# iosefa/obia

Measured on AMD Instinct MI355X. Metric: Mpixel/s (SLIC+zonal feats) on 16384²×8-band; achieved HBM GB/s fraction, higher is better.
Workload: dtype f32

## Files before the change

include/obia_testing.h:

```cpp
#ifndef OBIA_TESTING_H
#define OBIA_TESTING_H

#include "obia_hip.h"

#ifdef __cplusplus
extern "C" {
#endif

int obia_test_clear_ranges_dev(obia_ctx *ctx, void *const *dev_ptrs, const int64_t *bytes, const int32_t *values, int n);

int obia_test_sweep_plan(const int64_t *problems, int n_problems, const int32_t *settings, int repeat, const int32_t *switches,
                         const int64_t *residencies, char *text, int64_t text_bytes);

int obia_test_launch_grid(const char *name, const int64_t *sizes, int n_sizes, int64_t *out4);

int obia_test_launch_grid_names(char *text, int64_t text_bytes);

int obia_test_seam_sort_limit(void);

#ifdef __cplusplus
}
#endif
#endif
```

obia_amd/_lib.py:

```python
import ctypes
import os
import subprocess

import numpy as np

_CSRC = os.path.join(os.path.dirname(os.path.abspath(__file__)), "csrc")
LIB_PATH = os.environ.get("OBIA_HIP_LIB") or os.path.join(_CSRC, "libobia_hip.so")

OBIA_OK = 0
MASK_SEEDS_CHUNK = 1024
E_INVALID, E_HIP, E_NOMEM, E_UNSUPPORTED, E_EMPTY, E_NONFINITE = -1, -2, -3, -4, -5, -6
E_INTERNAL = -7


class SlicParams(ctypes.Structure):
    _fields_ = [("compactness", ctypes.c_double), ("min_size_factor", ctypes.c_double),
                ("max_size_factor", ctypes.c_double), ("n_segments", ctypes.c_int32),
                ("max_num_iter", ctypes.c_int32), ("convert2lab", ctypes.c_int32),
                ("enforce_connectivity", ctypes.c_int32), ("slic_zero", ctypes.c_int32),
                ("start_label", ctypes.c_int32), ("normalize_bands", ctypes.c_int32),
                ("exit_on_fixed_point", ctypes.c_int32), ("reserved", ctypes.c_int32),
                ("sigma_zyx", ctypes.c_double * 3), ("spacing_zyx", ctypes.c_double * 3)]


class SlicSeeds(ctypes.Structure):
    _fields_ = [("yx", ctypes.c_void_p), ("steps_zyx", ctypes.c_double * 3), ("n", ctypes.c_int32),
                ("reserved", ctypes.c_int32)]


class SlicStages(ctypes.Structure):
    _fields_ = [("features", ctypes.c_void_p), ("seeds_yx", ctypes.c_void_p), ("centroids", ctypes.c_void_p),
                ("labels_pre", ctypes.c_void_p), ("centroid_capacity", ctypes.c_int32), ("prepass_only", ctypes.c_int32),
                ("prepass_iters", ctypes.c_int32), ("K", ctypes.c_int32), ("step", ctypes.c_double), ("prescale", ctypes.c_double),
                ("fscale", ctypes.c_double)]


class TilingParams(ctypes.Structure):
    _fields_ = [("crown_radius", ctypes.c_double), ("pixel_width", ctypes.c_double),
                ("pixel_height", ctypes.c_double), ("tile_size", ctypes.c_int32), ("buffer", ctypes.c_int32),
                ("white_order", ctypes.c_int32), ("reserved", ctypes.c_int32)]


class Forest(ctypes.Structure):
    _fields_ = [("threshold", ctypes.c_void_p), ("feature", ctypes.c_void_p), ("left", ctypes.c_void_p), ("right", ctypes.c_void_p),
                ("missing_go_to_left", ctypes.c_void_p), ("tree_offset", ctypes.c_void_p), ("tree_offset_host", ctypes.c_void_p),
                ("value", ctypes.c_void_p), ("n_nodes", ctypes.c_int64), ("n_trees", ctypes.c_int32), ("n_classes", ctypes.c_int32)]


class Mlp(ctypes.Structure):
    _fields_ = [("weights", ctypes.c_void_p), ("biases", ctypes.c_void_p), ("layer_sizes", ctypes.c_void_p), ("n_layers", ctypes.c_int32),
                ("hidden_activation", ctypes.c_int32), ("out_activation", ctypes.c_int32), ("n_classes", ctypes.c_int32)]


_P = ctypes.c_void_p
_I = ctypes.c_int
SEEDING_GRID, SEEDING_SKIMAGE = 0, 1
PickFn = ctypes.CFUNCTYPE(ctypes.c_int, ctypes.c_void_p, ctypes.c_int64, ctypes.c_int32, ctypes.POINTER(ctypes.c_void_p),
                          ctypes.POINTER(ctypes.c_int32), ctypes.POINTER(ctypes.c_void_p), ctypes.POINTER(ctypes.c_int64))
_SIGNATURES = {
    "obia_abi_version": (ctypes.c_int, []),
    "obia_last_error": (ctypes.c_char_p, []),
    "obia_create": (_P, [_I]),
    "obia_create_on_stream": (_P, [_I, _P]),
    "obia_destroy": (None, [_P]),
    "obia_synchronize": (_I, [_P]),
    "obia_workspace_bytes": (ctypes.c_int64, [_P]),
    "obia_slic_default_params": (None, [ctypes.POINTER(SlicParams)]),
    "obia_slic_f32": (_I, [_P, _P, _I, _I, _I, _P, ctypes.POINTER(SlicParams), _P, ctypes.POINTER(_I)]),
    "obia_slic_f32_dev": (_I, [_P, _P, _I, _I, _I, _P, ctypes.POINTER(SlicParams), _P, ctypes.POINTER(_I)]),
    "obia_slic_assign_only_f32_dev": (_I, [_P, _P, _I, _I, _I, _P, ctypes.POINTER(SlicParams), _P, ctypes.POINTER(_I)]),
    "obia_slic_seeded_f32_dev": (_I, [_P, _P, _I, _I, _I, _P, ctypes.POINTER(SlicParams), ctypes.POINTER(SlicSeeds), _I, _P,
                                      ctypes.POINTER(_I)]),
    "obia_mask_centroids_dev": (_I, [_P, _P, _I, _I, _P, ctypes.c_int32, _P, ctypes.c_int64, _I, _P, _P]),
    "obia_slic_stages_f32_dev": (_I, [_P, _P, _I, _I, _I, _P, ctypes.POINTER(SlicParams), ctypes.POINTER(SlicSeeds),
                                      ctypes.POINTER(SlicStages)]),
    "obia_enforce_connectivity_i32_dev": (_I, [_P, _P, _I, _I, _I, _I, _I, _P, ctypes.POINTER(_I)]),
    "obia_zonal_stats_f32": (_I, [_P, _P, _P, _I, _I, _I, _P, _I, _I, _I, _P, _P, _P, _P, _P]),
    "obia_zonal_stats_f32_dev": (_I, [_P, _P, _P, _I, _I, _I, _P, _I, _I, _I, _P, _P, _P, _P, _P]),
    "obia_zonal_moments_f32_dev": (_I, [_P, _P, _P, _I, _I, _I, _P, _I, _I, _I, _P, _P, _P, _P]),
    "obia_zonal_moments_f32": (_I, [_P, _P, _P, _I, _I, _I, _P, _I, _I, _I, _P, _P, _P]),
    "obia_texture_stats_f32_dev": (_I, [_P, _P, _P, _I, _I, _I, _P, _I, _I, _I, _P]),
    "obia_label_edges_u8_dev": (_I, [_P, _P, _I, _I, _P, _P]),
    "obia_sample_labels_i32_dev": (_I, [_P, _P, _I, _I, _P, _P, ctypes.c_int64, _I, _P]),
    "obia_cost_bands_f32_dev": (_I, [_P, _P, ctypes.c_int64, _P, _P]),
    "obia_cost_ndvi_f32_dev": (_I, [_P, _P, _P, ctypes.c_int64, _P]),
    "obia_cost_sobel_f32_dev": (_I, [_P, _P, _I, _I, _P]),
    "obia_cost_select_dev": (_I, [_P, _P, _I, ctypes.c_int64, ctypes.c_double, ctypes.c_double, _P, _P]),
    "obia_cost_entropy_f32_dev": (_I, [_P, _P, _I, _I, ctypes.c_double, ctypes.c_double, _P, _P]),
    "obia_cost_normalise_dev": (_I, [_P, _P, _I, ctypes.c_int64, ctypes.c_double, ctypes.c_double, _P]),
    "obia_cost_edge_count_dev": (_I, [_P, _P, _I, _I, _P]),
    "obia_cost_combine_dev": (_I, [_P, _P, _P, _P, _P, _I, _I, _P, _P, _P, _P]),
    "obia_seeds_peaks_dev": (_I, [_P, _P, _I, _I, ctypes.c_double, _I, ctypes.c_float, _P, _P, _P, _P]),
    "obia_seeds_peaks_gather_dev": (_I, [_P, _P, _P, _P, _P, _I, _I, ctypes.c_int64, _P, _P, _P, _P]),
    "obia_seeds_pair_link_dev": (_I, [_P, _P, _P, _I, _P, _I, _I, _P, ctypes.c_double, ctypes.c_double, _I, _P, ctypes.c_double, _I, _P,
                                      ctypes.POINTER(_I)]),
    "obia_seeds_pair_stats_dev": (_I, [_P, _P, _P, _I, _P, _I, _I, _P, ctypes.c_double, ctypes.c_double, _I, _P, _P, _P]),
    "obia_seeds_pair_matrix_dev": (_I, [_P, _P, _P, _I, _P, _I, _I, _P, ctypes.c_double, ctypes.c_double, _I, _P, _P]),
    "obia_polygon_count_i32_dev": (_I, [_P, _P, _I, _I, _I, _P, _P]),
    "obia_polygon_rings_i32_dev": (_I, [_P, _P, _I, _I, _I, ctypes.c_int64, ctypes.c_int64, _P, _P, _P, _P, _P, _P]),
    "obia_rasterize_polygons_dev": (_I, [_P, _P, _P, ctypes.c_int64, _P, _P, ctypes.c_int64, _I, _I, ctypes.c_int32, _P]),
    "obia_rasterize_info": (_I, [ctypes.POINTER(ctypes.c_int64)]),
    "obia_quickshift_f32": (_I, [_P, _P, _I, _I, _I, ctypes.c_double, ctypes.c_double, ctypes.c_double, ctypes.c_double, _I, _P, _I, _P, ctypes.POINTER(_I)]),
    "obia_quickshift_f32_dev": (_I, [_P, _P, _I, _I, _I, ctypes.c_double, ctypes.c_double, ctypes.c_double, ctypes.c_double, _I, _P, _I, _P, ctypes.POINTER(_I)]),
    "obia_quickshift_stages_f32_dev": (_I, [_P, _P, _I, _I, _I, ctypes.c_double, ctypes.c_double, ctypes.c_double, ctypes.c_double, _I, _P, _I, _P,
                                            ctypes.POINTER(_I), _P, _P, _P, _P, _P, _P]),
    "obia_tiled_slic_f32_dev": (_I, [_P, _P, _P, _I, _I, _I, ctypes.POINTER(TilingParams), ctypes.POINTER(SlicParams), _P,
                                     ctypes.POINTER(ctypes.c_int64)]),
    "obia_tiled_slic_f32": (_I, [_P, _P, _P, _I, _I, _I, ctypes.POINTER(TilingParams), ctypes.POINTER(SlicParams), _P,
                                 ctypes.POINTER(ctypes.c_int64)]),
    "obia_tiled_slic_seeded_f32_dev": (_I, [_P, _P, _P, _I, _I, _I, ctypes.POINTER(TilingParams), ctypes.POINTER(SlicParams), _I, PickFn, _P,
                                            _P, ctypes.POINTER(ctypes.c_int64)]),
    "obia_tiled_slic_seeded_f32": (_I, [_P, _P, _P, _I, _I, _I, ctypes.POINTER(TilingParams), ctypes.POINTER(SlicParams), _I, PickFn, _P,
                                        _P, ctypes.POINTER(ctypes.c_int64)]),
    "obia_tiler_set_seeding": (_I, [_P, _I, PickFn, _P]),
    "obia_tiler_create": (_P, [_P, _P, _P, _I, _I, _I, _I, _I, ctypes.POINTER(TilingParams), ctypes.POINTER(SlicParams), _P, _I]),
    "obia_tiler_destroy": (None, [_P]),
    "obia_tiler_run": (_I, [_P, _I, _I, _I, _I]),
    "obia_tiler_next_id": (_I, [_P]),
    "obia_tiler_set_segments": (_I, [_P, _I, _I, _P]),
    "obia_tiler_get_alive": (_I, [_P, _P, _I]),
    "obia_tiler_set_alive": (_I, [_P, _P, _I]),
    "obia_tiler_finalize": (_I, [_P, ctypes.POINTER(ctypes.c_int64)]),
    "obia_tiler_import_seam": (_I, [_P, _P, _I, _I, _I, _P, _I, _P, _P, ctypes.POINTER(ctypes.c_int), ctypes.POINTER(ctypes.c_int),
                                    ctypes.POINTER(ctypes.c_int)]),
    "obia_table_scale_dev": (_I, [_P, _P, ctypes.c_int64, _I, _P, _P, _P]),
    "obia_forest_predict_dev": (_I, [_P, _P, ctypes.c_int64, _I, ctypes.POINTER(Forest), _P, _P, _P, _P]),
    "obia_mlp_predict_dev": (_I, [_P, _P, ctypes.c_int64, _I, ctypes.POINTER(Mlp), _P, _P, _P, _P, _P]),
    "obia_table_scale_f64_dev": (_I, [_P, _P, ctypes.c_int64, _I, _P, _P, _P]),
    "obia_forest_shap_dev": (_I, [_P, _P, ctypes.c_int64, _I, ctypes.POINTER(Forest), _P, _P, _P]),
    "obia_mlp_coalition_dev": (_I, [_P, _P, ctypes.c_int64, _I, ctypes.POINTER(Mlp), _P, ctypes.c_int64, _P, ctypes.c_int64, _P]),
    "obia_shapley_combine_dev": (_I, [_P, _P, ctypes.c_int64, _I, _I, _P, _P]),
    "obia_set_profiling": (_I, [_P, _I]),
    "obia_last_timing": (ctypes.c_double, [_P, _I]),
}
EXPORTED_SYMBOLS = tuple(_SIGNATURES)
_IMAGE_SIGNATURES = {
    "obia_image_stretch_u8_dev": (_I, [_P, _P, _I, ctypes.c_int64, ctypes.c_double, ctypes.c_double, _P]),
    "obia_image_gray_hist_dev": (_I, [_P, _P, _I, ctypes.c_int64, _P, _P]),
    "obia_image_lut_u8_dev": (_I, [_P, _P, ctypes.c_int64, _P, _I, _P]),
    "obia_image_clahe_u8_dev": (_I, [_P, _P, _I, _I, _I, _I, _P]),
    "obia_image_boundaries_dev": (_I, [_P, _P, _I, _I, _P]),
    "obia_image_mark_u8_dev": (_I, [_P, _P, _I, _P, _I, _I, _P, _P, _P]),
}
SHARP_MAX_WIN = 65536
_SHARPNESS_SIGNATURES = {
    "obia_sharp_gray_lap_dev": (_I, [_P, _P, _I, _I, _I, ctypes.POINTER(ctypes.c_int32), _P, _P]),
    "obia_sharp_laplacian_dev": (_I, [_P, _P, _I, _I, _P, _P]),
    "obia_sharp_box_dev": (_I, [_P, _P, _I, _I, _I, _P, _P, _P]),
    "obia_sharp_variance_dev": (_I, [_P, _P, _I, _I, _I, _P, _P]),
    "obia_sharp_stretch_f32_dev": (_I, [_P, _P, ctypes.c_int64, ctypes.c_double, ctypes.c_double, _P]),
}
TRAIN_MAX_KSIZE = 31
TRAIN_MAX_SIDE = 4096
TRAIN_MINMAX_WORK = 512
_TRAINING_SIGNATURES = {
    "obia_train_blur_u8_dev": (_I, [_P, _P, _I, _I, _I, _I, _I, _P, _P, _P]),
    "obia_train_distance_dev": (_I, [_P, _P, _I, _I, _I, _P, _P]),
    "obia_train_compose_u8_dev": (_I, [_P, _P, _P, _P, _P, _I, _I, _P, ctypes.c_double, _P, _P]),
    "obia_train_minmax_u8_dev": (_I, [_P, _P, ctypes.c_int64, _P, _P, _P]),
}
CROWNS_TILE = 32
_D = ctypes.c_double
_CROWNS_SIGNATURES = {
    "obia_crowns_allocate_dev": (_I, [_P, _P, _P, _I, _I, _P, _P, _I, _D, _D, _D, _D, _I, _D, _P, _P, _P]),
    "obia_crowns_last_work": (_I, [_P, _P]),
}
_L = ctypes.c_int64
_F = ctypes.c_float
_SEED_TABLE_SIGNATURES = {
    "obia_seedtab_cells_dev": (_I, [_P, _P, _P, _L, _D, _P, _P]),
    "obia_seedtab_sample_dev": (_I, [_P, _P, _P, _L, _P, _I, _I, _P, _P, _P]),
    "obia_seedtab_stage1_dev": (_I, [_P, _P, _P, _P, _P, _P, _L, _L, _F, _F, _F, _F, _I, _P, _P, _P]),
    "obia_seedtab_last_work": (_I, [_P, _P]),
    "obia_seedtab_segments_dev": (_I, [_P, _P, _P, _L, _F, _P, _P, _P]),
    "obia_seedtab_nms_dev": (_I, [_P, _P, _P, _P, _P, _P, _P, _L, _L, _D, _D, _P]),
}
BOXES_TABLE = 256
_I32 = ctypes.c_int32
_BOXES_SIGNATURES = {
    "obia_boxes_assign_dev": (_I, [_P, _P, _I, _I, _P, _L, _I32, _P, _P]),
    "obia_boxes_pair_count_dev": (_I, [_P, _P, _I, _I, _P, _L, _I32, _P, _P]),
    "obia_boxes_pair_write_dev": (_I, [_P, _P, _I, _I, _P, _L, _I32, _P, _P, _L, _P, _P, _P, _P]),
    "obia_boxes_dissolve_dev": (_I, [_P, _P, _L, _P, _I32, _P]),
    "obia_boxes_iou_dev": (_I, [_P, _P, _L, _P, _L, _P]),
    "obia_boxes_nms_dev": (_I, [_P, _P, _P, _P, _P, _L, _L, _D, _P, ctypes.POINTER(_I32)]),
}
POINTS_MAX_NZ = 4096
POINTS_CHUNK = 2048
_POINTS_SIGNATURES = {
    "obia_points_rasters_dev": (_I, [_P, _P, _P, _P, _L, ctypes.POINTER(_D), _I, _I, _P, _P]),
    "obia_points_rasters_finish_dev": (_I, [_P, _P, _P, _I, _I, _D, _P, _P]),
    "obia_points_segments_dev": (_I, [_P, _P, _P, _P, _P, _L, ctypes.POINTER(_D), _P, _I, _I, _I32, _I32, _I32, _D, _P, _P, _P, _P, _P, _P]),
    "obia_points_segment_columns_dev": (_I, [_P, _P, _P, _P, _P, _P, _I32, _I32, _D, _D, _D, _P, _P, _P, _P, _P, _P, _P]),
}
_TEST_SIGNATURES = {
    "obia_test_clear_ranges_dev": (_I, [_P, _P, _P, _P, _I]),
    "obia_test_sweep_plan": (_I, [_P, _I, _P, _I, _P, _P, _P, ctypes.c_int64]),
    "obia_test_launch_grid": (_I, [ctypes.c_char_p, _P, _I, _P]),
    "obia_test_launch_grid_names": (_I, [_P, ctypes.c_int64]),
    "obia_test_seam_sort_limit": (_I, []),
}

_lib = None


def build(force=False):
    args = ["make", "-C", _CSRC, "-j8"]
    if force:
        args.append("-B")
    subprocess.check_call(args, stdout=subprocess.DEVNULL)
    return LIB_PATH


def load():
    global _lib
    if _lib is None:
        if not os.path.exists(LIB_PATH):
            raise ImportError(f"{LIB_PATH} not found: build it with `python -c 'import __graft_entry__ as g; g.build()'` "
                              "(hipcc, gfx950). obia_amd has no CPU fallback.")
        lib = ctypes.CDLL(LIB_PATH)
        for name, (res, args) in (list(_SIGNATURES.items()) + list(_IMAGE_SIGNATURES.items()) + list(_SHARPNESS_SIGNATURES.items())
                                   + list(_TRAINING_SIGNATURES.items()) + list(_CROWNS_SIGNATURES.items()) + list(_SEED_TABLE_SIGNATURES.items())
                                   + list(_BOXES_SIGNATURES.items()) + list(_POINTS_SIGNATURES.items()) + list(_TEST_SIGNATURES.items())):
            try:
                fn = getattr(lib, name)
            except AttributeError:
                if os.environ.get("OBIA_HIP_LIB"):
                    continue
                raise
            fn.restype = res
            fn.argtypes = args
        _lib = lib
    return _lib


def last_error():
    return load().obia_last_error().decode("utf-8", "replace")


def check(rc):
    if rc == OBIA_OK:
        return
    msg = last_error()
    if rc in (E_INVALID, E_EMPTY, E_NONFINITE):
        raise ValueError(msg)
    if rc == E_UNSUPPORTED:
        raise NotImplementedError(msg)
    if rc == E_NOMEM:
        raise MemoryError(msg)
    raise RuntimeError(f"obia_hip error {rc}: {msg}")


class Context:

    def __init__(self, device=0, stream=None):
        lib = load()
        if stream is None:
            self._h = lib.obia_create(int(device))
        else:
            self._h = lib.obia_create_on_stream(int(device), ctypes.c_void_p(int(stream)))
        if not self._h:
            raise RuntimeError(f"obia_create failed: {last_error()} (obia_amd needs an AMD GPU; there is no CPU path)")
        self.device = int(device)

    @property
    def handle(self):
        return self._h

    def close(self):
        if getattr(self, "_h", None):
            load().obia_destroy(self._h)
            self._h = None

    def __del__(self):
        try:
            self.close()
        except Exception:
            pass

    def set_profiling(self, on):
        check(load().obia_set_profiling(self._h, int(on)))

    def timing(self):
        lib = load()
        names = ["assign_ms", "sweeps", "features_ms", "connectivity_ms", "zonal_ms", "total_ms", "prepass_ms", "assign_px",
                 "prepass_px", "assign_store_px", "assign_busy_ms", "prepass_busy_ms", "batch_repeats",
                 "prepass_shared_px", "feature_fused_px", "prepass_group_launches", "fills", "uploads", "readbacks",
                 "assign_group_launches", "assign_launch_sum_ms"]
        return {n: lib.obia_last_timing(self._h, i) for i, n in enumerate(names)}

    def workspace_bytes(self):
        return int(load().obia_workspace_bytes(self._h))


_default_ctx = {}


def default_context(device=0):
    ctx = _default_ctx.get(device)
    if ctx is None:
        ctx = _default_ctx[device] = Context(device)
    return ctx


def np_ptr(a):
    return None if a is None else ctypes.c_void_p(a.ctypes.data)


def mask_bytes(mask, device=None):
    import torch
    m = torch.as_tensor(mask, device=device)
    if m.dtype == torch.bool:
        m = m.contiguous().view(torch.uint8)
    elif m.dtype != torch.uint8:
        m = (m != 0).view(torch.uint8)
    return m.contiguous()
```

obia_amd/csrc/common.hpp:

```cpp
#pragma once
#include <hip/hip_runtime.h>
#include <algorithm>
#include <cstdint>
#include <cstdio>
#include <cstring>
#include <string>
#include <vector>

#include "../../include/obia_hip.h"
#include "launch_grids.hpp"

struct obia_ctx;

namespace obia {

void set_error(const char *fmt, ...);

#define OBIA_HIP_TRY(expr)                                                                       \
    do {                                                                                         \
        hipError_t e__ = (expr);                                                                 \
        if (e__ != hipSuccess) {                                                                 \
            obia::set_error("%s:%d: %s -> %s", __FILE__, __LINE__, #expr, hipGetErrorString(e__)); \
            return OBIA_E_HIP;                                                                   \
        }                                                                                        \
    } while (0)

#define OBIA_TRY(expr)            \
    do {                          \
        int rc__ = (expr);        \
        if (rc__ != OBIA_OK) return rc__; \
    } while (0)

class Arena {
  public:
    ~Arena() { release(); }
    void *alloc(size_t bytes);
    template <typename T> T *get(size_t n) { return static_cast<T *>(alloc(n * sizeof(T))); }
    void reset();
    void release();
    struct Mark { size_t block, used, total; };
    Mark mark() const;
    void rewind(const Mark &m);
    size_t capacity() const;
    bool failed() const { return failed_; }

  private:
    struct Block { char *p; size_t size; size_t used; };
    std::vector<Block> blocks_;
    size_t high_water_ = 0, cur_total_ = 0, cur_ = 0;
    bool failed_ = false;
};

class PlanBlob {
  public:
    template <typename T> T *add(obia_ctx *ctx, const T *host, size_t n) { return static_cast<T *>(add_bytes(ctx, host, n * sizeof(T))); }
    int flush(obia_ctx *ctx);
    void drop() { dev_ = host_ = nullptr; cap_ = used_ = 0; }
  private:
    void *add_bytes(obia_ctx *ctx, const void *host, size_t bytes);
    char *dev_ = nullptr, *host_ = nullptr;
    size_t cap_ = 0, used_ = 0;
};

struct Timing {
    double assign_ms = 0, prepass_ms = 0, feat_ms = 0, cc_ms = 0, zonal_ms = 0, total_ms = 0;
    double assign_px = 0, prepass_px = 0;
    double prepass_shared_px = 0;
    double assign_store_px = 0;
    double feat_fused_px = 0;
    int sweeps = 0;
    int prepass_group_launches = 0;
    int assign_group_launches = 0;
    int assign_group_batches = 0;
    double assign_launch_sum_ms = 0;
    int batch_repeats = 0;
    double assign_busy_ms = 0, prepass_busy_ms = 0;
    int fills = 0, uploads = 0, readbacks = 0;
};

}

struct obia_ctx {
    int device = 0;
    hipStream_t stream = nullptr;
    bool own_stream = false;
    obia::Arena arena;
    void *pinned = nullptr;
    size_t pinned_bytes = 0;
    unsigned long long *defer_buf = nullptr;
    bool defer_pending = false;
    double defer_shared_px = 0;
    int32_t *cc_visited = nullptr;
    size_t cc_visited_px = 0;
    bool cc_visited_dirty = false;
    char *up_buf = nullptr;
    size_t up_bytes = 0, up_used = 0;
    obia::PlanBlob plan;
    int profiling = 0;
    obia::Timing timing;
    struct Span { int kind; hipEvent_t a, b; int tag = 0; };
    std::vector<Span> spans;
    std::vector<hipEvent_t> event_pool;
    size_t events_used = 0;
    hipStream_t side = nullptr;
    hipEvent_t aux_fork = nullptr, aux_join = nullptr;
    hipEvent_t grp_fork = nullptr, grp_join = nullptr;
    int spatial_residency[4] = {0, 0, 0, 0};
    int sweep_residency[64] = {};
};

namespace obia {

enum TimeKind { T_ASSIGN = 0, T_FEAT = 2, T_CC = 3, T_ZONAL = 4, T_TOTAL = 5, T_PREPASS = 6, T_ASSIGN_GRP = 7 };

struct ScopedSpan {
    obia_ctx *ctx; bool on; size_t idx;
    ScopedSpan(obia_ctx *c, int kind);
    ~ScopedSpan();
};
struct KernelSpan {
    hipEvent_t a = nullptr, b = nullptr;
    KernelSpan() = default;
    KernelSpan(obia_ctx *c, int kind, int tag = 0);
};
void begin_timing(obia_ctx *ctx);
void resolve_timing(obia_ctx *ctx);

int read_back(obia_ctx *ctx, void *host_dst, const void *dev_src, size_t bytes);
int upload_async(obia_ctx *ctx, void *dev_dst, const void *host_src, size_t bytes);
int fill_async(obia_ctx *ctx, void *dev_dst, int byte, size_t bytes);

struct ClearRange { void *p; unsigned long long bytes; unsigned value, pad; };
struct ClearTable { ClearRange r[16]; int n; };
class ClearSet {
  public:
    explicit ClearSet(obia_ctx *ctx) : ctx_(ctx) { t_.n = 0; }
    int add(void *dev, int byte, size_t bytes);
    int flush();
  private:
    obia_ctx *ctx_;
    ClearTable t_;
};

int side_stream(obia_ctx *ctx);
void debug_sync(obia_ctx *ctx, const char *stage);

static inline int cdiv(long long a, long long b) { return (int)((a + b - 1) / b); }
static inline dim3 to_dim3(const grids::Grid &g) { return dim3((unsigned)g.x.n, (unsigned)g.y.n); }
static inline unsigned flat_grid(long long n) { return (unsigned)grids::flat(n).x.n; }

inline bool misaligned(const void *p, uintptr_t a) { return ((uintptr_t)p & (a - 1)) != 0; }
template <typename... P> bool shared_start(int n_out, P... ps) {
    const void *v[] = {static_cast<const void *>(ps)...};
    const int m = (int)sizeof...(ps);
    for (int i = 0; i < n_out; ++i)
        for (int j = i + 1; j < m; ++j)
            if (v[i] && v[i] == v[j]) return true;
    return false;
}


int enter(obia_ctx *ctx);

int quiesce(obia_ctx *ctx, int rc);

enum FrameOpts : unsigned { FRAME_PLAIN = 0, FRAME_TIMING = 1, FRAME_TOTAL = 2 | FRAME_TIMING };
void frame_begin(obia_ctx *ctx, unsigned opts);
int frame_end(obia_ctx *ctx, unsigned opts, int rc);
template <typename Body> int call_frame(obia_ctx *ctx, unsigned opts, Body &&body) {
    frame_begin(ctx, opts);
    int rc;
    if ((opts & FRAME_TOTAL) == FRAME_TOTAL) {
        ScopedSpan total(ctx, T_TOTAL);
        rc = body();
    } else {
        rc = body();
    }
    return frame_end(ctx, opts, rc);
}

class Staging {
  public:
    explicit Staging(obia_ctx *ctx) : ctx_(ctx) {}
    ~Staging() { (void)finish(); }
    Staging(const Staging &) = delete;
    Staging &operator=(const Staging &) = delete;
    template <typename T> T *in(const T *host, size_t n) { return static_cast<T *>(upload(host, n * sizeof(T))); }
    template <typename T> T *out(size_t n) { return static_cast<T *>(alloc(n * sizeof(T))); }
    template <typename T> void fetch(T *host, const T *dev, size_t n) { download(host, dev, n * sizeof(T)); }
    bool ok() const { return rc_ == OBIA_OK; }
    template <typename Call> void run(Call &&call) { if (ok()) rc_ = call(); }
    int finish();
  private:
    void *alloc(size_t bytes);
    void *upload(const void *host, size_t bytes);
    void download(void *host, const void *dev, size_t bytes);
    obia_ctx *ctx_;
    int rc_ = OBIA_OK;
    bool open_ = true;
    std::vector<void *> bufs_;
};

#if defined(__HIPCC__)
typedef float obia_v4f __attribute__((ext_vector_type(4)));
__device__ __forceinline__ float4 ld_stream_f4(const void *p) {
    const obia_v4f t = __builtin_nontemporal_load(reinterpret_cast<const obia_v4f *>(p));
    return make_float4(t.x, t.y, t.z, t.w);
}
__device__ __forceinline__ unsigned zkey(float f) {
    unsigned b = __float_as_uint(f);
    return (b & 0x80000000u) ? ~b : (b | 0x80000000u);
}
__device__ __forceinline__ float zunkey(unsigned k) {
    unsigned b = (k & 0x80000000u) ? (k & 0x7fffffffu) : ~k;
    return __uint_as_float(b);
}
#endif

}
```

obia_amd/csrc/context.cpp:

```cpp
#include "common.hpp"
#include "../../include/obia_testing.h"

#include <algorithm>
#include <cstdlib>
#include <utility>

#include <cstdarg>

namespace obia {

static thread_local std::string g_last_error;

void set_error(const char *fmt, ...) {
    char buf[1024];
    va_list ap;
    va_start(ap, fmt);
    vsnprintf(buf, sizeof(buf), fmt, ap);
    va_end(ap);
    g_last_error = buf;
}

void *Arena::alloc(size_t bytes) {
    bytes = (bytes + 255) & ~size_t(255);
    if (bytes == 0) bytes = 256;
    for (; cur_ < blocks_.size(); ++cur_) {
        Block &b = blocks_[cur_];
        if (b.size - b.used >= bytes) {
            void *p = b.p + b.used;
            b.used += bytes;
            cur_total_ += bytes;
            if (cur_total_ > high_water_) high_water_ = cur_total_;
            return p;
        }
    }
    size_t want = bytes;
    size_t grow = blocks_.empty() ? (size_t(64) << 20) : 2 * blocks_.back().size;
    if (grow > (size_t(4) << 30)) grow = size_t(4) << 30;
    if (want < grow) want = grow;
    void *p = nullptr;
    if (hipMalloc(&p, want) != hipSuccess) {
        if (want == bytes || hipMalloc(&p, bytes) != hipSuccess) {
            failed_ = true;
            set_error("workspace hipMalloc of %zu bytes failed", bytes);
            return nullptr;
        }
        want = bytes;
    }
    blocks_.push_back(Block{static_cast<char *>(p), want, bytes});
    cur_ = blocks_.size() - 1;
    cur_total_ += bytes;
    if (cur_total_ > high_water_) high_water_ = cur_total_;
    return p;
}

Arena::Mark Arena::mark() const {
    Mark m;
    m.block = cur_ < blocks_.size() ? cur_ : blocks_.size();
    m.used = m.block < blocks_.size() ? blocks_[m.block].used : 0;
    m.total = cur_total_;
    return m;
}

void Arena::rewind(const Mark &m) {
    for (size_t i = m.block + 1; i < blocks_.size(); ++i) blocks_[i].used = 0;
    if (m.block < blocks_.size()) blocks_[m.block].used = m.used;
    cur_ = m.block;
    cur_total_ = m.total;
}

void Arena::reset() {
    failed_ = false;
    cur_total_ = 0;
    cur_ = 0;
    if (blocks_.size() > 1) {
        size_t total = 0;
        for (auto &b : blocks_) total += b.size;
        for (auto &b : blocks_) (void)hipFree(b.p);
        blocks_.clear();
        void *p = nullptr;
        if (hipMalloc(&p, high_water_ + (high_water_ >> 3)) == hipSuccess) blocks_.push_back(Block{static_cast<char *>(p), high_water_ + (high_water_ >> 3), 0});
        (void)total;
    } else if (!blocks_.empty()) {
        blocks_[0].used = 0;
    }
}

void Arena::release() {
    for (auto &b : blocks_) (void)hipFree(b.p);
    blocks_.clear();
}

size_t Arena::capacity() const {
    size_t t = 0;
    for (auto &b : blocks_) t += b.size;
    return t;
}

static hipEvent_t get_event(obia_ctx *ctx) {
    if (ctx->events_used == ctx->event_pool.size()) {
        hipEvent_t e = nullptr;
        (void)hipEventCreate(&e);
        ctx->event_pool.push_back(e);
    }
    return ctx->event_pool[ctx->events_used++];
}

ScopedSpan::ScopedSpan(obia_ctx *c, int kind) : ctx(c), on(c->profiling == 1 || (c->profiling == 2 && kind == T_ASSIGN)), idx(0) {
    if (!on) return;
    obia_ctx::Span s{kind, get_event(ctx), get_event(ctx)};
    (void)hipEventRecord(s.a, ctx->stream);
    idx = ctx->spans.size();
    ctx->spans.push_back(s);
}
ScopedSpan::~ScopedSpan() {
    if (on) (void)hipEventRecord(ctx->spans[idx].b, ctx->stream);
}

int side_stream(obia_ctx *ctx) {
    if (!ctx->aux_fork) OBIA_HIP_TRY(hipEventCreateWithFlags(&ctx->aux_fork, hipEventDisableTiming));
    if (!ctx->aux_join) OBIA_HIP_TRY(hipEventCreateWithFlags(&ctx->aux_join, hipEventDisableTiming));
    if (!ctx->grp_fork) OBIA_HIP_TRY(hipEventCreateWithFlags(&ctx->grp_fork, hipEventDisableTiming));
    if (!ctx->grp_join) OBIA_HIP_TRY(hipEventCreateWithFlags(&ctx->grp_join, hipEventDisableTiming));
    if (!ctx->side) OBIA_HIP_TRY(hipStreamCreateWithFlags(&ctx->side, hipStreamNonBlocking));
    return OBIA_OK;
}

KernelSpan::KernelSpan(obia_ctx *c, int kind, int tag) {
    if (!(c->profiling == 1 || (c->profiling == 2 && (kind == T_ASSIGN || kind == T_ASSIGN_GRP)))) return;
    a = get_event(c);
    b = get_event(c);
    c->spans.push_back(obia_ctx::Span{kind, a, b, tag});
}

void begin_timing(obia_ctx *ctx) {
    ctx->spans.clear();
    ctx->events_used = 0;
    ctx->timing = Timing();
}

void resolve_timing(obia_ctx *ctx) {
    if (!ctx->profiling) return;
    (void)hipStreamSynchronize(ctx->stream);
    typedef std::vector<std::pair<double, double>> Intervals;
    auto union_ms = [](Intervals &v) {
        std::sort(v.begin(), v.end());
        double busy = 0, lo = 0, hi = -1;
        for (auto &x : v) {
            if (hi < lo || x.first > hi) { if (hi > lo) busy += hi - lo; lo = x.first; hi = x.second; }
            else if (x.second > hi) hi = x.second;
        }
        if (hi > lo) busy += hi - lo;
        return busy;
    };
    Intervals iv[2];
    std::vector<Intervals> grouped;
    hipEvent_t ref = nullptr;
    for (auto &s : ctx->spans) {
        float ms = 0;
        if (hipEventElapsedTime(&ms, s.a, s.b) != hipSuccess) { (void)hipGetLastError(); continue; }
        if (s.kind == T_ASSIGN || s.kind == T_ASSIGN_GRP || s.kind == T_PREPASS) {
            if (!ref) ref = s.a;
            float end = 0;
            if (hipEventElapsedTime(&end, ref, s.b) == hipSuccess) {
                const std::pair<double, double> x((double)end - ms, (double)end);
                iv[s.kind == T_PREPASS ? 1 : 0].push_back(x);
                if (s.kind == T_ASSIGN_GRP) {
                    const size_t batch = (size_t)(s.tag >> 1);
                    if (grouped.size() <= batch) grouped.resize(batch + 1);
                    grouped[batch].push_back(x);
                }
            }
            else (void)hipGetLastError();
        }
        switch (s.kind) {
            case T_ASSIGN: ctx->timing.assign_ms += ms; ctx->timing.assign_launch_sum_ms += ms; ctx->timing.sweeps += 1; break;
            case T_ASSIGN_GRP: ctx->timing.assign_launch_sum_ms += ms; if (!(s.tag & 1)) ctx->timing.sweeps += 1; break;
            case T_FEAT: ctx->timing.feat_ms += ms; break;
            case T_CC: ctx->timing.cc_ms += ms; break;
            case T_ZONAL: ctx->timing.zonal_ms += ms; break;
            case T_TOTAL: ctx->timing.total_ms += ms; break;
            case T_PREPASS: ctx->timing.prepass_ms += ms; break;
            default: break;
        }
    }
    for (auto &g : grouped) ctx->timing.assign_ms += union_ms(g);
    ctx->timing.assign_busy_ms += union_ms(iv[0]);
    ctx->timing.prepass_busy_ms += union_ms(iv[1]);
    ctx->spans.clear();
}

int read_back(obia_ctx *ctx, void *host_dst, const void *dev_src, size_t bytes) {
    if (bytes > ctx->pinned_bytes) {
        if (ctx->pinned) (void)hipHostFree(ctx->pinned);
        ctx->pinned = nullptr;
        size_t want = bytes < 4096 ? 4096 : bytes;
        OBIA_HIP_TRY(hipHostMalloc(&ctx->pinned, want, hipHostMallocDefault));
        ctx->pinned_bytes = want;
    }
    OBIA_TRY(ctx->plan.flush(ctx));
    OBIA_HIP_TRY(hipMemcpyAsync(ctx->pinned, dev_src, bytes, hipMemcpyDeviceToHost, ctx->stream));
    ctx->timing.readbacks += 1;
    OBIA_HIP_TRY(hipStreamSynchronize(ctx->stream));
    ctx->up_used = 0;
    memcpy(host_dst, ctx->pinned, bytes);
    return OBIA_OK;
}

void debug_sync(obia_ctx *ctx, const char *stage) {
    static const bool on = std::getenv("OBIA_DEBUG_SYNC") != nullptr;
    if (!on) return;
    const hipError_t e = hipStreamSynchronize(ctx->stream);
    fprintf(stderr, "[obia debug] %s: %s\n", stage, e == hipSuccess ? "ok" : hipGetErrorString(e));
    fflush(stderr);
}

int fill_async(obia_ctx *ctx, void *dev_dst, int byte, size_t bytes) {
    if (bytes == 0) return OBIA_OK;
    OBIA_HIP_TRY(hipMemsetAsync(dev_dst, byte, bytes, ctx->stream));
    ctx->timing.fills += 1;
    return OBIA_OK;
}

template <bool RAGGED> __global__ __launch_bounds__(256) void clear_ranges_kernel(const ClearTable T) {
    const size_t tid = (size_t)blockIdx.x * blockDim.x + threadIdx.x, stride = (size_t)gridDim.x * blockDim.x;
    for (int k = 0; k < T.n; ++k) {
        unsigned char *p = static_cast<unsigned char *>(T.r[k].p);
        const size_t n = T.r[k].bytes;
        const unsigned v = (T.r[k].value & 0xffu) * 0x01010101u;
        size_t head = RAGGED ? (16 - (reinterpret_cast<uintptr_t>(p) & 15)) & 15 : 0;
        if (head > n) head = n;
        const size_t nvec = (n - head) / 16, tail0 = head + nvec * 16;
        uint4 *pv = reinterpret_cast<uint4 *>(p + head);
        for (size_t i = tid; i < nvec; i += stride) pv[i] = make_uint4(v, v, v, v);
        if (RAGGED) {
            if (tid < head) p[tid] = (unsigned char)v;
            if (tid < n - tail0) p[tail0 + tid] = (unsigned char)v;
        }
    }
}

int ClearSet::add(void *dev, int byte, size_t bytes) {
    if (bytes == 0) return OBIA_OK;
    if (t_.n == 16) OBIA_TRY(flush());
    t_.r[t_.n++] = ClearRange{dev, (unsigned long long)bytes, (unsigned)byte & 0xffu, 0u};
    return OBIA_OK;
}

int ClearSet::flush() {
    const int n = t_.n;
    t_.n = 0;
    if (n == 0) return OBIA_OK;
    if (n == 1) return fill_async(ctx_, t_.r[0].p, (int)t_.r[0].value, (size_t)t_.r[0].bytes);
    unsigned long long longest = 0;
    bool ragged = false;
    for (int k = 0; k < n; ++k) {
        longest = std::max(longest, t_.r[k].bytes);
        ragged = ragged || ((reinterpret_cast<uintptr_t>(t_.r[k].p) | (uintptr_t)t_.r[k].bytes) & 15) != 0;
    }
    ClearTable t = t_;
    t.n = n;
    const dim3 grid(flat_grid((long long)((longest + 15) / 16)));
    if (ragged) hipLaunchKernelGGL(HIP_KERNEL_NAME(clear_ranges_kernel<true>), grid, dim3(256), 0, ctx_->stream, t);
    else hipLaunchKernelGGL(HIP_KERNEL_NAME(clear_ranges_kernel<false>), grid, dim3(256), 0, ctx_->stream, t);
    OBIA_HIP_TRY(hipGetLastError());
    ctx_->timing.fills += 1;
    return OBIA_OK;
}

constexpr size_t RING = 8u << 20;

static int ring_ready(obia_ctx *ctx) {
    if (ctx->up_buf) return OBIA_OK;
    void *p = nullptr;
    OBIA_HIP_TRY(hipHostMalloc(&p, RING, hipHostMallocDefault));
    ctx->up_buf = static_cast<char *>(p);
    ctx->up_bytes = RING;
    ctx->up_used = 0;
    return OBIA_OK;
}

void *PlanBlob::add_bytes(obia_ctx *ctx, const void *host, size_t bytes) {
    constexpr size_t BLOCK = 64u << 10;
    const size_t need = (bytes + 15) & ~size_t(15);
    if (dev_ && used_ + need > cap_ && flush(ctx) != OBIA_OK) return nullptr;
    if (ring_ready(ctx) != OBIA_OK) return nullptr;
    if (need > ctx->up_bytes / 2) {
        if (flush(ctx) != OBIA_OK) return nullptr;
        void *d = ctx->arena.alloc(need);
        return d && upload_async(ctx, d, host, bytes) == OBIA_OK ? d : nullptr;
    }
    if (!dev_) {
        const size_t cap = (std::max(need, BLOCK) + 63) & ~size_t(63);
        if (ctx->up_used + cap > ctx->up_bytes) {
            if (hipStreamSynchronize(ctx->stream) != hipSuccess) { set_error("stream synchronisation failed (plan upload)"); return nullptr; }
            ctx->up_used = 0;
        }
        char *d = static_cast<char *>(ctx->arena.alloc(cap));
        if (!d) return nullptr;
        dev_ = d;
        host_ = ctx->up_buf + ctx->up_used;
        ctx->up_used += cap;
        cap_ = cap;
        used_ = 0;
    }
    void *d = dev_ + used_;
    if (bytes) memcpy(host_ + used_, host, bytes);
    used_ += need;
    return d;
}

int PlanBlob::flush(obia_ctx *ctx) {
    if (!dev_) return OBIA_OK;
    char *const dev = dev_, *const host = host_;
    const size_t used = used_, cap = cap_;
    dev_ = host_ = nullptr;
    cap_ = used_ = 0;
    if (ctx->up_buf && host + cap == ctx->up_buf + ctx->up_used) ctx->up_used -= cap - ((used + 63) & ~size_t(63));
    if (used == 0) return OBIA_OK;
    OBIA_HIP_TRY(hipMemcpyAsync(dev, host, used, hipMemcpyHostToDevice, ctx->stream));
    ctx->timing.uploads += 1;
    return OBIA_OK;
}

int upload_async(obia_ctx *ctx, void *dev_dst, const void *host_src, size_t bytes) {
    if (bytes == 0) return OBIA_OK;
    ctx->timing.uploads += 1;
    OBIA_TRY(ring_ready(ctx));
    if (bytes > ctx->up_bytes) {
        OBIA_TRY(ctx->plan.flush(ctx));
        OBIA_HIP_TRY(hipMemcpyAsync(dev_dst, host_src, bytes, hipMemcpyHostToDevice, ctx->stream));
        OBIA_HIP_TRY(hipStreamSynchronize(ctx->stream));
        ctx->up_used = 0;
        return OBIA_OK;
    }
    if (ctx->up_used + bytes > ctx->up_bytes) {
        OBIA_TRY(ctx->plan.flush(ctx));
        OBIA_HIP_TRY(hipStreamSynchronize(ctx->stream));
        ctx->up_used = 0;
    }
    char *slot = ctx->up_buf + ctx->up_used;
    memcpy(slot, host_src, bytes);
    OBIA_HIP_TRY(hipMemcpyAsync(dev_dst, slot, bytes, hipMemcpyHostToDevice, ctx->stream));
    ctx->up_used += (bytes + 63) & ~(size_t)63;
    return OBIA_OK;
}

int enter(obia_ctx *ctx) {
    if (!ctx) { set_error("null context"); return OBIA_E_INVALID; }
    if (hipSetDevice(ctx->device) != hipSuccess) { set_error("hipSetDevice(%d) failed", ctx->device); return OBIA_E_HIP; }
    return OBIA_OK;
}

int quiesce(obia_ctx *ctx, int rc) {
    (void)hipStreamSynchronize(ctx->stream);
    if (ctx->side) (void)hipStreamSynchronize(ctx->side);
    return rc;
}

void frame_begin(obia_ctx *ctx, unsigned opts) {
    ctx->plan.drop();
    ctx->arena.reset();
    if (opts & FRAME_TIMING) begin_timing(ctx);
}

int frame_end(obia_ctx *ctx, unsigned opts, int rc) {
    if (rc != OBIA_OK) return quiesce(ctx, rc);
    OBIA_TRY(ctx->plan.flush(ctx));
    OBIA_HIP_TRY(hipStreamSynchronize(ctx->stream));
    if (opts & FRAME_TIMING) resolve_timing(ctx);
    return OBIA_OK;
}

void *Staging::alloc(size_t bytes) {
    if (!ok()) return nullptr;
    void *p = nullptr;
    if (hipMalloc(&p, bytes) != hipSuccess) {
        set_error("device allocation for host-pointer call failed");
        rc_ = OBIA_E_NOMEM;
        return nullptr;
    }
    bufs_.push_back(p);
    return p;
}

void *Staging::upload(const void *host, size_t bytes) {
    if (!host) return nullptr;
    void *p = alloc(bytes);
    if (p && hipMemcpyAsync(p, host, bytes, hipMemcpyHostToDevice, ctx_->stream) != hipSuccess) {
        set_error("host->device copy failed in a host-pointer call");
        rc_ = OBIA_E_HIP;
    }
    return p;
}

void Staging::download(void *host, const void *dev, size_t bytes) {
    if (ok() && hipMemcpyAsync(host, dev, bytes, hipMemcpyDeviceToHost, ctx_->stream) != hipSuccess) {
        set_error("device->host copy failed in a host-pointer call");
        rc_ = OBIA_E_HIP;
    }
}

int Staging::finish() {
    if (open_) {
        open_ = false;
        (void)hipStreamSynchronize(ctx_->stream);
        for (void *p : bufs_) (void)hipFree(p);
        bufs_.clear();
    }
    return rc_;
}

}

using namespace obia;

extern "C" {

int obia_abi_version(void) { return OBIA_ABI_VERSION; }

const char *obia_last_error(void) { return g_last_error.c_str(); }

static obia_ctx *create_impl(int device_id, void *stream, bool own) {
    int n = 0;
    if (hipGetDeviceCount(&n) != hipSuccess || n <= 0) {
        set_error("no HIP device available");
        return nullptr;
    }
    if (device_id < 0 || device_id >= n) {
        set_error("device_id %d out of range (%d devices)", device_id, n);
        return nullptr;
    }
    if (hipSetDevice(device_id) != hipSuccess) {
        set_error("hipSetDevice(%d) failed", device_id);
        return nullptr;
    }
    obia_ctx *ctx = new obia_ctx();
    ctx->device = device_id;
    if (own) {
        if (hipStreamCreateWithFlags(&ctx->stream, hipStreamNonBlocking) != hipSuccess) {
            set_error("hipStreamCreate failed");
            delete ctx;
            return nullptr;
        }
        ctx->own_stream = true;
    } else {
        ctx->stream = static_cast<hipStream_t>(stream);
    }
    return ctx;
}

obia_ctx *obia_create(int device_id) { return create_impl(device_id, nullptr, true); }
obia_ctx *obia_create_on_stream(int device_id, void *hip_stream) { return create_impl(device_id, hip_stream, false); }

void obia_destroy(obia_ctx *ctx) {
    if (!ctx) return;
    (void)hipSetDevice(ctx->device);
    (void)hipStreamSynchronize(ctx->stream);
    ctx->arena.release();
    if (ctx->up_buf) (void)hipHostFree(ctx->up_buf);
    if (ctx->pinned) (void)hipHostFree(ctx->pinned);
    if (ctx->defer_buf) (void)hipHostFree(ctx->defer_buf);
    if (ctx->cc_visited) (void)hipFree(ctx->cc_visited);
    for (auto e : ctx->event_pool) (void)hipEventDestroy(e);
    if (ctx->side) (void)hipStreamDestroy(ctx->side);
    if (ctx->aux_fork) (void)hipEventDestroy(ctx->aux_fork);
    if (ctx->aux_join) (void)hipEventDestroy(ctx->aux_join);
    if (ctx->grp_fork) (void)hipEventDestroy(ctx->grp_fork);
    if (ctx->grp_join) (void)hipEventDestroy(ctx->grp_join);
    if (ctx->own_stream) (void)hipStreamDestroy(ctx->stream);
    delete ctx;
}

int obia_synchronize(obia_ctx *ctx) {
    if (!ctx) { set_error("null context"); return OBIA_E_INVALID; }
    OBIA_HIP_TRY(hipStreamSynchronize(ctx->stream));
    return OBIA_OK;
}

int obia_test_clear_ranges_dev(obia_ctx *ctx, void *const *dev_ptrs, const int64_t *bytes, const int32_t *values, int n) {
    OBIA_TRY(enter(ctx));
    if (!dev_ptrs || !bytes || !values || n < 0) { set_error("clear ranges: null array or negative count"); return OBIA_E_INVALID; }
    for (int i = 0; i < n; ++i)
        if (bytes[i] < 0 || (bytes[i] > 0 && !dev_ptrs[i])) { set_error("clear ranges: range %d is not a range", i); return OBIA_E_INVALID; }
    return call_frame(ctx, FRAME_TIMING, [&] {
        ClearSet clr(ctx);
        for (int i = 0; i < n; ++i) OBIA_TRY(clr.add(dev_ptrs[i], values[i], (size_t)bytes[i]));
        return clr.flush();
    });
}

int64_t obia_workspace_bytes(obia_ctx *ctx) { return ctx ? (int64_t)ctx->arena.capacity() : 0; }

void obia_slic_default_params(obia_slic_params *p) {
    if (!p) return;
    p->n_segments = 100;
    p->compactness = 10.0;
    p->max_num_iter = 10;
    p->convert2lab = -1;
    p->enforce_connectivity = 1;
    p->min_size_factor = 0.5;
    p->max_size_factor = 3.0;
    p->slic_zero = 0;
    p->start_label = 1;
    p->normalize_bands = 0;
    p->exit_on_fixed_point = 0;
    p->reserved = 0;
    p->sigma_zyx[0] = p->sigma_zyx[1] = p->sigma_zyx[2] = 0.0;
    p->spacing_zyx[0] = p->spacing_zyx[1] = p->spacing_zyx[2] = 1.0;
}

int obia_set_profiling(obia_ctx *ctx, int enabled) {
    if (!ctx) { set_error("null context"); return OBIA_E_INVALID; }
    ctx->profiling = enabled < 0 ? 0 : (enabled > 2 ? 1 : enabled);
    return OBIA_OK;
}

double obia_last_timing(obia_ctx *ctx, int what) {
    if (!ctx) return -1.0;
    switch (what) {
        case 0: return ctx->timing.assign_ms;
        case 1: return (double)ctx->timing.sweeps;
        case 2: return ctx->timing.feat_ms;
        case 3: return ctx->timing.cc_ms;
        case 4: return ctx->timing.zonal_ms;
        case 5: return ctx->timing.total_ms;
        case 6: return ctx->timing.prepass_ms;
        case 7: return ctx->timing.assign_px;
        case 8: return ctx->timing.prepass_px;
        case 9: return ctx->timing.assign_store_px;
        case 10: return ctx->timing.assign_busy_ms;
        case 11: return ctx->timing.prepass_busy_ms;
        case 12: return (double)ctx->timing.batch_repeats;
        case 13: return ctx->timing.prepass_shared_px;
        case 14: return ctx->timing.feat_fused_px;
        case 15: return (double)ctx->timing.prepass_group_launches;
        case 16: return (double)ctx->timing.fills;
        case 17: return (double)ctx->timing.uploads;
        case 18: return (double)ctx->timing.readbacks;
        case 19: return (double)ctx->timing.assign_group_launches;
        case 20: return ctx->timing.assign_launch_sum_ms;
        default: return -1.0;
    }
}

}
```

obia_amd/csrc/launch_grids.hpp:

```cpp
#pragma once
#include <algorithm>
#include <cstdint>

#include "../../include/obia_points.h"
#include "../../include/obia_training.h"

namespace obia {
namespace grids {

constexpr long long GRID_X_MAX = 0x7fffffffLL, GRID_Y_MAX = 65535;

constexpr int COST_SOBEL_TW = 64, COST_SOBEL_TH = 16;
constexpr int COST_ENTROPY_TW = 64, COST_ENTROPY_TH = 16;
constexpr int COST_SELECT_THREADS = 1024;
constexpr int SEEDS_FLAG_TW = 64, SEEDS_FLAG_TH = 16;
constexpr int SEEDS_PAIR_TILE = 64;
constexpr int CLAHE_ROWS = 32;
constexpr int QS_TILE = 16;
constexpr int RAST_LARGE_TILE_W = 2048;
constexpr int SHARPNESS_MINMAX_PARTS = 2048;
constexpr int TILER_IDS_PER_WG = 256 * 16;

inline long long cdivl(long long a, long long b) { return (a + b - 1) / b; }

struct Axis { long long n, trips; };
struct Grid { Axis x, y; };

inline Axis strided(long long units, long long cap) {
    const long long g = std::max(1LL, std::min(units, std::max(1LL, cap)));
    return Axis{g, std::max(1LL, cdivl(units, g))};
}
inline Axis whole(long long units) { return Axis{std::max(1LL, units), 1}; }
inline Grid one_axis(Axis x) { return Grid{x, Axis{1, 1}}; }

inline Grid flat(long long n) { return one_axis(strided(cdivl(n, 256), 8192)); }
inline Grid image_stretch(long long n) { return flat(n / 4 + 2); }
inline Grid image_lut(long long n, long long rep) { return flat(n * rep / 4 + 2); }
inline Grid image_gray_hist(long long n) { return one_axis(strided(cdivl(n / 4 + 2, 256), 2048)); }
inline Grid training_compose(long long npx) { return flat((3 * npx + 6) / 4); }
inline Grid training_minmax_scale(long long n) { return flat((n + 6) / 4); }
inline Grid training_minmax_reduce(long long n) { return one_axis(strided(cdivl(n, 256), OBIA_TRAIN_MINMAX_WORK / 2)); }
inline Grid sharpness_minmax(long long npx) { return one_axis(strided(cdivl(npx, 256), SHARPNESS_MINMAX_PARTS)); }
inline Grid scale_transform(long long n_rows, long long F) { return one_axis(strided(cdivl(n_rows * F, 256), 2048)); }
inline Grid cost_select(long long nv) { return one_axis(strided(cdivl(nv, COST_SELECT_THREADS), 512)); }
inline Grid seeds_gauss(long long npx) { return one_axis(strided(cdivl(npx, 256), 16384)); }
inline Grid seeds_pairs(long long n) {
    const long long nt = cdivl(n, SEEDS_PAIR_TILE);
    return one_axis(strided(nt * (nt + 1) / 2, 256 * 16));
}
inline Grid points_segments(long long n) { return one_axis(strided(cdivl(n, OBIA_POINTS_CHUNK), 1280)); }
inline Grid boxes_walk(long long n) { return one_axis(strided(n, 4096)); }
inline Grid quickshift_flat(long long npx) { return one_axis(strided(cdivl(npx, 256 * 4), 65535)); }
inline Grid quickshift_gauss(long long n) { return one_axis(strided(cdivl(n, 256), 65535)); }
inline Grid polygons_candidates(long long npx) { return one_axis(strided(cdivl(npx, 256 * 4), 262144)); }
inline Grid rast_value(long long npx) { return one_axis(strided(cdivl(npx, 256 * 4), 16384)); }
inline Grid zonal_labels(long long nlb) { return one_axis(strided(cdivl(nlb, 256), 4096)); }
inline Grid texture_segments(long long n_labels) { return one_axis(strided(n_labels, 65536)); }
inline Grid texture_big_segments(long long n_big) { return one_axis(strided(n_big, 256)); }
inline Grid label_edges(long long H) { return one_axis(strided(H, 8192)); }

inline Grid image_rows(long long H, long long W) { return Grid{strided(cdivl(W / 4 + 2, 256), 64), strided(H, GRID_Y_MAX)}; }
inline Grid image_clahe_interp(long long H, long long W) { return Grid{whole(cdivl(W, 256)), strided(cdivl(H, CLAHE_ROWS), GRID_Y_MAX)}; }
inline long long image_clahe_hist_rows(long long th, long long tw) {
    return std::max(std::max(1LL, 16384 / std::max(1LL, tw)), cdivl(th, GRID_Y_MAX));
}
inline Grid image_clahe_hist(long long th, long long tw) { return Grid{whole(64), whole(cdivl(th, image_clahe_hist_rows(th, tw)))}; }
inline Grid cost_rows(long long H, long long W) { return Grid{whole(cdivl(W, 256)), strided(H, GRID_Y_MAX)}; }
inline Grid tiles(long long H, long long W, long long tw, long long th) { return Grid{whole(cdivl(W, tw)), strided(cdivl(H, th), GRID_Y_MAX)}; }
inline Grid cost_sobel(long long H, long long W) { return tiles(H, W, COST_SOBEL_TW, COST_SOBEL_TH); }
inline Grid cost_entropy(long long H, long long W) { return tiles(H, W, COST_ENTROPY_TW, COST_ENTROPY_TH); }
inline Grid seeds_flag(long long H, long long W) { return tiles(H, W, SEEDS_FLAG_TW, SEEDS_FLAG_TH); }
inline Grid quickshift_density(long long H, long long W) { return tiles(H, W, QS_TILE, QS_TILE); }
inline Grid cost_edge_count(long long H, long long W) {
    const Axis x = strided(cdivl(W, 256), 16);
    return Grid{x, strided(H, std::max(1LL, 4096 / x.n))};
}
inline Grid boxes_iou(long long na, long long nb) { return Grid{strided(cdivl(nb, 256), 4096), strided(na, 4096)}; }
inline Grid rast_band_bin(long long n_large, long long max_nv) { return Grid{whole(n_large), strided(cdivl(max_nv, 256), 64)}; }
inline Grid rast_large(long long n_bands, long long max_w) { return Grid{whole(n_bands), strided(cdivl(max_w, RAST_LARGE_TILE_W), 1024)}; }

inline Grid slic_band_minmax(long long maxh, long long np) { return Grid{strided(maxh, 2048), whole(np)}; }
inline Grid slic_feature_rows(long long rows, long long np) { return Grid{strided(rows, 4096), whole(np)}; }
inline Grid slic_gauss(long long n, long long np) { return Grid{strided(cdivl(n, 256), 65535), whole(np)}; }
inline Grid slic_stage_features(long long n) { return one_axis(strided(cdivl(n, 256), 65535)); }
inline Grid slic_fill_labels(long long npx) { return one_axis(strided(cdivl(npx, 256 * 8), 65535)); }
inline Grid slic_mask_pack(long long maxh, long long np) { return Grid{strided((maxh + 3) / 4, 16384), whole(np)}; }
inline Grid slic_maxdist(long long maxh, long long np) { return Grid{strided(maxh, 4096), whole(np)}; }
inline Grid cc_flat(long long npx) { return one_axis(strided(cdivl(npx, 256 * 4), 65535 * 4)); }
inline Grid cc_seam(long long max_seam, long long np) { return Grid{strided(cdivl(max_seam, 256), 65535), whole(np)}; }
inline Grid tiler_rows(long long maxh, long long np) { return Grid{strided(maxh, 8192), whole(np)}; }
inline Grid tiler_ids_apply(long long npx) { return one_axis(strided(cdivl(npx, TILER_IDS_PER_WG), 65535)); }
inline Grid tiler_seam(long long n) { return one_axis(strided(cdivl(n, 256), 2048)); }

struct Named {
    const char *name;
    int n_sizes;
    const char *sizes;
    Grid (*fn)(const long long *s);
};

#define OBIA_GRID1(f, doc) {#f, 1, doc, [](const long long *s) { return f(s[0]); }}
#define OBIA_GRID2(f, doc) {#f, 2, doc, [](const long long *s) { return f(s[0], s[1]); }}
#define OBIA_GRID4(f, doc) {#f, 4, doc, [](const long long *s) { return f(s[0], s[1], s[2], s[3]); }}
inline const Named *table(int *count) {
    static const Named TABLE[] = {
    OBIA_GRID1(flat, "n"),
    OBIA_GRID1(image_stretch, "n"),
    OBIA_GRID2(image_lut, "n rep"),
    OBIA_GRID1(image_gray_hist, "n"),
    OBIA_GRID1(training_compose, "npx"),
    OBIA_GRID1(training_minmax_scale, "n"),
    OBIA_GRID1(training_minmax_reduce, "n"),
    OBIA_GRID1(sharpness_minmax, "npx"),
    OBIA_GRID2(scale_transform, "n_rows F"),
    OBIA_GRID1(cost_select, "nv"),
    OBIA_GRID1(seeds_gauss, "npx"),
    OBIA_GRID1(seeds_pairs, "n"),
    OBIA_GRID1(points_segments, "n"),
    OBIA_GRID1(boxes_walk, "n"),
    OBIA_GRID1(quickshift_flat, "npx"),
    OBIA_GRID1(quickshift_gauss, "n"),
    OBIA_GRID1(polygons_candidates, "npx"),
    OBIA_GRID1(rast_value, "npx"),
    OBIA_GRID1(zonal_labels, "nlb"),
    OBIA_GRID1(texture_segments, "n_labels"),
    OBIA_GRID1(texture_big_segments, "n_big"),
    OBIA_GRID1(label_edges, "H"),
    OBIA_GRID2(image_rows, "H W"),
    OBIA_GRID2(image_clahe_interp, "H W"),
    OBIA_GRID2(image_clahe_hist, "th tw"),
    OBIA_GRID2(cost_rows, "H W"),
    OBIA_GRID4(tiles, "H W tw th"),
    OBIA_GRID2(cost_sobel, "H W"),
    OBIA_GRID2(cost_entropy, "H W"),
    OBIA_GRID2(seeds_flag, "H W"),
    OBIA_GRID2(quickshift_density, "H W"),
    OBIA_GRID2(cost_edge_count, "H W"),
    OBIA_GRID2(boxes_iou, "na nb"),
    OBIA_GRID2(rast_band_bin, "n_large max_nv"),
    OBIA_GRID2(rast_large, "n_bands max_w"),
    OBIA_GRID2(slic_band_minmax, "maxh np"),
    OBIA_GRID2(slic_feature_rows, "rows np"),
    OBIA_GRID2(slic_gauss, "n np"),
    OBIA_GRID1(slic_stage_features, "n"),
    OBIA_GRID1(slic_fill_labels, "npx"),
    OBIA_GRID2(slic_mask_pack, "maxh np"),
    OBIA_GRID2(slic_maxdist, "maxh np"),
    OBIA_GRID1(cc_flat, "npx"),
    OBIA_GRID2(cc_seam, "max_seam np"),
    OBIA_GRID2(tiler_rows, "maxh np"),
    OBIA_GRID1(tiler_ids_apply, "npx"),
    OBIA_GRID1(tiler_seam, "n"),
    };
    *count = (int)(sizeof(TABLE) / sizeof(TABLE[0]));
    return TABLE;
}
#undef OBIA_GRID1
#undef OBIA_GRID2
#undef OBIA_GRID4

}
}
```

obia_amd/csrc/slic.hip:

```cpp
#include "slic.hpp"
#include "slic_features.hpp"

#include <cmath>
#include <cstdlib>

namespace obia {

void regular_grid_hw(long long H, long long W, long long n, long long out[4]) {
    long long dims[3] = {1, H, W};
    int order[3] = {0, 1, 2};
    for (int i = 0; i < 3; ++i)
        for (int j = i + 1; j < 3; ++j)
            if (dims[order[j]] < dims[order[i]]) std::swap(order[i], order[j]);
    double sd[3];
    for (int i = 0; i < 3; ++i) sd[i] = (double)dims[order[i]];
    double space = sd[0] * sd[1] * sd[2];
    if (space <= (double)n) { out[0] = out[1] = out[2] = out[3] = 0; return; }
    double st[3];
    for (int i = 0; i < 3; ++i) st[i] = std::pow(space / (double)n, 1.0 / 3.0);
    auto all_ge = [&]() { return sd[0] >= st[0] && sd[1] >= st[1] && sd[2] >= st[2]; };
    if (!all_ge()) {
        for (int d = 0; d < 3; ++d) {
            st[d] = sd[d];
            double sp = 1.0;
            for (int e = d + 1; e < 3; ++e) sp *= sd[e];
            if (d < 2) {
                double v = std::pow(sp / (double)n, 1.0 / (double)(3 - d - 1));
                for (int e = d + 1; e < 3; ++e) st[e] = v;
            }
            if (all_ge()) break;
        }
    }
    long long start[3], step[3], s_of[3], t_of[3];
    for (int i = 0; i < 3; ++i) {
        start[i] = (long long)std::floor(st[i] / 2.0);
        step[i] = (long long)std::nearbyint(st[i]);
    }
    for (int i = 0; i < 3; ++i) { s_of[order[i]] = start[i]; t_of[order[i]] = step[i]; }
    out[0] = s_of[1]; out[1] = t_of[1]; out[2] = s_of[2]; out[3] = t_of[2];
}

static long long slice_len(long long L, long long start, long long step) {
    if (step == 0) return L;
    if (start >= L) return 0;
    return (L - start + step - 1) / step;
}


constexpr int FP_NT = 256;

__device__ __forceinline__ void lazy_atomic_min(unsigned *a, unsigned v) {
    if (v < __hip_atomic_load(a, __ATOMIC_RELAXED, __HIP_MEMORY_SCOPE_AGENT)) atomicMin(a, v);
}
__device__ __forceinline__ void lazy_atomic_max(unsigned *a, unsigned v) {
    if (v > __hip_atomic_load(a, __ATOMIC_RELAXED, __HIP_MEMORY_SCOPE_AGENT)) atomicMax(a, v);
}

template <int VEC>
__global__ __launch_bounds__(FP_NT) void band_minmax_kernel(const float *__restrict__ src, int Ws, int C,
                                                            const SrcWindow *__restrict__ wins,
                                                            unsigned *__restrict__ keys ,
                                                            int *__restrict__ nonfinite) {
    __shared__ unsigned s_mn[32], s_mx[32];
    const int p = blockIdx.y;
    const SrcWindow wdw = wins[p];
    const int period = C / VEC;
    const int active = (FP_NT / period) * period;
    const int tid = threadIdx.x;
    if (tid < 32) { s_mn[tid] = 0xffffffffu; s_mx[tid] = 0u; }
    __syncthreads();
    float lo[VEC], hi[VEC];
#pragma unroll
    for (int v = 0; v < VEC; ++v) { lo[v] = INFINITY; hi[v] = -INFINITY; }
    bool bad = false;
    if (tid < active) {
        const long long row_vecs = (long long)wdw.w * period;
        for (int y = blockIdx.x; y < wdw.h; y += gridDim.x) {
            const float *row = src + ((long long)(wdw.y0 + y) * Ws + wdw.x0) * C;
            constexpr int MU = 4;
            for (long long e0 = tid; e0 < row_vecs; e0 += (long long)MU * active) {
                float v[MU][VEC];
#pragma unroll
                for (int u = 0; u < MU; ++u) {
                    const long long e = e0 + (long long)u * active;
                    if (e < row_vecs) {
                        if (VEC == 4) {
                            const float4 t = *reinterpret_cast<const float4 *>(row + 4 * e);
                            v[u][0] = t.x; v[u][1 % VEC] = t.y; v[u][2 % VEC] = t.z; v[u][3 % VEC] = t.w;
                        } else v[u][0] = row[e];
                    } else {
#pragma unroll
                        for (int q = 0; q < VEC; ++q) v[u][q] = lo[q];
                    }
                }
#pragma unroll
                for (int u = 0; u < MU; ++u) {
                    const bool live = e0 + (long long)u * active < row_vecs;
#pragma unroll
                    for (int q = 0; q < VEC; ++q) {
                        if (live) bad |= !(fabsf(v[u][q]) <= 3.4028234e38f);
                        lo[q] = fminf(lo[q], v[u][q]);
                        if (live) hi[q] = fmaxf(hi[q], v[u][q]);
                    }
                }
            }
        }
        const int band0 = (tid % period) * VEC;
#pragma unroll
        for (int q = 0; q < VEC; ++q)
            if (lo[q] <= hi[q]) {
                atomicMin(&s_mn[band0 + q], f2key(lo[q]));
                atomicMax(&s_mx[band0 + q], f2key(hi[q]));
            }
        if (bad && __hip_atomic_load(&nonfinite[p], __ATOMIC_RELAXED, __HIP_MEMORY_SCOPE_AGENT) == 0) atomicOr(&nonfinite[p], 1);
    }
    __syncthreads();
    if (tid < C) {
        if (s_mn[tid] != 0xffffffffu) atomicMin(&keys[((long long)p * C + tid) * 2 + 0], s_mn[tid]);
        if (s_mx[tid] != 0u) atomicMax(&keys[((long long)p * C + tid) * 2 + 1], s_mx[tid]);
    }
}

__device__ __forceinline__ void rgb2lab_f32(float r, float g, float b, float &L, float &A, float &B) {
    float a[3] = {r, g, b};
#pragma unroll
    for (int c = 0; c < 3; ++c) {
        float v = a[c];
        a[c] = (v > 0.04045f) ? powf((v + 0.055f) / 1.055f, 2.4f) : v / 12.92f;
    }
    const float m[3][3] = {{0.412453f, 0.357580f, 0.180423f},
                           {0.212671f, 0.715160f, 0.072169f},
                           {0.019334f, 0.119193f, 0.950227f}};
    const float wr[3] = {0.95047f, 1.0f, 1.08883f};
    float xyz[3];
#pragma unroll
    for (int i = 0; i < 3; ++i) {
        float s = a[0] * m[i][0];
        s = s + a[1] * m[i][1];
        s = s + a[2] * m[i][2];
        s = s / wr[i];
        xyz[i] = (s > 0.008856f) ? cbrtf(s) : 7.787f * s + 16.0f / 116.0f;
    }
    L = 116.0f * xyz[1] - 16.0f;
    A = 500.0f * (xyz[0] - xyz[1]);
    B = 200.0f * (xyz[1] - xyz[2]);
}

template <int CP>
__device__ __forceinline__ float feature_pixel(const float *__restrict__ px, int C, bool vec, int normalize, int to_lab, float ratio,
                                               const float (&bmn)[CP], const float (&bden)[CP], float (&v)[CP]) {
    if (vec) {
#pragma unroll
        for (int q = 0; q < CP / 4; ++q) {
            const float4 t = reinterpret_cast<const float4 *>(px)[q];
            v[4 * q] = t.x; v[4 * q + 1] = t.y; v[4 * q + 2] = t.z; v[4 * q + 3] = t.w;
        }
    } else {
#pragma unroll
        for (int c = 0; c < CP; ++c) v[c] = (c < C) ? px[c] : 0.0f;
    }
    if (normalize) {
#pragma unroll
        for (int c = 0; c < CP; ++c) v[c] = feature_normalized(v[c], bmn[c], bden[c]);
    } else {
#pragma unroll
        for (int c = 0; c < CP; ++c) if (!(fabsf(v[c]) <= 3.0e38f)) v[c] = 0.0f;
    }
    if (to_lab) {
        float L, A, B;
        rgb2lab_f32(v[0], v[1], v[2], L, A, B);
        v[0] = L; v[1] = A; v[2] = B;
    }
    float m = 0.0f;
#pragma unroll
    for (int c = 0; c < CP; ++c) {
        v[c] = v[c] * ratio;
        m = fmaxf(m, fabsf(v[c]));
    }
    return m;
}

template <int CP>
__device__ __forceinline__ void feature_band_params(const unsigned *__restrict__ keys, int p, int C, int normalize, float (&bmn)[CP],
                                                    float (&bden)[CP]) {
#pragma unroll
    for (int c = 0; c < CP; ++c) {
        bmn[c] = 0.0f; bden[c] = 1.0f;
        if (normalize && c < C) feature_band_param(keys, p, C, c, bmn[c], bden[c]);
    }
}

template <int CP>
__global__ __launch_bounds__(256) void features_kernel(const float *__restrict__ src, int Ws, int C,
                                                       const SrcWindow *__restrict__ wins,
                                                       const unsigned *__restrict__ keys, int normalize,
                                                       int to_lab, float ratio, float *__restrict__ feat,
                                                       unsigned *__restrict__ maxabs_bits) {
    const int p = blockIdx.y;
    const SrcWindow wdw = wins[p];
    float bmn[CP], bden[CP];
    feature_band_params<CP>(keys, p, C, normalize, bmn, bden);
    const bool vec = (C == CP);
    float local_max = 0.0f;
    for (int y = blockIdx.x; y < wdw.h; y += gridDim.x)
    for (int x = threadIdx.x; x < wdw.w; x += blockDim.x) {
        const long long i = (long long)y * wdw.w + x;
        const float *px = src + ((long long)(wdw.y0 + y) * Ws + wdw.x0 + x) * C;
        float v[CP];
        local_max = fmaxf(local_max, feature_pixel<CP>(px, C, vec, normalize, to_lab, ratio, bmn, bden, v));
        float4 *dst = reinterpret_cast<float4 *>(feat + (wdw.pix_off + i) * CP);
#pragma unroll
        for (int q = 0; q < CP / 4; ++q) dst[q] = make_float4(v[4 * q], v[4 * q + 1], v[4 * q + 2], v[4 * q + 3]);
    }
#pragma unroll
    for (int off = 32; off > 0; off >>= 1) local_max = fmaxf(local_max, __shfl_xor(local_max, off));
    if ((threadIdx.x & 63) == 0) lazy_atomic_max(maxabs_bits + p, __float_as_uint(local_max));
}

template <int CP, bool BOX>
__global__ __launch_bounds__(256) void features_planes_kernel(const float *__restrict__ src, int Ws, int C,
                                                              const SrcWindow *__restrict__ wins,
                                                              const unsigned *__restrict__ keys, int normalize,
                                                              int to_lab, float ratio, float *__restrict__ feat,
                                                              unsigned *__restrict__ maxabs_bits, float *__restrict__ fbox, int dense) {
    const int p = blockIdx.y;
    const SrcWindow wdw = wins[p];
    float bmn[CP], bden[CP];
    feature_band_params<CP>(keys, p, C, normalize, bmn, bden);
    const bool vec = (C == CP);
    float local_max = 0.0f;
    const int QH = (wdw.h + 3) >> 2, XB = (wdw.w + 15) >> 4;
    float4 *__restrict__ planes = reinterpret_cast<float4 *>(feat) + wdw.feat_off;
    auto quad = [&](int q, int x, float (&v)[4][CP]) {
#pragma unroll
        for (int i = 0; i < 4; ++i) {
            const int y = 4 * q + i;
            if (y < wdw.h && x < wdw.w) {
                const float *px = dense ? src + (wdw.pix_off + (long long)y * wdw.w + x) * CP
                                        : src + ((long long)(wdw.y0 + y) * Ws + wdw.x0 + x) * C;
                local_max = fmaxf(local_max, feature_pixel<CP>(px, C, vec, normalize, to_lab, ratio, bmn, bden, v[i]));
            } else {
#pragma unroll
                for (int c = 0; c < CP; ++c) v[i][c] = 0.0f;
            }
        }
        float4 *dst = planes + ((long long)q * XB + (x >> 4)) * (CP * 16) + (x & 15);
#pragma unroll
        for (int c = 0; c < CP; ++c)
            if (c < C) dst[c * 16] = make_float4(v[0][c], v[1][c], v[2][c], v[3][c]);
    };
    if (!BOX) {
        for (int q = blockIdx.x; q < QH; q += gridDim.x)
            for (int x = threadIdx.x; x < 16 * XB; x += blockDim.x) {
                float v[4][CP];
                quad(q, x, v);
            }
    } else {
        const int FH = (QH + 3) >> 2;
        for (int fy = blockIdx.x; fy < FH; fy += gridDim.x)
            for (int x = threadIdx.x; x < 16 * XB; x += blockDim.x) {
                float lo[CP], hi[CP];
#pragma unroll
                for (int c = 0; c < CP; ++c) { lo[c] = INFINITY; hi[c] = -INFINITY; }
                for (int qq = 0; qq < 4; ++qq) {
                    const int q = 4 * fy + qq;
                    if (q >= QH) break;
                    float v[4][CP];
                    quad(q, x, v);
#pragma unroll
                    for (int i = 0; i < 4; ++i)
                        if (4 * q + i < wdw.h && x < wdw.w) {
#pragma unroll
                            for (int c = 0; c < CP; ++c) { lo[c] = fminf(lo[c], v[i][c]); hi[c] = fmaxf(hi[c], v[i][c]); }
                        }
                }
#pragma unroll
                for (int c = 0; c < CP; ++c)
#pragma unroll
                    for (int off = 8; off > 0; off >>= 1) {
                        lo[c] = fminf(lo[c], __shfl_xor(lo[c], off));
                        hi[c] = fmaxf(hi[c], __shfl_xor(hi[c], off));
                    }
                if ((x & 15) == 0) {
                    float *o = fbox + (wdw.fb_off + (long long)fy * XB + (x >> 4)) * (2 * CP);
#pragma unroll
                    for (int c = 0; c < CP; ++c) { o[c] = lo[c]; o[CP + c] = hi[c]; }
                }
            }
    }
#pragma unroll
    for (int off = 32; off > 0; off >>= 1) local_max = fmaxf(local_max, __shfl_xor(local_max, off));
    if ((threadIdx.x & 63) == 0) lazy_atomic_max(maxabs_bits + p, __float_as_uint(local_max));
}

bool slic_use_colour_bound(float ratio, bool to_lab) {
    return ratio * (to_lab ? 100.0f : 1.0f) >= 2.0f;
}

__global__ void keys_init_kernel(unsigned *keys, int nkeys, int ntot) {
    const int i = blockIdx.x * blockDim.x + threadIdx.x;
    if (i < ntot) keys[i] = (i < nkeys && (i & 1) == 0) ? 0xffffffffu : 0u;
}


template <int AXIS>
__global__ __launch_bounds__(256) void gauss_axis_kernel(const SrcWindow *__restrict__ wins, const float *__restrict__ in,
                                                         float *__restrict__ out, int CP, const double *__restrict__ w, int r) {
    const SrcWindow wdw = wins[blockIdx.y];
    const long long n_el = (long long)wdw.h * wdw.w * CP;
    const float *a = in + wdw.pix_off * CP;
    float *o = out + wdw.pix_off * CP;
    const int n = AXIS == 1 ? wdw.h : (AXIS == 2 ? wdw.w : 1);
    const long long stride = AXIS == 1 ? (long long)wdw.w * CP : (long long)CP;
    for (long long i = (long long)blockIdx.x * blockDim.x + threadIdx.x; i < n_el; i += (long long)gridDim.x * blockDim.x) {
        const int pos = AXIS == 1 ? (int)(i / stride) : (AXIS == 2 ? (int)((i / CP) % wdw.w) : 0);
        const float *line = a + (i - (long long)pos * stride);
        double tmp = (double)a[i] * w[0];
        for (int j = r; j >= 1; --j) {
            int lo = pos - j, hi = pos + j;
            if (AXIS == 0) { lo = 0; hi = 0; }
            else {
                const int per = 2 * n;
                lo %= per; if (lo < 0) lo += per; if (lo >= n) lo = per - 1 - lo;
                hi %= per; if (hi >= n) hi = per - 1 - hi;
            }
            tmp += ((double)line[(long long)lo * stride] + (double)line[(long long)hi * stride]) * w[j];
        }
        o[i] = (float)tmp;
    }
}

static double np_pairwise_sum(const double *a, size_t n) {
    if (n < 8) { double r = 0.0; for (size_t i = 0; i < n; ++i) r += a[i]; return r; }
    if (n <= 128) {
        double r[8];
        for (int j = 0; j < 8; ++j) r[j] = a[j];
        size_t i = 8;
        for (; i < n - (n % 8); i += 8) for (int j = 0; j < 8; ++j) r[j] += a[i + j];
        double res = ((r[0] + r[1]) + (r[2] + r[3])) + ((r[4] + r[5]) + (r[6] + r[7]));
        for (; i < n; ++i) res += a[i];
        return res;
    }
    size_t n2 = n / 2;
    n2 -= n2 % 8;
    return np_pairwise_sum(a, n2) + np_pairwise_sum(a + n2, n - n2);
}

int gaussian_weights_host(double sigma, bool sigma_is_f32, std::vector<double> &w) {
    const float s32 = (float)sigma;
    const double sd = sigma_is_f32 ? (double)s32 : sigma;
    const int r = (int)(4.0 * sd + 0.5);
    const double sigma2 = sigma_is_f32 ? (double)(s32 * s32) : sigma * sigma;
    std::vector<double> phi((size_t)2 * r + 1);
    for (int x = -r; x <= r; ++x) phi[(size_t)(x + r)] = std::exp(-0.5 / sigma2 * (double)((long long)x * x));
    const double sum = np_pairwise_sum(phi.data(), phi.size());
    w.resize((size_t)r + 1);
    for (int j = 0; j <= r; ++j) w[(size_t)j] = phi[(size_t)(r + j)] / sum;
    return r;
}

int smooth_prepare(obia_ctx *ctx, SmoothSpec &sm, long long total_pix, int CP, int np) {
    if (!sm.on()) return OBIA_OK;
    Arena &A = ctx->arena;
    sm.tmp_a = A.get<float>((size_t)total_pix * CP);
    sm.tmp_b = A.get<float>((size_t)total_pix * CP);
    sm.d_scratch = A.get<unsigned>((size_t)np);
    if (!sm.tmp_a || !sm.tmp_b || !sm.d_scratch) return OBIA_E_NOMEM;
    for (int ax = 0; ax < 3; ++ax) {
        if (!(sm.sigma[ax] > 1e-15)) continue;
        if (!(sm.sigma[ax] < 1.0e6)) { set_error("sigma %g not supported", sm.sigma[ax]); return OBIA_E_INVALID; }
        std::vector<double> w;
        const int r = gaussian_weights_host(sm.sigma[ax], true, w);
        sm.radius[ax] = r;
        sm.d_w[ax] = A.get<double>((size_t)r + 1);
        if (!sm.d_w[ax]) return OBIA_E_NOMEM;
        OBIA_TRY(upload_async(ctx, sm.d_w[ax], w.data(), sizeof(double) * w.size()));
    }
    return OBIA_OK;
}

int slic_features_launch(hipStream_t stream, const SlicBatch &b, const float *src, int Ws, unsigned *d_keys, const SmoothSpec *smooth,
                         bool minmax_only) {
    const int C = b.C, CP = b.CP, np = b.nprob, maxh = b.maxh, normalize = b.normalize, to_lab = b.to_lab;
    const SrcWindow *d_windows = b.d_windows;
    const float ratio = b.feat_ratio;
    float *d_feat = b.d_feat, *d_fbox = b.col_lb ? b.d_fbox : nullptr;
    const bool planes = b.feat_planes;
    if (C < 1 || C > 16) { set_error("band count %d not supported (1..16)", C); return OBIA_E_UNSUPPORTED; }
    const size_t nkeys = (size_t)np * C * 2, ntot = nkeys + 2 * (size_t)np;
    unsigned *d_nonfinite = d_keys + nkeys, *d_maxabs = d_nonfinite + np;
    hipLaunchKernelGGL(keys_init_kernel, dim3(cdiv((long long)ntot, 256)), dim3(256), 0, stream, d_keys, (int)nkeys, (int)ntot);
    if (normalize) {
        const int gx = (int)grids::slic_band_minmax(maxh, np).x.n;
        if (C % 4 == 0 && (reinterpret_cast<uintptr_t>(src) & 15) == 0)
            hipLaunchKernelGGL(HIP_KERNEL_NAME(band_minmax_kernel<4>), dim3(gx, np), dim3(FP_NT), 0, stream, src, Ws, C, d_windows,
                               d_keys, (int *)d_nonfinite);
        else
            hipLaunchKernelGGL(HIP_KERNEL_NAME(band_minmax_kernel<1>), dim3(gx, np), dim3(FP_NT), 0, stream, src, Ws, C, d_windows,
                               d_keys, (int *)d_nonfinite);
    }
    if (minmax_only) { OBIA_HIP_TRY(hipGetLastError()); return OBIA_OK; }
    const bool box = planes && d_fbox != nullptr;
    const int rows = box ? (maxh + 15) / 16 : (planes ? (maxh + 3) / 4 : maxh);
    const dim3 grid = to_dim3(grids::slic_feature_rows(rows, np));
    const bool smoothing = smooth && smooth->on();
    if (smoothing && !planes) { set_error("Gaussian pre-smoothing is built for the SLIC feature layout only"); return OBIA_E_UNSUPPORTED; }
    const float *planes_src = src;
    int planes_norm = normalize, planes_lab = to_lab, dense = 0;
    if (smoothing) {
        OBIA_HIP_TRY(hipMemsetAsync(smooth->d_scratch, 0, sizeof(unsigned) * (size_t)np, stream));
        const dim3 g1 = to_dim3(grids::slic_feature_rows(maxh, np));
#define LAUNCH_UNSCALED(CPV) hipLaunchKernelGGL(HIP_KERNEL_NAME(features_kernel<CPV>), g1, dim3(256), 0, stream, src, Ws, C, d_windows, \
                                                d_keys, normalize, to_lab, 1.0f, smooth->tmp_a, smooth->d_scratch)
        switch (CP) {
            case 4: LAUNCH_UNSCALED(4); break;
            case 8: LAUNCH_UNSCALED(8); break;
            case 12: LAUNCH_UNSCALED(12); break;
            default: LAUNCH_UNSCALED(16); break;
        }
#undef LAUNCH_UNSCALED
        float *cur = smooth->tmp_a, *oth = smooth->tmp_b;
        const dim3 gg = to_dim3(grids::slic_gauss(b.maxpix * CP, np));
        for (int ax = 0; ax < 3; ++ax) {
            if (!(smooth->sigma[ax] > 1e-15)) continue;
            if (ax == 0) hipLaunchKernelGGL(HIP_KERNEL_NAME(gauss_axis_kernel<0>), gg, dim3(256), 0, stream, d_windows, cur, oth, CP, smooth->d_w[0], smooth->radius[0]);
            else if (ax == 1) hipLaunchKernelGGL(HIP_KERNEL_NAME(gauss_axis_kernel<1>), gg, dim3(256), 0, stream, d_windows, cur, oth, CP, smooth->d_w[1], smooth->radius[1]);
            else hipLaunchKernelGGL(HIP_KERNEL_NAME(gauss_axis_kernel<2>), gg, dim3(256), 0, stream, d_windows, cur, oth, CP, smooth->d_w[2], smooth->radius[2]);
            std::swap(cur, oth);
        }
        planes_src = cur; planes_norm = 0; planes_lab = 0; dense = 1;
    }
#define LAUNCH_FEAT(CPV)                                                                                                  \
    do {                                                                                                                  \
        if (box) hipLaunchKernelGGL(HIP_KERNEL_NAME(features_planes_kernel<CPV, true>), grid, dim3(256), 0, stream, planes_src, Ws, C, \
                                    d_windows, d_keys, planes_norm, planes_lab, ratio, d_feat, d_maxabs, d_fbox, dense);  \
        else if (planes) hipLaunchKernelGGL(HIP_KERNEL_NAME(features_planes_kernel<CPV, false>), grid, dim3(256), 0, stream, planes_src, Ws, C, \
                                       d_windows, d_keys, planes_norm, planes_lab, ratio, d_feat, d_maxabs, (float *)nullptr, dense); \
        else hipLaunchKernelGGL(HIP_KERNEL_NAME(features_kernel<CPV>), grid, dim3(256), 0, stream, src, Ws, C, d_windows,  \
                                d_keys, normalize, to_lab, ratio, d_feat, d_maxabs);                                      \
    } while (0)
    switch (CP) {
        case 4: LAUNCH_FEAT(4); break;
        case 8: LAUNCH_FEAT(8); break;
        case 12: LAUNCH_FEAT(12); break;
        case 16: LAUNCH_FEAT(16); break;
        default: set_error("bad CP %d", CP); return OBIA_E_INVALID;
    }
#undef LAUNCH_FEAT
    OBIA_HIP_TRY(hipGetLastError());
    return OBIA_OK;
}

int slic_features_finish(SlicBatch &b, const unsigned *keys, const unsigned *nonfinite, const unsigned *maxabs_bits, std::vector<int> *skip) {
    const int C = b.C, np = b.nprob;
    auto k2f = [](unsigned k) { unsigned bb = (k & 0x80000000u) ? (k & 0x7fffffffu) : ~k; float f; memcpy(&f, &bb, 4); return f; };
    if (skip) skip->assign(np, 0);
    if (b.normalize) {
        for (int p = 0; p < np; ++p) {
            bool bad = nonfinite[p] != 0;
            int cb = -1;
            float cv = 0;
            for (int c = 0; c < C && !bad; ++c) {
                float mn = k2f(keys[((size_t)p * C + c) * 2]), mx = k2f(keys[((size_t)p * C + c) * 2 + 1]);
                if (!(mx > mn)) { cb = c; cv = mn; }
            }
            if (bad || cb >= 0) {
                if (skip) { (*skip)[p] = 1; continue; }
                if (bad) set_error("input raster holds NaN or infinite values");
                else set_error("band %d is constant (%g): normalize_band would divide 0 by 0 "
                               "(obia/segmentation/segment_boundaries.py:16)", cb, (double)cv);
                return OBIA_E_NONFINITE;
            }
        }
    }
    if (b.fuse_features) { b.fscale = slic_fscale(b.feat_ratio); return OBIA_OK; }
    float maxabs = 0.0f;
    for (int p = 0; p < np; ++p) {
        float v; memcpy(&v, &maxabs_bits[p], 4);
        if (!(v <= 3.0e38f)) { set_error("non-finite feature values"); return OBIA_E_NONFINITE; }
        if (v > maxabs) maxabs = v;
    }
    b.fscale = slic_fscale(maxabs);
    const bool smoothed = b.sigma[0] > 1e-15 || b.sigma[1] > 1e-15 || b.sigma[2] > 1e-15;
    if (b.prescale != 1.0f && !smoothed && maxabs > 0.0f && b.fscale != slic_fscale(b.feat_ratio)) {
        set_error("largest feature %g of normalised bands is not the ratio %g", (double)maxabs, (double)b.feat_ratio);
        return OBIA_E_INVALID;
    }
    return OBIA_OK;
}

double slic_fscale(float maxabs) {
    int s = 0;
    if (maxabs > 0.0f) {
        int e = 0;
        (void)std::frexp((double)maxabs, &e);
        s = 29 - e;
    }
    if (s > 100) s = 100;
    if (s < -90) s = -90;
    return std::ldexp(1.0, s);
}

#ifndef OBIA_FUSE_FEATURES_DEFAULT
#define OBIA_FUSE_FEATURES_DEFAULT 1
#endif
bool slic_fuse_features(const SlicBatch &b, const float *src, int Ws) {
    const char *e = std::getenv("OBIA_FUSE_FEATURES");
    if (e ? e[0] == '0' : !OBIA_FUSE_FEATURES_DEFAULT) return false;
    if (!b.feat_planes || !b.normalize || b.to_lab || b.slic_zero || b.prescale == 1.0f) return false;
    if (b.sigma[0] > 1e-15 || b.sigma[1] > 1e-15 || b.sigma[2] > 1e-15) return false;
    if (!b.masked || b.max_iter < 1) return false;
    if (b.direct || b.exit_on_fixed_point) return false;
    if (b.col_lb) return false;
    if (b.C % 4 != 0 || (reinterpret_cast<uintptr_t>(src) & 15) != 0) return false;
    if (b.CP > 12) return false;
    if ((double)Ws * b.C * 4.0 * 20.0 >= 4294967296.0) return false;
    return true;
}

float slic_prescale(float ratio, int normalize, int to_lab, bool slic_zero) {
    if (!normalize || to_lab || slic_zero || !(ratio > 0.0f) || !(ratio < 3.0e38f)) return 1.0f;
    int e = 0;
    (void)std::frexp((double)ratio, &e);
    int s = 29 - e;
    if (s > 40 || s < -24) return 1.0f;
    return (float)std::ldexp(1.0, s);
}

void slic_batch_settings(SlicBatch &b, const obia_slic_params &p, int C, int normalize_bands, bool masked) {
    b.C = C;
    b.CP = (C + 3) & ~3;
    b.masked = masked;
    b.start_label = p.start_label;
    b.max_iter = p.max_num_iter;
    b.slic_zero = p.slic_zero != 0;
    for (int i = 0; i < 3; ++i) { b.sigma[i] = p.sigma_zyx[i]; b.spacing[i] = p.spacing_zyx[i]; }
    b.direct = (float)b.spacing[1] != 1.0f || (float)b.spacing[2] != 1.0f;
    b.exit_on_fixed_point = p.exit_on_fixed_point != 0 && !b.direct;
    b.normalize = normalize_bands;
    b.to_lab = (C == 3 && p.convert2lab != 0) ? 1 : 0;
    const float ratio = (float)(1.0 / p.compactness);
    b.col_lb = slic_use_colour_bound(ratio, b.to_lab != 0) && !b.slic_zero && !b.exit_on_fixed_point && !b.direct;
    b.prescale = slic_prescale(ratio, normalize_bands, b.to_lab, b.slic_zero);
    b.feat_ratio = ratio * b.prescale;
}

int slic_batch_layout(SlicBatch &b) {
    if ((long long)b.windows.size() > grids::GRID_Y_MAX) { set_error("%zu windows in one batch, the limit is %lld", b.windows.size(), grids::GRID_Y_MAX); return OBIA_E_UNSUPPORTED; }
    b.nprob = (int)b.windows.size();
    b.probs.assign(b.windows.size(), SlicProblem{});
    long long off = 0, foff = 0, boff = 0, m4 = 0;
    for (int p = 0; p < b.nprob; ++p) {
        SrcWindow &w = b.windows[p];
        SlicProblem &P = b.probs[p];
        P.H = w.h; P.W = w.w; P.XB = feat_xb(w.w);
        P.pix_off = w.pix_off = off;
        P.feat_off = w.feat_off = foff;
        P.fb_off = w.fb_off = boff;
        P.m4_off = (int)m4;
        const long long n = (long long)w.h * w.w;
        if (n > b.maxpix) b.maxpix = n;
        if (w.h > b.maxh) b.maxh = w.h;
        off += n;
        foff += feat_block_f4(w.h, w.w, b.CP);
        boff += feat_boxes(w.h, w.w);
        m4 += (long long)((w.h + 3) / 4) * w.w;
    }
    if (off > 0x7fffffffLL || m4 > 0x7fffffffLL) { set_error("batch of %lld pixels too large", off); return OBIA_E_INVALID; }
    b.total_pix = off; b.total_feat_f4 = foff; b.total_boxes = boff;
    b.total_m4 = m4 > 0 ? m4 : 1;
    return OBIA_OK;
}

int slic_prepare_features(obia_ctx *ctx, SlicBatch &b, const float *src, int Ws, std::vector<int> *skip) {
    ScopedSpan span(ctx, T_FEAT);
    const int np = b.nprob;
    const size_t nkeys = (size_t)np * b.C * 2, ntot = nkeys + 2 * (size_t)np;
    unsigned *d_keys = ctx->arena.get<unsigned>(ntot);
    if (!d_keys) return OBIA_E_NOMEM;
    SmoothSpec sm;
    for (int i = 0; i < 3; ++i) sm.sigma[i] = b.sigma[i];
    OBIA_TRY(smooth_prepare(ctx, sm, b.total_pix, b.CP, np));
    b.fuse_features = slic_fuse_features(b, src, Ws);
    if (b.fuse_features) { b.raw_src = src; b.raw_ws = Ws; b.d_keys = d_keys; }
    OBIA_TRY(slic_features_launch(ctx->stream, b, src, Ws, d_keys, &sm, b.fuse_features));
    std::vector<unsigned> host(ntot);
    OBIA_TRY(read_back(ctx, host.data(), d_keys, ntot * sizeof(unsigned)));
    return slic_features_finish(b, host.data(), host.data() + nkeys, host.data() + nkeys + np, skip);
}

struct SeedGrid { int start_y, step_y, ny, start_x, step_x, nx; int cent_off; int slots; };

__global__ void seed_grid_kernel(const SeedGrid *__restrict__ grids, int nprob, float *__restrict__ seed,
                                 int *__restrict__ cent_prob) {
    const int p = blockIdx.y;
    const SeedGrid g = grids[p];
    const int K = g.ny * g.nx;
    for (int k = blockIdx.x * blockDim.x + threadIdx.x; k < K; k += gridDim.x * blockDim.x) {
        const int iy = k / g.nx, ix = k % g.nx;
        seed[2 * (size_t)(g.cent_off + k)] = (float)(g.start_y + iy * g.step_y);
        seed[2 * (size_t)(g.cent_off + k) + 1] = (float)(g.start_x + ix * g.step_x);
        cent_prob[g.cent_off + k] = p;
    }
}

__global__ __launch_bounds__(256) void seed_masked_kernel(const SeedGrid *__restrict__ grids,
                                                          const SlicProblem *__restrict__ probs,
                                                          const uint8_t *__restrict__ mask, float *__restrict__ seed,
                                                          int *__restrict__ cent_prob, int *__restrict__ K_out) {
    constexpr int U = 4;
    __shared__ int s_wave[2][U][4];
    __shared__ unsigned long long s_first;
    const int p = blockIdx.x;
    const SeedGrid g = grids[p];
    const SlicProblem P = probs[p];
    const int tid = threadIdx.x, lane = tid & 63, wv = tid >> 6;
    if (tid == 0) s_first = ~0ull;
    const int Kg = g.ny * g.nx;
    int base = 0;
    for (int k0 = 0, it = 0; k0 < Kg; k0 += U * 256, ++it) {
        int y[U], x[U];
        bool keep[U];
        unsigned long long bal[U];
#pragma unroll
        for (int u = 0; u < U; ++u) {
            const int k = k0 + u * 256 + tid;
            y[u] = x[u] = 0;
            keep[u] = false;
            if (k < Kg) {
                y[u] = g.start_y + (k / g.nx) * g.step_y;
                x[u] = g.start_x + (k % g.nx) * g.step_x;
                keep[u] = mask[P.pix_off + (long long)y[u] * P.W + x[u]] != 0;
            }
        }
#pragma unroll
        for (int u = 0; u < U; ++u) {
            bal[u] = __ballot(keep[u]);
            if (lane == 0) s_wave[it & 1][u][wv] = __popcll(bal[u]);
        }
        __syncthreads();
        int run = base;
#pragma unroll
        for (int u = 0; u < U; ++u) {
            int before = 0, total = 0;
#pragma unroll
            for (int w = 0; w < 4; ++w) { const int c = s_wave[it & 1][u][w]; total += c; if (w < wv) before += c; }
            if (keep[u]) {
                const int rank = run + before + __popcll(bal[u] & ((1ull << lane) - 1ull));
                seed[2 * (size_t)(g.cent_off + rank)] = (float)y[u];
                seed[2 * (size_t)(g.cent_off + rank) + 1] = (float)x[u];
                cent_prob[g.cent_off + rank] = p;
            }
            run += total;
        }
        base = run;
    }
    __syncthreads();
    int K = base;
    if (K == 0 && g.slots > 0) {
        const long long npix = (long long)P.H * P.W;
        unsigned long long best = ~0ull;
        for (long long i = tid; i < npix; i += 256)
            if (mask[P.pix_off + i]) { best = (unsigned long long)i; break; }
        atomicMin(&s_first, best);
        __syncthreads();
        if (tid == 0 && s_first != ~0ull) {
            seed[2 * (size_t)g.cent_off] = (float)(s_first / P.W);
            seed[2 * (size_t)g.cent_off + 1] = (float)(s_first % P.W);
            cent_prob[g.cent_off] = p;
        }
        K = (s_first != ~0ull) ? 1 : 0;
    }
    if (tid == 0) K_out[p] = K;
}

__global__ __launch_bounds__(256) void count_valid_kernel(const SlicProblem *__restrict__ probs,
                                                          const uint8_t *__restrict__ mask, int *__restrict__ out) {
    const int p = blockIdx.y;
    const SlicProblem P = probs[p];
    const long long npix = (long long)P.H * P.W;
    const uint8_t *m = mask + P.pix_off;
    int c = 0;
    const long long head = ((16 - (reinterpret_cast<uintptr_t>(m) & 15)) & 15);
    const long long h0 = head < npix ? head : npix;
    const long long nvec = (npix - h0) / 16;
    const uint4 *mv = reinterpret_cast<const uint4 *>(m + h0);
    auto popnz = [](const uint4 &t) {
        int n = 0;
        const unsigned wds[4] = {t.x, t.y, t.z, t.w};
#pragma unroll
        for (int q = 0; q < 4; ++q) {
            unsigned nz = wds[q] | (wds[q] >> 4);
            nz |= nz >> 2; nz |= nz >> 1;
            n += __popc(nz & 0x01010101u);
        }
        return n;
    };
    const long long stride = (long long)gridDim.x * blockDim.x;
    long long i = (long long)blockIdx.x * blockDim.x + threadIdx.x;
    for (; i + 3 * stride < nvec; i += 4 * stride) {
        const uint4 t0 = mv[i], t1 = mv[i + stride], t2 = mv[i + 2 * stride], t3 = mv[i + 3 * stride];
        c += popnz(t0) + popnz(t1) + popnz(t2) + popnz(t3);
    }
    for (; i < nvec; i += stride) c += popnz(mv[i]);
    if (blockIdx.x == 0) {
        for (long long j = threadIdx.x; j < h0; j += blockDim.x) c += m[j] != 0;
        for (long long j = h0 + nvec * 16 + threadIdx.x; j < npix; j += blockDim.x) c += m[j] != 0;
    }
    __shared__ int s_c[4];
#pragma unroll
    for (int off = 32; off > 0; off >>= 1) c += __shfl_xor(c, off);
    if ((threadIdx.x & 63) == 0) s_c[threadIdx.x >> 6] = c;
    __syncthreads();
    if (threadIdx.x == 0) {
        const int tot = s_c[0] + s_c[1] + s_c[2] + s_c[3];
        if (tot) atomicAdd(&out[p], tot);
    }
}

int slic_plan_layout(obia_ctx *ctx, SlicBatch &b) {
    if (b.d_tile_prob) return OBIA_OK;
    const int np = b.nprob;
    long long tiles_all = 0;
    int tile_max = 0;
    for (int p = 0; p < np; ++p) {
        SlicProblem &P = b.probs[p];
        P.tiles_x = cdiv(P.W, SWEEP_TW);
        P.tiles_y = cdiv(P.H, SWEEP_TH);
        const int nt = P.tiles_x * P.tiles_y;
        if (tiles_all + nt > 0x7fff0000LL) { set_error("too many sweep tiles in one batch"); return OBIA_E_INVALID; }
        P.tile_off = (int)tiles_all;
        tiles_all += nt;
        if (nt > tile_max) tile_max = nt;
    }
    b.total_tiles_all = tiles_all > 0 ? tiles_all : 1;
    b.total_tiles = tile_max;
    std::vector<int> tp((size_t)b.total_tiles_all, 0);
    for (int p = 0; p < np; ++p)
        for (int t = 0; t < b.probs[p].tiles_x * b.probs[p].tiles_y; ++t) tp[(size_t)b.probs[p].tile_off + t] = p;
    b.d_probs = ctx->plan.add(ctx, b.probs.data(), (size_t)np);
    b.d_tile_prob = ctx->plan.add(ctx, tp.data(), tp.size());
    if (!b.d_probs || !b.d_tile_prob) return OBIA_E_NOMEM;
    return OBIA_OK;
}

int slic_count_valid(obia_ctx *ctx, SlicBatch &b, std::vector<int> &nvalid, int *d_cnt_cleared) {
    const int np = b.nprob;
    Arena &A = ctx->arena;
    nvalid.assign(np, 0);
    OBIA_TRY(slic_plan_layout(ctx, b));
    if (b.masked) {
        OBIA_TRY(ctx->plan.flush(ctx));
        int *d_cnt = d_cnt_cleared;
        if (!d_cnt) {
            d_cnt = A.get<int>(np);
            if (!d_cnt) return OBIA_E_NOMEM;
            OBIA_TRY(fill_async(ctx, d_cnt, 0, sizeof(int) * np));
        }
        int blocks = cdiv(b.maxpix, 256 * 16 * 32);
        if (blocks < 1) blocks = 1;
        hipLaunchKernelGGL(count_valid_kernel, dim3(blocks, np), dim3(256), 0, ctx->stream, b.d_probs, b.d_mask, d_cnt);
        OBIA_TRY(read_back(ctx, nvalid.data(), d_cnt, sizeof(int) * np));
    } else {
        for (int p = 0; p < np; ++p) nvalid[p] = b.probs[p].H * b.probs[p].W;
    }
    return OBIA_OK;
}

int slic_plan_and_seed(obia_ctx *ctx, SlicBatch &b, const std::vector<int> &n_segments, const std::vector<int> *nvalid_in,
                       const ExternalSeeds *ext) {
    const int np = b.nprob;
    if (ext)
        for (int p = 0; p < np; ++p)
            if (ext[p].n < 0 || (ext[p].n > 0 && !ext[p].yx && !ext[p].d_yx)) { set_error("external seeds of problem %d: bad set", p); return OBIA_E_INVALID; }
    Arena &A = ctx->arena;
    OBIA_TRY(slic_plan_layout(ctx, b));
    std::vector<int> nvalid;
    if (nvalid_in) nvalid = *nvalid_in;
    else OBIA_TRY(slic_count_valid(ctx, b, nvalid));
    if (ext && np == 1 && ext->n > 0 && nvalid[0] <= 0) { set_error("the mask has no valid pixel"); return OBIA_E_EMPTY; }
    std::vector<SeedGrid> grids(np);
    std::vector<double> stepmax(np);
    b.step.assign(np, 1.0f);
    b.grid_n.assign(np, 0);
    int cent_off = 0;
    for (int p = 0; p < np; ++p) {
        SlicProblem &P = b.probs[p];
        P.n_valid = nvalid[p];
        SeedGrid &g = grids[p];
        g.cent_off = cent_off; g.slots = 0;
        if (ext && ext[p].n > 0 && nvalid[p] > 0) {
            if ((long long)cent_off + ext[p].n > 0x7fff0000LL) { set_error("too many centroids in one batch"); return OBIA_E_INVALID; }
            g.start_y = g.start_x = 0; g.step_y = g.step_x = 1; g.ny = 1; g.nx = ext[p].n;
            stepmax[p] = ext[p].step < 1.0 ? 1.0 : ext[p].step;
            P.cent_off = cent_off;
            cent_off += ext[p].n;
            continue;
        }
        if (ext || nvalid[p] <= 0 || n_segments[p] <= 0) {
            g.start_y = g.start_x = 0; g.step_y = g.step_x = 1; g.ny = g.nx = 0;
            stepmax[p] = 1.0;
            P.cent_off = cent_off;
            continue;
        }
        long long n_eff = n_segments[p];
        if (b.masked) {
            double ne = std::nearbyint((double)n_segments[p] * ((double)P.H * (double)P.W) / (double)nvalid[p]);
            n_eff = ne < 1.0 ? 1 : (long long)ne;
        }
        b.grid_n[p] = n_eff;
        long long gr[4];
        regular_grid_hw(P.H, P.W, n_eff, gr);
        g.start_y = (int)gr[0]; g.step_y = gr[1] ? (int)gr[1] : 1; g.ny = (int)slice_len(P.H, gr[0], gr[1]);
        g.start_x = (int)gr[2]; g.step_x = gr[3] ? (int)gr[3] : 1; g.nx = (int)slice_len(P.W, gr[2], gr[3]);
        double sy = gr[1] ? (double)gr[1] : 1.0, sx = gr[3] ? (double)gr[3] : 1.0;
        stepmax[p] = sy > sx ? sy : sx;
        if (stepmax[p] < 1.0) stepmax[p] = 1.0;
        P.cent_off = cent_off;
        long long Kg = (long long)g.ny * g.nx;
        if (Kg < 1) Kg = 1;
        if (cent_off + Kg > 0x7fff0000LL) { set_error("too many centroids in one batch"); return OBIA_E_INVALID; }
        g.slots = (int)Kg;
        cent_off += (int)Kg;
    }
    b.total_cent = cent_off > 0 ? cent_off : 1;
    b.d_seed = A.get<float>((size_t)b.total_cent * 2);
    b.d_cent_prob = A.get<int>(b.total_cent);
    SeedGrid *d_grids = ctx->plan.add(ctx, grids.data(), (size_t)np);
    if (!b.d_seed || !b.d_cent_prob || !d_grids) return OBIA_E_NOMEM;
    OBIA_TRY(fill_async(ctx, b.d_cent_prob, 0xff, sizeof(int) * b.total_cent));
    std::vector<int> K(np);
    if (ext) {
        std::vector<int> hp((size_t)b.total_cent, 0);
        std::vector<float> hs;
        for (int p = 0; p < np; ++p) {
            K[p] = grids[p].ny * grids[p].nx;
            if (K[p] <= 0) continue;
            float *dst = b.d_seed + 2 * (size_t)grids[p].cent_off;
            for (int k = 0; k < K[p]; ++k) hp[(size_t)grids[p].cent_off + k] = p;
            if (ext[p].d_yx) {
                OBIA_HIP_TRY(hipMemcpyAsync(dst, ext[p].d_yx, sizeof(float) * 2 * (size_t)K[p], hipMemcpyDeviceToDevice, ctx->stream));
            } else {
                hs.resize((size_t)K[p] * 2);
                for (size_t i = 0; i < hs.size(); ++i) hs[i] = (float)ext[p].yx[i];
                OBIA_TRY(upload_async(ctx, dst, hs.data(), sizeof(float) * hs.size()));
            }
        }
        OBIA_TRY(upload_async(ctx, b.d_cent_prob, hp.data(), sizeof(int) * hp.size()));
    } else if (b.masked) {
        int *d_K = A.get<int>(np);
        if (!d_K) return OBIA_E_NOMEM;
        OBIA_TRY(ctx->plan.flush(ctx));
        hipLaunchKernelGGL(seed_masked_kernel, dim3(np), dim3(256), 0, ctx->stream, d_grids, b.d_probs, b.d_mask,
                           b.d_seed, b.d_cent_prob, d_K);
        OBIA_TRY(read_back(ctx, K.data(), d_K, sizeof(int) * np));
        for (int p = 0; p < np; ++p) if (nvalid[p] <= 0 || n_segments[p] <= 0) K[p] = 0;
    } else {
        int maxK = 1;
        for (int p = 0; p < np; ++p) { K[p] = grids[p].ny * grids[p].nx; if (K[p] > maxK) maxK = K[p]; }
        OBIA_TRY(ctx->plan.flush(ctx));
        hipLaunchKernelGGL(seed_grid_kernel, dim3(cdiv(maxK, 256), np), dim3(256), 0, ctx->stream, d_grids, np,
                           b.d_seed, b.d_cent_prob);
    }
    int cell_off = 0;
    for (int p = 0; p < np; ++p) {
        SlicProblem &P = b.probs[p];
        P.K = K[p];
        long long gr[4] = {0, 0, 0, 0};
        if (P.K > 0) regular_grid_hw(P.H, P.W, P.K, gr);
        P.sy = gr[1] ? (int)gr[1] : 1;
        P.sx = gr[3] ? (int)gr[3] : 1;
        P.ncy = cdiv(P.H, P.sy);
        P.ncx = cdiv(P.W, P.sx);
        const float stepf = (float)stepmax[p];
        b.step[p] = stepf;
        P.spatial_w = (float)(1.0 / ((double)stepf * (double)stepf)) * (b.prescale * b.prescale);
        P.sp_y = (float)b.spacing[1]; P.sp_x = (float)b.spacing[2];
        P.direct = b.direct ? 1 : 0;
        P.cell_off = cell_off;
        long long nc = (long long)P.ncy * P.ncx;
        if (cell_off + nc > 0x7fff0000LL) { set_error("too many bins in one batch"); return OBIA_E_INVALID; }
        cell_off += (int)nc;
    }
    b.total_cells = cell_off > 0 ? cell_off : 1;
    b.d_probs = ctx->plan.add(ctx, b.probs.data(), (size_t)np);
    if (!b.d_probs) return OBIA_E_NOMEM;
    const int RS = CENT_REC + b.CP;
    b.d_cent = A.get<float>((size_t)b.total_cent * RS);
    b.d_head = A.get<int>((size_t)b.total_cells * 2);
    const size_t acc_q = (size_t)b.total_cent * acc_record_qwords(b.CP);
    b.d_acc = A.get<unsigned long long>(acc_q);
    if (!b.d_cent || !b.d_head || !b.d_acc) return OBIA_E_NOMEM;
    return OBIA_OK;
}

__global__ __launch_bounds__(256) void stage_features_kernel(const float *__restrict__ feat, SlicProblem P, int C, int CP, float inv_prescale,
                                                             float *__restrict__ out) {
    const long long n = (long long)P.H * P.W * C;
    for (long long i = (long long)blockIdx.x * blockDim.x + threadIdx.x; i < n; i += (long long)gridDim.x * blockDim.x) {
        const int c = (int)(i % C);
        const long long pix = i / C;
        const int y = (int)(pix / P.W), x = (int)(pix % P.W);
        const long long f4 = P.feat_off + (((long long)(y >> 2) * P.XB + (x >> 4)) * CP + c) * 16 + (x & 15);
        out[i] = feat[4 * f4 + (y & 3)] * inv_prescale;
    }
}

__global__ void stage_centroids_kernel(const float *__restrict__ cent, int cent_off, int K, int C, int CP, float inv_prescale,
                                       float *__restrict__ out) {
    const long long i = (long long)blockIdx.x * blockDim.x + threadIdx.x;
    if (i >= (long long)K * (2 + C)) return;
    const int k = (int)(i / (2 + C)), f = (int)(i % (2 + C));
    const float *rec = cent + (size_t)(cent_off + k) * (CENT_REC + CP);
    out[i] = f < 2 ? rec[f] : rec[CENT_REC + f - 2] * inv_prescale;
}

int slic_stage_outputs(obia_ctx *ctx, const SlicBatch &b, float *features, float *seeds_yx, float *centroids) {
    if (b.nprob != 1 || !b.feat_planes) { set_error("stage outputs: one raster in the plane layout"); return OBIA_E_INVALID; }
    const SlicProblem &P = b.probs[0];
    const float inv_prescale = 1.0f / b.prescale;
    if (features) {
        const long long n = (long long)P.H * P.W * b.C;
        hipLaunchKernelGGL(stage_features_kernel, to_dim3(grids::slic_stage_features(n)), dim3(256), 0, ctx->stream, b.d_feat, P, b.C, b.CP, inv_prescale, features);
    }
    if (seeds_yx && P.K > 0)
        OBIA_HIP_TRY(hipMemcpyAsync(seeds_yx, b.d_seed + 2 * (size_t)P.cent_off, sizeof(float) * 2 * (size_t)P.K, hipMemcpyDeviceToDevice, ctx->stream));
    if (centroids && P.K > 0)
        hipLaunchKernelGGL(stage_centroids_kernel, dim3(cdiv((long long)P.K * (2 + b.C), 256)), dim3(256), 0, ctx->stream, b.d_cent, P.cent_off,
                           P.K, b.C, b.CP, inv_prescale, centroids);
    OBIA_HIP_TRY(hipGetLastError());
    return OBIA_OK;
}

}
```

obia_amd/csrc/slic.hpp:

```cpp
#pragma once
#include "common.hpp"

namespace obia {

struct SlicProblem {
    int H, W;
    int K;
    int sy, sx;
    int ncy, ncx;
    float spatial_w;
    int cent_off;
    int cell_off;
    int tile_off;
    int tiles_x, tiles_y;
    long long pix_off;
    long long feat_off;
    int XB;
    int n_valid;
    long long fb_off;
    float sp_y, sp_x;
    int direct;
    int m4_off;
};

struct SrcWindow {
    int y0, x0, h, w;
    long long pix_off;
    long long feat_off;
    long long fb_off;
};


inline int feat_xb(int w) { return (w + 15) >> 4; }
inline long long feat_block_f4(int h, int w, int CP) { return (long long)((h + 3) / 4) * feat_xb(w) * CP * 16; }

inline long long feat_boxes(int h, int w) { return (long long)(((h + 3) / 4 + 3) / 4) * feat_xb(w); }

void regular_grid_hw(long long H, long long W, long long n, long long out[4]);

#ifndef OBIA_SWEEP_TW
#define OBIA_SWEEP_TW 64
#endif
#ifndef OBIA_SWEEP_MAXC
#define OBIA_SWEEP_MAXC 96
#endif
constexpr int SWEEP_TW = OBIA_SWEEP_TW, SWEEP_TH = 64;
constexpr int SWEEP_MAXC = OBIA_SWEEP_MAXC;
constexpr int CENT_REC = 8;
inline int acc_record_qwords(int CP) { return CP <= 12 ? 16 : 32; }

struct SlicBatch {
    int nprob = 0;
    int C = 0, CP = 0;
    bool masked = false;
    int start_label = 1;
    int max_iter = 10;
    bool direct = false;
    int normalize = 0, to_lab = 0;
    float feat_ratio = 1.0f;
    long long total_pix = 0, total_boxes = 0, maxpix = 1;
    int maxh = 1;
    int total_cent = 0, total_cells = 0, total_tiles = 0;
    long long total_tiles_all = 0;
    std::vector<SlicProblem> probs;
    std::vector<SrcWindow> windows;
    SlicProblem *d_probs = nullptr;
    SrcWindow *d_windows = nullptr;
    float *d_fbox = nullptr;
    bool col_lb = false;
    float *d_feat = nullptr;
    bool fuse_features = false;
    const float *raw_src = nullptr;
    int raw_ws = 0;
    const unsigned *d_keys = nullptr;
    bool feat_planes = true;
    double sigma[3] = {0.0, 0.0, 0.0};
    double spacing[3] = {1.0, 1.0, 1.0};
    long long total_feat_f4 = 0;
    uint8_t *d_mask = nullptr;
    unsigned *d_mask4 = nullptr;
    long long total_m4 = 0;
    int32_t *d_labels = nullptr;
    float *d_seed = nullptr;
    int *d_cent_prob = nullptr;
    int *d_tile_prob = nullptr;
    float *d_cent = nullptr;
    int *d_head = nullptr;
    int *d_head_cur = nullptr;
    unsigned long long *d_acc = nullptr;
    int *d_tl_k = nullptr;
    unsigned *d_tl_fp = nullptr;
    int *d_tl_meta = nullptr;
    int *d_tl_req = nullptr;
    float *d_ref = nullptr;
    double fscale = 1.0;
    float prescale = 1.0f;
    bool exit_on_fixed_point = false;
    bool slic_zero = false;
    bool prepass_only = false;
    int prepass_iter = 0;
    std::vector<float> step;
    std::vector<long long> grid_n;
};

inline int slic_prepass_classes(const std::vector<SlicProblem> &probs, const std::vector<long long> &grid_n, std::vector<int> &rep) {
    const int np = (int)probs.size();
    rep.resize(np);
    std::vector<int> reps;
    int members = 0;
    for (int p = 0; p < np; ++p) {
        const SlicProblem &P = probs[p];
        rep[p] = p;
        if ((int)grid_n.size() != np || grid_n[p] <= 0 || P.K <= 0 || P.direct) continue;
        if ((long long)P.n_valid != (long long)P.H * (long long)P.W) continue;
        bool found = false;
        for (int r : reps) {
            const SlicProblem &R = probs[r];
            if (R.H == P.H && R.W == P.W && R.K == P.K && grid_n[r] == grid_n[p] && R.sy == P.sy && R.sx == P.sx && R.ncy == P.ncy &&
                R.ncx == P.ncx && R.tiles_x == P.tiles_x && R.tiles_y == P.tiles_y && R.spatial_w == P.spatial_w && R.sp_y == P.sp_y &&
                R.sp_x == P.sp_x) {
                rep[p] = r; ++members; found = true;
                break;
            }
        }
        if (!found) reps.push_back(p);
    }
    return members;
}

struct SmoothSpec {
    double sigma[3] = {0.0, 0.0, 0.0};
    float *tmp_a = nullptr, *tmp_b = nullptr;
    double *d_w[3] = {nullptr, nullptr, nullptr};
    int radius[3] = {0, 0, 0};
    unsigned *d_scratch = nullptr;
    bool on() const { return sigma[0] > 1e-15 || sigma[1] > 1e-15 || sigma[2] > 1e-15; }
};
int smooth_prepare(obia_ctx *ctx, SmoothSpec &sm, long long total_pix, int CP, int np);
int gaussian_weights_host(double sigma, bool sigma_is_f32, std::vector<double> &w);
int slic_features_launch(hipStream_t stream, const SlicBatch &b, const float *src, int Ws, unsigned *d_keys, const SmoothSpec *smooth = nullptr,
                         bool minmax_only = false);
bool slic_fuse_features(const SlicBatch &b, const float *src, int Ws);
double slic_fscale(float maxabs);
int slic_features_finish(SlicBatch &b, const unsigned *keys, const unsigned *nonfinite, const unsigned *maxabs_bits, std::vector<int> *skip);
int slic_prepare_features(obia_ctx *ctx, SlicBatch &b, const float *src, int Ws, std::vector<int> *skip = nullptr);
float slic_prescale(float ratio, int normalize, int to_lab, bool slic_zero);
bool slic_use_colour_bound(float ratio, bool to_lab = false);
void slic_batch_settings(SlicBatch &b, const obia_slic_params &p, int C, int normalize_bands, bool masked);
int slic_batch_layout(SlicBatch &b);
inline std::pair<int, int> slic_cc_sizes(double min_size_factor, double max_size_factor, int n_valid, int K) {
    const double segment_size = K > 0 ? (double)n_valid / (double)K : 1.0;
    const double mxd = max_size_factor * segment_size;
    return {(int)(min_size_factor * segment_size), mxd >= 2147483647.0 ? 2147483647 : (mxd >= 1.0 ? (int)mxd : 1)};
}

struct ExternalSeeds { const double *yx; int n; double step; const float *d_yx = nullptr; };
int slic_plan_and_seed(obia_ctx *ctx, SlicBatch &b, const std::vector<int> &n_segments,
                       const std::vector<int> *nvalid = nullptr, const ExternalSeeds *ext = nullptr);
int slic_count_valid(obia_ctx *ctx, SlicBatch &b, std::vector<int> &nvalid, int *d_cnt_cleared = nullptr);
int slic_plan_layout(obia_ctx *ctx, SlicBatch &b);

int slic_run_sweeps(obia_ctx *ctx, SlicBatch &b);
int slic_sweeps_settle(obia_ctx *ctx, bool *repeat);
int slic_rerun_storing(obia_ctx *ctx, SlicBatch &b);

int slic_stage_outputs(obia_ctx *ctx, const SlicBatch &b, float *features, float *seeds_yx, float *centroids);

int mask_centroids_dev(obia_ctx *ctx, const uint8_t *mask, int H, int W, const int64_t *picks, int K, const int64_t *dense, long long n_dense,
                       int iters, double *centroids_yx_out, double *steps_zyx_out);
int mask_centroids_queue(obia_ctx *ctx, const uint8_t *mask, int h, int w, long long n_valid, const int64_t *picks, int K, const int64_t *dense,
                         long long n_dense, int iters, float *seeds_out_dev, double *steps_out_dev);

struct CcProblem { int H, W; long long pix_off; int min_size; int max_size; };
struct CcResolve { const int *parent; const int *newlab; const int *small_final; int start_label; int mask_label; };
#if defined(__HIPCC__)
__device__ __forceinline__ int cc_resolve_label(const CcResolve &R, long long i) {
    const int p = R.parent[i];
    if (p < 0) return R.mask_label;
    const int r = R.parent[p];
    int nl = R.newlab[r];
    if (nl < 0) nl = R.small_final[-nl - 2];
    return (nl >= 0) ? nl + R.start_label : 0;
}
#endif
int enforce_connectivity_batch(obia_ctx *ctx, const std::vector<CcProblem> &probs, const int32_t *labels_in,
                               long long total_pix, int start_label, int32_t *labels_out, int *h_n_labels_out,
                               CcResolve *deferred = nullptr, const CcProblem *d_probs = nullptr);

int enforce_connectivity_dev(obia_ctx *ctx, const int32_t *labels_in, int H, int W, int min_size,
                             int max_size, int start_label, int32_t *labels_out, int *d_n_labels_out);

int zonal_stats_dev(obia_ctx *ctx, const float *raw, const int32_t *labels, int H, int W, int C,
                    const int32_t *bands_host, int n_bands, int n_labels, int start_label,
                    int64_t *count, double *mean, double *var, float *mn, float *mx);
int zonal_moments_dev(obia_ctx *ctx, const float *raw, const int32_t *labels, int H, int W, int C,
                      const int32_t *bands_host, int n_bands, int n_labels, int start_label, const double *mean,
                      double *skew, double *kurt, double *var );

}
```

obia_amd/csrc/tiling.hip:

```cpp
#include "slic.hpp"
#include "../../include/obia_testing.h"

#include <cmath>
#include <cstdlib>

namespace obia {

struct TileWin { int y0, x0, h, w; long long pix_off; int cly, clx; int cly_in, clx_in, cly_any, clx_any; int m4_off; };

__device__ __forceinline__ void wave_hist_add(unsigned *hist, int key, bool active) {
    bool todo = active;
    while (true) {
        const unsigned long long act = __ballot(todo);
        if (!act) break;
        const int leader = __ffsll((long long)act) - 1;
        const int kk = __shfl(key, leader);
        const unsigned long long same = __ballot(todo && key == kk);
        if ((int)(threadIdx.x & 63) == leader) atomicAdd(&hist[kk], (unsigned)__popcll(same));
        if (key == kk) todo = false;
    }
}

__device__ __forceinline__ bool in_corner(const TileWin &t, int y, int x) {
    return (y >= t.h - t.cly) && (x < t.clx || x >= t.w - t.clx);
}
__device__ __forceinline__ bool wholly_in_corner(const TileWin &t, int y, int x) {
    return (y >= t.h - t.cly_in) && (x < t.clx_in || x >= t.w - t.clx_in);
}
__device__ __forceinline__ bool meets_corner(const TileWin &t, int y, int x) {
    return (y >= t.h - t.cly_any) && (x < t.clx_any || x >= t.w - t.clx_any);
}

__global__ __launch_bounds__(256) void tile_count_inside_kernel(const TileWin *__restrict__ wins, const int32_t *__restrict__ G,
                                                                int Wr, unsigned *__restrict__ inside, int *__restrict__ tile_any) {
    const TileWin t = wins[blockIdx.y];
    bool seen = false;
    const int wround = ((t.w + 255) / 256) * 256;
    for (int y = blockIdx.x; y < t.h; y += gridDim.x) {
        const bool low = y >= t.h - t.cly_any;
        for (int x0 = 0; x0 < wround; x0 += 4 * 256) {
            int g[4];
#pragma unroll
            for (int u = 0; u < 4; ++u) {
                const int x = x0 + 256 * u + threadIdx.x;
                g[u] = 0;
                if (x < t.w && !(low && wholly_in_corner(t, y, x))) {
                    g[u] = G[(long long)(t.y0 + y) * Wr + t.x0 + x];
                    seen |= g[u] > 0;
                    if (low && meets_corner(t, y, x)) g[u] = 0;
                }
            }
#pragma unroll
            for (int u = 0; u < 4; ++u)
                if (x0 + 256 * u < wround) wave_hist_add(inside, g[u], g[u] > 0);
        }
    }
    if (__ballot(seen) && (threadIdx.x & 63) == 0) tile_any[blockIdx.y] = 1;
}

template <bool VEC4>
__global__ __launch_bounds__(256) void tile_mask_kernel(const TileWin *__restrict__ wins, const uint8_t *__restrict__ inmask,
                                                        int32_t *__restrict__ G, int Wr, int white,
                                                        const unsigned *__restrict__ inside, const unsigned *__restrict__ seg_size,
                                                        uint8_t *__restrict__ alive, uint8_t *__restrict__ dmask,
                                                        const int *__restrict__ tile_any, unsigned *__restrict__ dmask4) {
    const TileWin t = wins[blockIdx.y];
    if (white && tile_any[blockIdx.y] == 0) white = 0;
    auto decide = [&](int y, int x, long long gp, uint8_t m, int g) -> uint8_t {
        if (!white) return m;
        if (in_corner(t, y, x)) return 0;
        if (g > 0) {
            if (inside[g] == seg_size[g]) { G[gp] = 0; alive[g] = 0; }
            else m = 0;
        }
        return m;
    };
    if (VEC4) {
        const int w4 = t.w >> 2, nq = (t.h + 3) >> 2;
        for (int q = blockIdx.x; q < nq; q += gridDim.x)
            for (int x4 = threadIdx.x; x4 < w4; x4 += 256) {
                const int x = 4 * x4;
                unsigned mw[4];
                int4 g[4];
#pragma unroll
                for (int j = 0; j < 4; ++j) {
                    const int y = 4 * q + j;
                    const long long gp = (long long)(t.y0 + (y < t.h ? y : t.h - 1)) * Wr + t.x0 + x;
                    mw[j] = inmask ? *reinterpret_cast<const unsigned *>(inmask + gp) : 0x01010101u;
                    g[j] = make_int4(0, 0, 0, 0);
                    if (white) g[j] = *reinterpret_cast<const int4 *>(G + gp);
                }
                unsigned out[4] = {0u, 0u, 0u, 0u};
#pragma unroll
                for (int j = 0; j < 4; ++j) {
                    const int y = 4 * q + j;
                    if (y >= t.h) continue;
                    const long long gp = (long long)(t.y0 + y) * Wr + t.x0 + x;
                    const int gv[4] = {g[j].x, g[j].y, g[j].z, g[j].w};
#pragma unroll
                    for (int u = 0; u < 4; ++u) {
                        const uint8_t m = ((mw[j] >> (8 * u)) & 0xffu) != 0;
                        out[j] |= (unsigned)decide(y, x + u, gp + u, m, gv[u]) << (8 * u);
                    }
                    *reinterpret_cast<unsigned *>(dmask + t.pix_off + (long long)y * t.w + x) = out[j];
                }
                uint4 o;
                unsigned *ov = &o.x;
#pragma unroll
                for (int c = 0; c < 4; ++c)
                    ov[c] = ((out[0] >> (8 * c)) & 0xffu) | (((out[1] >> (8 * c)) & 0xffu) << 8) | (((out[2] >> (8 * c)) & 0xffu) << 16) |
                            (((out[3] >> (8 * c)) & 0xffu) << 24);
                *reinterpret_cast<uint4 *>(dmask4 + (long long)t.m4_off + (long long)q * t.w + x) = o;
            }
        return;
    }
    for (int y = blockIdx.x; y < t.h; y += gridDim.x)
    for (int x0 = threadIdx.x; x0 < t.w; x0 += 4 * 256) {
        uint8_t mv[4];
        int gv[4];
#pragma unroll
        for (int u = 0; u < 4; ++u) {
            const int x = x0 + 256 * u;
            mv[u] = 0; gv[u] = 0;
            if (x < t.w) {
                const long long gp = (long long)(t.y0 + y) * Wr + t.x0 + x;
                mv[u] = inmask ? (inmask[gp] != 0) : 1;
                if (white && !in_corner(t, y, x)) gv[u] = G[gp];
            }
        }
#pragma unroll
        for (int u = 0; u < 4; ++u) {
            const int x = x0 + 256 * u;
            if (x >= t.w) continue;
            const long long gp = (long long)(t.y0 + y) * Wr + t.x0 + x;
            dmask[t.pix_off + (long long)y * t.w + x] = decide(y, x, gp, mv[u], gv[u]);
        }
    }
}

constexpr int TS_SLOTS = 128;
__global__ __launch_bounds__(64) void tile_scatter_kernel(const TileWin *__restrict__ wins, const CcResolve R,
                                                          int32_t *__restrict__ G, int Wr, int id_base,
                                                          unsigned *__restrict__ seg_size) {
    __shared__ int s_key[TS_SLOTS];
    __shared__ unsigned s_cnt[TS_SLOTS];
    const TileWin t = wins[blockIdx.y];
    const int bw = (t.w + 63) / 64;
    const int by = blockIdx.x / bw, bx = blockIdx.x % bw;
    if (by * 64 >= t.h) return;
    const int lane = threadIdx.x;
    for (int i = lane; i < TS_SLOTS; i += 64) { s_key[i] = 0; s_cnt[i] = 0; }
    __syncthreads();
    const int x = bx * 64 + lane;
    const bool col_ok = x < t.w;
    const int y_lo = by * 64, y_hi = min(y_lo + 64, t.h);
    int rid = 0;
    unsigned rn = 0;
    auto close_run = [&]() {
        if (rid <= 0) return;
        const unsigned h = ((unsigned)rid * 2654435761u) >> 25;
        int slot = -1;
#pragma unroll 1
        for (int probe = 0; probe < TS_SLOTS; ++probe) {
            const int sidx = (h + probe) & (TS_SLOTS - 1);
            const int old = atomicCAS(&s_key[sidx], 0, rid);
            if (old == 0 || old == rid) { slot = sidx; break; }
        }
        if (slot >= 0) atomicAdd(&s_cnt[slot], rn);
        else atomicAdd(&seg_size[rid], rn);
    };
#pragma unroll 1
    for (int y0 = y_lo; y0 < y_hi; y0 += 8) {
        int l[8];
#pragma unroll
        for (int j = 0; j < 8; ++j) {
            const int y = y0 + j;
            l[j] = (col_ok && y < y_hi) ? cc_resolve_label(R, t.pix_off + (long long)y * t.w + x) : 0;
        }
#pragma unroll
        for (int j = 0; j < 8; ++j) {
            const int y = y0 + j;
            const int id = l[j] > 0 ? id_base + l[j] : 0;
            if (id > 0) G[(long long)(t.y0 + y) * Wr + t.x0 + x] = id;
            if (id != rid) { close_run(); rid = id; rn = 0; }
            rn += 1;
        }
    }
    close_run();
    __syncthreads();
    for (int i = lane; i < TS_SLOTS; i += 64)
        if (s_key[i] > 0 && s_cnt[i]) atomicAdd(&seg_size[s_key[i]], s_cnt[i]);
}

constexpr int IDS_CHUNK = 1024 * 16;

__global__ __launch_bounds__(1024) void ids_count_kernel(const uint8_t *__restrict__ alive, int n_ids, int *__restrict__ partial) {
    __shared__ int s_wave[16];
    const int tid = threadIdx.x, lane = tid & 63, wv = tid >> 6;
    const int i0 = blockIdx.x * IDS_CHUNK + tid * 16;
    int c = 0;
#pragma unroll
    for (int q = 0; q < 16; ++q) c += (i0 + q < n_ids) ? (alive[i0 + q] != 0) : 0;
#pragma unroll
    for (int off = 32; off > 0; off >>= 1) c += __shfl_xor(c, off);
    if (lane == 0) s_wave[wv] = c;
    __syncthreads();
    if (tid == 0) {
        int t = 0;
        for (int w2 = 0; w2 < 16; ++w2) t += s_wave[w2];
        partial[blockIdx.x] = t;
    }
}

__global__ __launch_bounds__(1024) void ids_scan_kernel(const uint8_t *__restrict__ alive, int n_ids, const int *__restrict__ partial,
                                                        int *__restrict__ newid, long long *__restrict__ total) {
    __shared__ int s_wave[16];
    __shared__ int s_base[16];
    const int tid = threadIdx.x, lane = tid & 63, wv = tid >> 6;
    int pre = 0;
    for (int j = tid; j < (int)blockIdx.x; j += 1024) pre += partial[j];
#pragma unroll
    for (int off = 32; off > 0; off >>= 1) pre += __shfl_xor(pre, off);
    if (lane == 0) s_base[wv] = pre;
    const int i0 = blockIdx.x * IDS_CHUNK + tid * 16;
    unsigned char f[16];
#pragma unroll
    for (int q = 0; q < 16; ++q) f[q] = (i0 + q < n_ids) ? alive[i0 + q] : 0;
    int c = 0;
#pragma unroll
    for (int q = 0; q < 16; ++q) c += f[q] != 0;
    int inc = c;
#pragma unroll
    for (int off = 1; off < 64; off <<= 1) {
        const int v = __shfl_up(inc, off);
        if (lane >= off) inc += v;
    }
    if (lane == 63) s_wave[wv] = inc;
    __syncthreads();
    int before = 0;
    for (int w2 = 0; w2 < 16; ++w2) { before += s_base[w2]; if (w2 < wv) before += s_wave[w2]; }
    int run = before + inc - c;
#pragma unroll
    for (int q = 0; q < 16; ++q)
        if (i0 + q < n_ids) { if (f[q]) { run += 1; newid[i0 + q] = run; } else newid[i0 + q] = 0; }
    if (blockIdx.x == gridDim.x - 1 && tid == 1023) *total = before + inc;
}

__global__ __launch_bounds__(256) void ids_apply_kernel(int32_t *__restrict__ G, long long n, const int *__restrict__ newid) {
    const long long n4 = ((reinterpret_cast<uintptr_t>(G) & 15) == 0) ? n / 4 : 0;
    int4 *G4 = reinterpret_cast<int4 *>(G);
    for (long long i = (long long)blockIdx.x * blockDim.x + threadIdx.x; i < n4; i += (long long)gridDim.x * blockDim.x) {
        int4 g = G4[i];
        g.x = g.x > 0 ? newid[g.x] : 0;
        g.y = g.y > 0 ? newid[g.y] : 0;
        g.z = g.z > 0 ? newid[g.z] : 0;
        g.w = g.w > 0 ? newid[g.w] : 0;
        G4[i] = g;
    }
    for (long long i = n4 * 4 + (long long)blockIdx.x * blockDim.x + threadIdx.x; i < n; i += (long long)gridDim.x * blockDim.x) {
        const int g = G[i];
        G[i] = g > 0 ? newid[g] : 0;
    }
}

struct TileState {
    int H, W, C;
    int Hg, row0;
    const float *img;
    const uint8_t *inmask;
    int32_t *G;
    unsigned *seg_size, *inside;
    uint8_t *alive;
    int *newid;
    long long *d_total;
    int id_cap, next_id;
    int clx, cly, clx_in, cly_in, clx_any, cly_any;
    obia_tiling_params tp;
    obia_slic_params sp;
    SlicBatch settings;
    int seeding = OBIA_SEEDING_GRID;
    obia_pick_fn pick_fn = nullptr;
    void *pick_user = nullptr;
    struct PreFeat {
        bool ready = false;
        bool planned = false;
        bool fused = false;
        SlicBatch b;
        std::vector<unsigned> host;
        unsigned *d_keys = nullptr;
        bool launched = false;
        bool on_side = false;
        size_t cursor = 0;
    } pf;
};


static int grid_rows(const std::vector<TileWin> &wins) {
    int g = 1;
    for (auto &t : wins) if (t.h > g) g = t.h;
    return (int)grids::tiler_rows(g, 1).x.n;
}

#ifndef OBIA_PREFETCH_BESIDE
#define OBIA_PREFETCH_BESIDE 0
#endif
static int prefetch_white_launch(obia_ctx *ctx, TileState &S, bool beside = false);

static int seed_tiles_skimage(obia_ctx *ctx, TileState &S, const SlicBatch &b, const std::vector<int> &nvalid, std::vector<int> &nseg,
                              std::vector<ExternalSeeds> &ext) {
    const int np = b.nprob;
    if (!S.pick_fn) { set_error("seeding = skimage needs a pick function"); return OBIA_E_INVALID; }
    Arena &A = ctx->arena;
    ext.assign(np, ExternalSeeds{nullptr, 0, 1.0, nullptr});
    std::vector<long long> off(np, 0);
    long long total = 0;
    for (int p = 0; p < np; ++p) {
        if (nseg[p] < 2 || nvalid[p] < 2) { nseg[p] = 0; continue; }
        off[p] = total;
        total += std::min(nseg[p], nvalid[p]);
    }
    if (total == 0) return OBIA_OK;
    if (total > 0x7fff0000LL) { set_error("too many centroids in one batch"); return OBIA_E_INVALID; }
    float *d_seeds = A.get<float>(2 * (size_t)total);
    double *d_steps = A.get<double>(2 * (size_t)np);
    if (!d_seeds || !d_steps) return OBIA_E_NOMEM;
    OBIA_TRY(fill_async(ctx, d_steps, 0, sizeof(double) * 2 * (size_t)np));
    auto ascending_below = [](const int64_t *v, long long n, long long bound) {
        if (v[0] < 0 || v[n - 1] >= bound) return false;
        for (long long i = 1; i < n; ++i) if (v[i] <= v[i - 1]) return false;
        return true;
    };
    for (int p = 0; p < np; ++p) {
        if (nseg[p] == 0) continue;
        const int K = std::min(nseg[p], nvalid[p]);
        const int64_t *idx = nullptr, *dense = nullptr;
        int32_t n_idx = 0;
        int64_t n_dense = 0;
        if (S.pick_fn(S.pick_user, (int64_t)nvalid[p], (int32_t)nseg[p], &idx, &n_idx, &dense, &n_dense) != 0) {
            set_error("the pick function failed for a tile with %d valid pixels and n_segments = %d", nvalid[p], nseg[p]);
            return OBIA_E_INVALID;
        }
        if (!idx || n_idx != K || !ascending_below(idx, K, nvalid[p]) ||
            (dense && (n_dense < 1 || n_dense > nvalid[p] || !ascending_below(dense, n_dense, nvalid[p])))) {
            set_error("the pick function returned bad picks for a tile with %d valid pixels and n_segments = %d: %d strictly ascending ranks below the "
                      "valid count are needed", nvalid[p], nseg[p], K);
            return OBIA_E_INVALID;
        }
        const SlicProblem &P = b.probs[p];
        OBIA_TRY(mask_centroids_queue(ctx, b.d_mask + P.pix_off, P.H, P.W, nvalid[p], idx, K, dense, dense ? (long long)n_dense : 0, 5,
                                      d_seeds + 2 * off[p], d_steps + 2 * (size_t)p));
        ext[p].n = K;
        ext[p].d_yx = d_seeds + 2 * off[p];
    }
    std::vector<double> steps(2 * (size_t)np);
    OBIA_TRY(read_back(ctx, steps.data(), d_steps, sizeof(double) * steps.size()));
    for (int p = 0; p < np; ++p) {
        if (ext[p].n == 0) continue;
        const double st = std::max(steps[2 * (size_t)p], steps[2 * (size_t)p + 1]);
        if (!(st >= 0.0) || !(st < 1e9)) { set_error("tile seeding: steps are not finite"); return OBIA_E_INVALID; }
        ext[p].step = st;
    }
    return OBIA_OK;
}

static int run_tile_batch(obia_ctx *ctx, TileState &S, std::vector<TileWin> &wins, bool white) {
    const int np = (int)wins.size();
    if (np == 0) return OBIA_OK;
    Arena &A = ctx->arena;
    const Arena::Mark mk = A.mark();
    SlicBatch b = S.settings;
    for (auto &t : wins) b.windows.push_back(SrcWindow{t.y0, t.x0, t.h, t.w, 0, 0, 0});
    OBIA_TRY(slic_batch_layout(b));
    for (int p = 0; p < np; ++p) { wins[p].pix_off = b.probs[p].pix_off; wins[p].m4_off = b.probs[p].m4_off; }
    b.d_mask = A.get<uint8_t>((size_t)b.total_pix);
    unsigned *d_mask4 = A.get<unsigned>((size_t)b.total_m4);
    if (!d_mask4) return OBIA_E_NOMEM;
    const bool pre = white && S.pf.ready;
    if (pre) {
        const SlicBatch &pb = S.pf.b;
        if (S.pf.cursor + np > pb.windows.size()) { set_error("white batch beyond the prefetched windows"); return OBIA_E_INVALID; }
        const SrcWindow *a = &pb.windows[S.pf.cursor];
        for (int p = 0; p < np; ++p)
            if (a[p].y0 != wins[p].y0 || a[p].x0 != wins[p].x0 || a[p].h != wins[p].h || a[p].w != wins[p].w) { set_error("white batch does not match the prefetched windows"); return OBIA_E_INVALID; }
        if (S.pf.fused) {
            b.d_feat = A.get<float>(4 * (size_t)b.total_feat_f4);
            b.fuse_features = true;
            b.raw_src = S.img; b.raw_ws = S.W;
            b.d_keys = S.pf.d_keys + S.pf.cursor * (size_t)S.C * 2;
        } else {
            b.d_feat = pb.d_feat + 4 * (size_t)a[0].feat_off;
            if (b.col_lb) b.d_fbox = pb.d_fbox + (size_t)a[0].fb_off * 2 * b.CP;
        }
    } else {
        b.d_feat = A.get<float>(4 * (size_t)b.total_feat_f4);
        if (b.col_lb) {
            b.d_fbox = A.get<float>((size_t)b.total_boxes * 2 * b.CP);
            if (!b.d_fbox) return OBIA_E_NOMEM;
        }
    }
    b.d_labels = A.get<int32_t>((size_t)b.total_pix);
    if (!b.d_mask || !b.d_feat || !b.d_labels) return OBIA_E_NOMEM;
    TileWin *d_wins = ctx->plan.add(ctx, wins.data(), (size_t)np);
    b.d_windows = ctx->plan.add(ctx, b.windows.data(), (size_t)np);
    if (!d_wins || !b.d_windows) return OBIA_E_NOMEM;
    OBIA_TRY(slic_plan_layout(ctx, b));
    OBIA_TRY(ctx->plan.flush(ctx));
    int *d_tile_any = A.get<int>(np), *d_cnt = A.get<int>(np);
    if (!d_tile_any || !d_cnt) return OBIA_E_NOMEM;
    {
        ClearSet clr(ctx);
        if (white) {
            OBIA_TRY(clr.add(S.inside, 0, sizeof(unsigned) * (size_t)S.next_id));
            OBIA_TRY(clr.add(d_tile_any, 0, sizeof(int) * (size_t)np));
        }
        OBIA_TRY(clr.add(d_cnt, 0, sizeof(int) * (size_t)np));
        OBIA_TRY(clr.flush());
    }
    if (white) {
        hipLaunchKernelGGL(tile_count_inside_kernel, dim3(grid_rows(wins), np), dim3(256), 0, ctx->stream, d_wins, S.G, S.W, S.inside, d_tile_any);
    }
    {
        bool vec4 = (S.W % 4 == 0) && (reinterpret_cast<uintptr_t>(S.inmask) % 4 == 0) && (reinterpret_cast<uintptr_t>(S.G) % 16 == 0) &&
                    (reinterpret_cast<uintptr_t>(b.d_mask) % 4 == 0) && (reinterpret_cast<uintptr_t>(d_mask4) % 16 == 0);
        for (auto &t : wins) vec4 = vec4 && (t.x0 % 4 == 0) && (t.w % 4 == 0) && (t.pix_off % 4 == 0);
        if (vec4) {
            hipLaunchKernelGGL(HIP_KERNEL_NAME(tile_mask_kernel<true>), dim3((grid_rows(wins) + 3) / 4, np), dim3(256), 0, ctx->stream, d_wins, S.inmask,
                               S.G, S.W, white ? 1 : 0, S.inside, S.seg_size, S.alive, b.d_mask, d_tile_any, d_mask4);
            b.d_mask4 = d_mask4;
        } else {
            hipLaunchKernelGGL(HIP_KERNEL_NAME(tile_mask_kernel<false>), dim3(grid_rows(wins), np), dim3(256), 0, ctx->stream, d_wins, S.inmask,
                               S.G, S.W, white ? 1 : 0, S.inside, S.seg_size, S.alive, b.d_mask, d_tile_any, d_mask4);
        }
    }
    std::vector<int> skip;
    if (pre) {
        const size_t NP = S.pf.b.windows.size(), nkeys = NP * (size_t)S.C * 2;
        const unsigned *h = S.pf.host.data();
        OBIA_TRY(slic_features_finish(b, h + S.pf.cursor * (size_t)S.C * 2, h + nkeys + S.pf.cursor, h + nkeys + NP + S.pf.cursor, &skip));
        S.pf.cursor += np;
    } else {
        OBIA_TRY(slic_prepare_features(ctx, b, S.img, S.W, &skip));
    }
    std::vector<int> nvalid;
    debug_sync(ctx, "tiler: mask + features");
    OBIA_TRY(slic_count_valid(ctx, b, nvalid, d_cnt));
    debug_sync(ctx, "tiler: count_valid");
    std::vector<int> nseg(np);
    const double pixel_area = S.tp.pixel_width * S.tp.pixel_height;
    const double crown_area = M_PI * S.tp.crown_radius * S.tp.crown_radius;
    for (int p = 0; p < np; ++p) {
        double n;
        if (S.sp.n_segments > 0)
            n = std::nearbyint((double)S.sp.n_segments * (double)nvalid[p] / ((double)S.tp.tile_size * S.tp.tile_size));
        else
            n = std::nearbyint((double)nvalid[p] * pixel_area / crown_area);
        nseg[p] = (skip[p] || n < 1.0) ? 0 : (n > 2.0e9 ? 2000000000 : (int)n);
    }
    std::vector<ExternalSeeds> ext;
    if (S.seeding == OBIA_SEEDING_SKIMAGE) OBIA_TRY(seed_tiles_skimage(ctx, S, b, nvalid, nseg, ext));
    OBIA_TRY(slic_plan_and_seed(ctx, b, nseg, &nvalid, ext.empty() ? nullptr : ext.data()));
    debug_sync(ctx, "tiler: plan_and_seed");
    std::vector<CcProblem> cps(np);
    for (int p = 0; p < np; ++p) {
        const SlicProblem &P = b.probs[p];
        const auto [min_size, max_size] = slic_cc_sizes(S.sp.min_size_factor, S.sp.max_size_factor, P.n_valid, P.K);
        cps[p] = CcProblem{P.H, P.W, P.pix_off, min_size, max_size};
    }
    const CcProblem *d_cps = S.sp.enforce_connectivity ? ctx->plan.add(ctx, cps.data(), (size_t)np) : nullptr;
    if (S.sp.enforce_connectivity && !d_cps) return OBIA_E_NOMEM;
    if (!white && S.pf.planned && !S.pf.launched)
        OBIA_TRY(prefetch_white_launch(ctx, S, OBIA_PREFETCH_BESIDE != 0 || b.exit_on_fixed_point || b.slic_zero));
    const Arena::Mark sweeps_mk = A.mark();
    unsigned *const mask4 = b.d_mask4;
    OBIA_TRY(slic_run_sweeps(ctx, b));
    debug_sync(ctx, "tiler: sweeps");
    int n_new = 0;
    CcResolve resolve{};
    if (S.sp.enforce_connectivity) {
        OBIA_TRY(enforce_connectivity_batch(ctx, cps, b.d_labels, b.total_pix, 1, nullptr, &n_new, &resolve, d_cps));
        bool repeat = false;
        OBIA_TRY(slic_sweeps_settle(ctx, &repeat));
        if (repeat) {
            A.rewind(sweeps_mk);
            b.d_mask4 = mask4;
            OBIA_TRY(slic_rerun_storing(ctx, b));
            OBIA_TRY(enforce_connectivity_batch(ctx, cps, b.d_labels, b.total_pix, 1, nullptr, &n_new, &resolve, d_cps));
            OBIA_TRY(slic_sweeps_settle(ctx, nullptr));
        }
        debug_sync(ctx, "tiler: connectivity");
    } else {
        set_error("the tiled driver needs enforce_connectivity=True (segments must be connected pixel sets)");
        return OBIA_E_UNSUPPORTED;
    }
    if (S.next_id + n_new > S.id_cap) { set_error("segment id capacity exceeded (%d + %d > %d)", S.next_id, n_new, S.id_cap); return OBIA_E_NOMEM; }
    if (n_new > 0) {
        int sblocks = 1;
        for (auto &t : wins) sblocks = std::max(sblocks, cdiv(t.w, 64) * cdiv(t.h, 64));
        hipLaunchKernelGGL(tile_scatter_kernel, dim3(sblocks, np), dim3(64), 0, ctx->stream, d_wins, resolve, S.G, S.W,
                           S.next_id - 1, S.seg_size);
        OBIA_TRY(fill_async(ctx, S.alive + S.next_id, 1, (size_t)n_new));
        S.next_id += n_new;
    }
    OBIA_HIP_TRY(hipGetLastError());
    OBIA_TRY(ctx->plan.flush(ctx));
    A.rewind(mk);
    return OBIA_OK;
}

__global__ __launch_bounds__(256) void seam_mark_kernel(const int32_t *__restrict__ codes, int n, int me, int owner, int32_t *__restrict__ fmap,
                                                        int cap, int *__restrict__ new_list, int *__restrict__ ctr, int32_t *__restrict__ ids) {
    int tmax = 0;
    for (int i = blockIdx.x * blockDim.x + threadIdx.x; i < n; i += gridDim.x * blockDim.x) {
        const int c = codes[i];
        int id = 0;
        if (c > 0) {
            const int o = (c >> 24) - 1, t = c & 0xffffff;
            if (o == me) id = t;
            else if (o == owner) {
                tmax = max(tmax, t);
                if (t > 0 && t < cap) {
                    const int f = fmap[t];
                    if (f > 0) id = f;
                    else if (f == 0 && atomicCAS(&fmap[t], 0, -1) == 0) new_list[atomicAdd(&ctr[0], 1)] = t;
                }
            }
        }
        ids[i] = id;
    }
    for (int off = 32; off > 0; off >>= 1) tmax = max(tmax, __shfl_xor(tmax, off));
    if ((threadIdx.x & 63) == 0 && tmax > 0) atomicMax(&ctr[1], tmax);
}
constexpr int SEAM_SORT = 16384;
__global__ __launch_bounds__(1024) void seam_assign_sort_kernel(int *__restrict__ new_list, int m, int first, int owner,
                                                                int32_t *__restrict__ fmap, int32_t *__restrict__ code_of) {
    __shared__ int s[SEAM_SORT];
    int np2 = 1;
    while (np2 < m) np2 <<= 1;
    for (int i = threadIdx.x; i < np2; i += 1024) s[i] = i < m ? new_list[i] : 0x7fffffff;
    __syncthreads();
    for (int k = 2; k <= np2; k <<= 1)
        for (int j = k >> 1; j > 0; j >>= 1) {
            for (int i = threadIdx.x; i < np2; i += 1024) {
                const int ixj = i ^ j;
                if (ixj > i) {
                    const int a = s[i], b = s[ixj];
                    if (((i & k) == 0) ? (a > b) : (a < b)) { s[i] = b; s[ixj] = a; }
                }
            }
            __syncthreads();
        }
    for (int i = threadIdx.x; i < m; i += 1024) {
        const int t = s[i];
        fmap[t] = first + i;
        code_of[first + i] = t | ((owner + 1) << 24);
    }
}
__global__ __launch_bounds__(256) void seam_assign_count_kernel(const int *__restrict__ new_list, int m, int first, int owner,
                                                                int32_t *__restrict__ fmap, int32_t *__restrict__ code_of) {
    for (int i = blockIdx.x * blockDim.x + threadIdx.x; i < m; i += gridDim.x * blockDim.x) {
        const int t = new_list[i];
        int rank = 0;
        for (int j = 0; j < m; ++j) rank += new_list[j] < t;
        fmap[t] = first + rank;
        code_of[first + rank] = t | ((owner + 1) << 24);
    }
}
__global__ __launch_bounds__(256) void seam_translate_kernel(const int32_t *__restrict__ codes, int n, int owner,
                                                             const int32_t *__restrict__ fmap, int cap, int32_t *__restrict__ ids) {
    for (int i = blockIdx.x * blockDim.x + threadIdx.x; i < n; i += gridDim.x * blockDim.x) {
        if (ids[i] != 0) continue;
        const int c = codes[i];
        if (c <= 0 || (c >> 24) - 1 != owner) continue;
        const int t = c & 0xffffff;
        if (t > 0 && t < cap) ids[i] = fmap[t];
    }
}
__global__ __launch_bounds__(256) void seam_unclaim_kernel(const int *__restrict__ new_list, int m, int32_t *__restrict__ fmap) {
    for (int i = blockIdx.x * blockDim.x + threadIdx.x; i < m; i += gridDim.x * blockDim.x) fmap[new_list[i]] = 0;
}
__global__ void seam_register_kernel(unsigned *__restrict__ seg_size, uint8_t *__restrict__ alive, int first, int count) {
    const int i = blockIdx.x * blockDim.x + threadIdx.x;
    if (i < count) { seg_size[first + i] = 0xffffffffu; alive[first + i] = 1; }
}

static int tiler_check(const float *img, int H, int W, int C, int Hg, int row0, const obia_tiling_params *tp,
                       const obia_slic_params *sp, const int32_t *labels) {
    if (!img || !tp || !sp || !labels) { set_error("null argument"); return OBIA_E_INVALID; }
    if (H <= 0 || W <= 0 || C <= 0 || C > 16) { set_error("bad raster shape (%d,%d,%d)", H, W, C); return OBIA_E_INVALID; }
    if (row0 < 0 || row0 + H > Hg) { set_error("local rows [%d,%d) outside the global raster of %d rows", row0, row0 + H, Hg); return OBIA_E_INVALID; }
    if ((long long)H * W > 0x7fffffffLL) { set_error("raster above 2^31 pixels: shard it across GPUs"); return OBIA_E_INVALID; }
    if (tp->tile_size <= 0 || tp->buffer < 0) { set_error("tile_size must be positive and buffer non-negative"); return OBIA_E_INVALID; }
    if (!(sp->compactness > 0.0) || sp->max_num_iter < 0) { set_error("bad SLIC parameters"); return OBIA_E_INVALID; }
    for (int i = 0; i < 3; ++i) {
        if (!(sp->sigma_zyx[i] >= 0.0)) { set_error("sigma must be >= 0"); return OBIA_E_INVALID; }
        if (!(sp->spacing_zyx[i] > 0.0) || !(sp->spacing_zyx[i] < 1.0e30)) { set_error("spacing must be positive and finite"); return OBIA_E_INVALID; }
    }
    if (!sp->enforce_connectivity) { set_error("the tiled driver needs enforce_connectivity=True (segments must be connected pixel sets)"); return OBIA_E_UNSUPPORTED; }
    if (sp->n_segments <= 0 && !(tp->crown_radius > 0.0 && tp->pixel_width > 0.0 && tp->pixel_height > 0.0)) {
        set_error("crown_radius and pixel size must be positive when n_segments is not given");
        return OBIA_E_INVALID;
    }
    return OBIA_OK;
}

static int tiler_init(obia_ctx *ctx, TileState &S, const float *img, const uint8_t *mask, int H, int W, int C, int Hg,
                      int row0, const obia_tiling_params *tp, const obia_slic_params *sp, int32_t *labels, int extra_ids) {
    OBIA_TRY(tiler_check(img, H, W, C, Hg, row0, tp, sp, labels));
    const int T = tp->tile_size, B = tp->buffer;
    Arena &A = ctx->arena;
    const int ntx = cdiv(W, T), nty = cdiv(H, T) + 2;
    const double pixel_area = tp->pixel_width * tp->pixel_height;
    const double crown_area = M_PI * tp->crown_radius * tp->crown_radius;
    const long long wh = (long long)(T + 2 * B) * (T + 2 * B);
    double n = sp->n_segments > 0 ? (double)sp->n_segments * (double)wh / ((double)T * T) : (double)wh * pixel_area / crown_area;
    if (n < 1) n = 1;
    long long cap = (long long)(n * 1.5 + 64.0) * (long long)ntx * nty + 16 + extra_ids;
    if (cap > 0x7ffffff0LL) { set_error("too many segments for int32 ids"); return OBIA_E_INVALID; }
    S.H = H; S.W = W; S.C = C; S.Hg = Hg; S.row0 = row0; S.img = img; S.inmask = mask; S.G = labels; S.tp = *tp; S.sp = *sp;
    S.id_cap = (int)cap; S.next_id = 1;
    slic_batch_settings(S.settings, *sp, C, 1, true);
    S.settings.start_label = 1;
    S.seg_size = A.get<unsigned>((size_t)cap);
    S.inside = A.get<unsigned>((size_t)cap);
    S.alive = A.get<uint8_t>((size_t)cap);
    S.newid = A.get<int>((size_t)cap);
    S.d_total = A.get<long long>(1);
    if (!S.seg_size || !S.inside || !S.alive || !S.newid || !S.d_total) return OBIA_E_NOMEM;
    OBIA_TRY(fill_async(ctx, S.seg_size, 0, sizeof(unsigned) * (size_t)cap));
    OBIA_TRY(fill_async(ctx, S.alive, 0, (size_t)cap));
    S.clx = S.cly = S.clx_in = S.cly_in = S.clx_any = S.cly_any = 0;
    if (B > 0) {
        const double cl = (double)B / 2.0;
        auto count = [](double px, double cl, int kind) {
            if (!(px > 0.0)) px = 1.0;
            long long k = (long long)std::floor(cl / px) + 2;
            if (k < 0) k = 0;
            auto holds = [&](long long i) { return kind == 0 ? (i + 0.5) * px < cl : (kind == 1 ? (i + 1.0) * px <= cl : i * px < cl); };
            while (k > 0 && !holds(k - 1)) --k;
            return (int)std::min<long long>(k, 0x3fffffff);
        };
        S.clx = count(tp->pixel_width, cl, 0);  S.cly = count(tp->pixel_height, cl, 0);
        S.clx_in = count(tp->pixel_width, cl, 1);  S.cly_in = count(tp->pixel_height, cl, 1);
        S.clx_any = count(tp->pixel_width, cl, 2);  S.cly_any = count(tp->pixel_height, cl, 2);
    }
    return OBIA_OK;
}

static TileWin white_window(const TileState &S, int tj, int ti) {
    const int T = S.tp.tile_size, B = S.tp.buffer;
    const int y0 = std::max(0, tj * T - B), y1 = std::min(S.Hg, tj * T + T + B);
    const int x0 = std::max(0, ti * T - B), x1 = std::min(S.W, ti * T + T + B);
    const int h = y1 - y0, w = x1 - x0;
    return TileWin{y0 - S.row0, x0, h, w, 0, std::min(S.cly, h), std::min(S.clx, w), std::min(S.cly_in, h), std::min(S.clx_in, w),
                   std::min(S.cly_any, h), std::min(S.clx_any, w), 0};
}

static int prefetch_white_plan(obia_ctx *ctx, TileState &S, int white_order) {
    const int T = S.tp.tile_size;
    const int ntx = cdiv(S.W, T), nty = cdiv(S.Hg, T);
    TileState::PreFeat &pf = S.pf;
    pf = TileState::PreFeat();
    if (S.sp.sigma_zyx[0] > 0.0 || S.sp.sigma_zyx[1] > 0.0 || S.sp.sigma_zyx[2] > 0.0) return OBIA_OK;
    SlicBatch b = S.settings;
    for (int cls = 0; cls < (white_order == 1 ? 2 : 1); ++cls)
        for (int tj = 0; tj < nty; ++tj) {
            if (white_order == 1 && (tj & 1) != cls) continue;
            for (int ti = 0; ti < ntx; ++ti) {
                if ((ti + tj) % 2 == 0) continue;
                const TileWin t = white_window(S, tj, ti);
                if (t.h <= 0 || t.w <= 0) continue;
                if (t.y0 < 0 || t.y0 + t.h > S.H) return OBIA_OK;
                b.windows.push_back(SrcWindow{t.y0, t.x0, t.h, t.w, 0, 0, 0});
            }
        }
    const size_t NP = b.windows.size();
    if (NP == 0) return OBIA_OK;
    if (slic_batch_layout(b) != OBIA_OK) return OBIA_OK;
    pf.fused = slic_fuse_features(b, S.img, S.W);
    if (!pf.fused && (double)b.total_feat_f4 * 16.0 > 32.0 * 1024 * 1024 * 1024) return OBIA_OK;
    Arena &A = ctx->arena;
    const size_t ntot = NP * (size_t)S.C * 2 + 2 * NP;
    b.d_windows = A.get<SrcWindow>(NP);
    pf.d_keys = A.get<unsigned>(ntot);
    if (!pf.fused) b.d_feat = A.get<float>(4 * (size_t)b.total_feat_f4);
    if (!b.d_windows || !pf.d_keys || (!pf.fused && !b.d_feat)) return OBIA_E_NOMEM;
    if (b.col_lb) {
        b.d_fbox = A.get<float>((size_t)b.total_boxes * 2 * b.CP);
        if (!b.d_fbox) return OBIA_E_NOMEM;
    }
    pf.host.resize(ntot);
    pf.b = std::move(b);
    pf.planned = true;
    return OBIA_OK;
}

static int prefetch_white_launch(obia_ctx *ctx, TileState &S, bool beside) {
    TileState::PreFeat &pf = S.pf;
    if (pf.launched || !pf.planned) return OBIA_OK;
    pf.launched = true;
    if (pf.fused) beside = false;
    OBIA_TRY(upload_async(ctx, pf.b.d_windows, pf.b.windows.data(), sizeof(SrcWindow) * pf.b.windows.size()));
    if (beside) {
        OBIA_TRY(side_stream(ctx));
        hipStream_t side = ctx->side;
        OBIA_HIP_TRY(hipEventRecord(ctx->aux_fork, ctx->stream));
        OBIA_HIP_TRY(hipStreamWaitEvent(side, ctx->aux_fork, 0));
        OBIA_TRY(slic_features_launch(side, pf.b, S.img, S.W, pf.d_keys, nullptr, false));
        OBIA_HIP_TRY(hipEventRecord(ctx->aux_join, side));
        pf.on_side = true;
        return OBIA_OK;
    }
    ScopedSpan span(ctx, T_FEAT);
    OBIA_TRY(slic_features_launch(ctx->stream, pf.b, S.img, S.W, pf.d_keys, nullptr, pf.fused));
    return OBIA_OK;
}

static int prefetch_white_fetch(obia_ctx *ctx, TileState &S) {
    if (!S.pf.planned) return OBIA_OK;
    OBIA_TRY(prefetch_white_launch(ctx, S));
    if (S.pf.on_side) { OBIA_HIP_TRY(hipStreamWaitEvent(ctx->stream, ctx->aux_join, 0)); S.pf.on_side = false; }
    OBIA_TRY(read_back(ctx, S.pf.host.data(), S.pf.d_keys, S.pf.host.size() * sizeof(unsigned)));
    S.pf.ready = true;
    S.pf.cursor = 0;
    return OBIA_OK;
}

static int tiler_run(obia_ctx *ctx, TileState &S, bool white, int tr_lo, int tr_hi, int parity) {
    const int T = S.tp.tile_size, B = S.tp.buffer;
    const int ntx = cdiv(S.W, T), nty = cdiv(S.Hg, T);
    if (tr_lo < 0) tr_lo = 0;
    if (tr_hi > nty) tr_hi = nty;
    const bool per_row = !(parity >= 0 && T > 2 * B);
    const bool per_tile = white && T <= 2 * B;
    std::vector<TileWin> wins;
    auto flush = [&]() -> int {
        for (auto &t : wins)
            if (t.y0 < 0 || t.y0 + t.h > S.H) { set_error("tile window rows [%d,%d) (local) outside the %d local rows: halo too small", t.y0, t.y0 + t.h, S.H); return OBIA_E_INVALID; }
        int rc = run_tile_batch(ctx, S, wins, white);
        wins.clear();
        return rc;
    };
    for (int tj = tr_lo; tj < tr_hi; ++tj) {
        if (parity >= 0 && (tj & 1) != parity) continue;
        for (int ti = 0; ti < ntx; ++ti) {
            const bool is_white = (ti + tj) % 2 != 0;
            if (is_white != white) continue;
            if (!white) {
                TileWin t{tj * T - S.row0, ti * T, std::min(T, S.Hg - tj * T), std::min(T, S.W - ti * T), 0, 0, 0, 0, 0, 0, 0, 0};
                if (t.h > 0 && t.w > 0) wins.push_back(t);
            } else {
                const TileWin t = white_window(S, tj, ti);
                if (t.h > 0 && t.w > 0) wins.push_back(t);
                if (per_tile && !wins.empty()) OBIA_TRY(flush());
            }
        }
        if (white && per_row) OBIA_TRY(flush());
    }
    if (!wins.empty()) OBIA_TRY(flush());
    return OBIA_OK;
}

static int tiler_finalize(obia_ctx *ctx, TileState &S, int64_t *n_segments_out) {
    const int nchunks = cdiv(S.next_id, IDS_CHUNK);
    int *d_partial = ctx->arena.get<int>((size_t)nchunks);
    if (!d_partial) return OBIA_E_NOMEM;
    hipLaunchKernelGGL(ids_count_kernel, dim3(nchunks), dim3(1024), 0, ctx->stream, S.alive, S.next_id, d_partial);
    hipLaunchKernelGGL(ids_scan_kernel, dim3(nchunks), dim3(1024), 0, ctx->stream, S.alive, S.next_id, d_partial, S.newid, S.d_total);
    const int g = (int)grids::tiler_ids_apply((long long)S.H * S.W).x.n;
    hipLaunchKernelGGL(ids_apply_kernel, dim3(g), dim3(256), 0, ctx->stream, S.G, (long long)S.H * S.W, S.newid);
    OBIA_HIP_TRY(hipGetLastError());
    long long total = 0;
    OBIA_TRY(read_back(ctx, &total, S.d_total, sizeof(long long)));
    if (n_segments_out) *n_segments_out = total;
    return OBIA_OK;
}

static int check_seeding(int seeding, obia_pick_fn picks) {
    if (seeding != OBIA_SEEDING_GRID && seeding != OBIA_SEEDING_SKIMAGE) { set_error("seeding must be OBIA_SEEDING_GRID or OBIA_SEEDING_SKIMAGE (got %d)", seeding); return OBIA_E_INVALID; }
    if (seeding == OBIA_SEEDING_SKIMAGE && !picks) { set_error("seeding = skimage needs a pick function"); return OBIA_E_INVALID; }
    return OBIA_OK;
}

static int tiled_slic_dev(obia_ctx *ctx, const float *img, const uint8_t *mask, int H, int W, int C,
                          const obia_tiling_params *tp, const obia_slic_params *sp, int seeding, obia_pick_fn picks, void *picks_user,
                          int32_t *labels_out, int64_t *n_segments_out) {
    TileState S;
    OBIA_TRY(check_seeding(seeding, picks));
    OBIA_TRY(tiler_init(ctx, S, img, mask, H, W, C, H, 0, tp, sp, labels_out, 0));
    S.seeding = seeding; S.pick_fn = picks; S.pick_user = picks_user;
    OBIA_TRY(fill_async(ctx, labels_out, 0, sizeof(int32_t) * (size_t)H * W));
    const int nty = cdiv(H, tp->tile_size);
    OBIA_TRY(prefetch_white_plan(ctx, S, tp->white_order));
    OBIA_TRY(tiler_run(ctx, S, false, 0, nty, -1));
    if (std::getenv("OBIA_DEBUG_FAIL_AFTER_BLACK")) {
        set_error("debug: forced failure after the black pass");
        return OBIA_E_INVALID;
    }
    OBIA_TRY(prefetch_white_fetch(ctx, S));
    if (tp->white_order == 1) {
        OBIA_TRY(tiler_run(ctx, S, true, 0, nty, 0));
        OBIA_TRY(tiler_run(ctx, S, true, 0, nty, 1));
    } else {
        OBIA_TRY(tiler_run(ctx, S, true, 0, nty, -1));
    }
    return tiler_finalize(ctx, S, n_segments_out);
}

}

struct obia_tiler {
    obia_ctx *ctx;
    obia::TileState S;
    int *seam_buf = nullptr;
    size_t seam_cap = 0;
};

using namespace obia;

static int enter(obia_tiler *t) {
    if (!t) { set_error("null tiler"); return OBIA_E_INVALID; }
    return enter(t->ctx);
}

extern "C" {

obia_tiler *obia_tiler_create(obia_ctx *ctx, const float *img_local, const uint8_t *mask_local, int H_local, int W, int C,
                              int H_global, int row0, const obia_tiling_params *tiling, const obia_slic_params *params,
                              int32_t *labels_local, int extra_ids) {
    if (enter(ctx) != OBIA_OK) return nullptr;
    frame_begin(ctx, FRAME_TIMING);
    obia_tiler *t = new obia_tiler();
    t->ctx = ctx;
    if (tiler_init(ctx, t->S, img_local, mask_local, H_local, W, C, H_global, row0, tiling, params, labels_local,
                   extra_ids < 0 ? 0 : extra_ids) != OBIA_OK) { delete t; return nullptr; }
    return t;
}

void obia_tiler_destroy(obia_tiler *t) {
    if (!t) return;
    (void)enter(t->ctx);
    (void)quiesce(t->ctx, 0);
    if (t->seam_buf) (void)hipFree(t->seam_buf);
    resolve_timing(t->ctx);
    delete t;
}

int obia_tiler_run(obia_tiler *t, int white, int tile_row_lo, int tile_row_hi, int row_parity) {
    OBIA_TRY(enter(t));
    const int rc = tiler_run(t->ctx, t->S, white != 0, tile_row_lo, tile_row_hi, row_parity);
    if (rc != OBIA_OK) return quiesce(t->ctx, rc);
    OBIA_HIP_TRY(hipStreamSynchronize(t->ctx->stream));
    return OBIA_OK;
}

int obia_tiler_next_id(obia_tiler *t) { return t ? t->S.next_id : -1; }

int obia_tiler_set_seeding(obia_tiler *t, int seeding, obia_pick_fn picks, void *picks_user) {
    OBIA_TRY(enter(t));
    OBIA_TRY(check_seeding(seeding, picks));
    t->S.seeding = seeding; t->S.pick_fn = picks; t->S.pick_user = picks_user;
    return OBIA_OK;
}

int obia_tiler_set_segments(obia_tiler *t, int first_id, int count, const uint32_t *sizes_dev) {
    OBIA_TRY(enter(t));
    if (!sizes_dev || first_id < 1 || count < 0) { set_error("bad arguments"); return OBIA_E_INVALID; }
    if (first_id + count > t->S.id_cap) { set_error("segment id capacity exceeded (%d + %d > %d)", first_id, count, t->S.id_cap); return OBIA_E_NOMEM; }
    if (count == 0) return OBIA_OK;
    OBIA_HIP_TRY(hipMemcpyAsync(t->S.seg_size + first_id, sizes_dev, sizeof(uint32_t) * (size_t)count, hipMemcpyDeviceToDevice, t->ctx->stream));
    OBIA_TRY(fill_async(t->ctx, t->S.alive + first_id, 1, (size_t)count));
    if (first_id + count > t->S.next_id) t->S.next_id = first_id + count;
    OBIA_HIP_TRY(hipStreamSynchronize(t->ctx->stream));
    return OBIA_OK;
}

int obia_tiler_get_alive(obia_tiler *t, uint8_t *alive_out_dev, int count) {
    OBIA_TRY(enter(t));
    if (!alive_out_dev || count < 0 || count > t->S.id_cap) { set_error("bad arguments"); return OBIA_E_INVALID; }
    OBIA_HIP_TRY(hipMemcpyAsync(alive_out_dev, t->S.alive, (size_t)count, hipMemcpyDeviceToDevice, t->ctx->stream));
    OBIA_HIP_TRY(hipStreamSynchronize(t->ctx->stream));
    return OBIA_OK;
}

int obia_tiler_set_alive(obia_tiler *t, const uint8_t *alive_in_dev, int count) {
    OBIA_TRY(enter(t));
    if (!alive_in_dev || count < 0 || count > t->S.id_cap) { set_error("bad arguments"); return OBIA_E_INVALID; }
    OBIA_HIP_TRY(hipMemcpyAsync(t->S.alive, alive_in_dev, (size_t)count, hipMemcpyDeviceToDevice, t->ctx->stream));
    OBIA_HIP_TRY(hipStreamSynchronize(t->ctx->stream));
    return OBIA_OK;
}

int obia_tiler_import_seam(obia_tiler *t, const int32_t *codes_dev, int n, int my_rank, int owner_rank,
                           int32_t *fmap_dev, int fmap_cap, int32_t *code_of_dev, int32_t *ids_out_dev,
                           int *first_new_out, int *n_new_out, int *max_owner_id_out) {
    OBIA_TRY(enter(t));
    if (!codes_dev || !fmap_dev || !code_of_dev || !ids_out_dev || n < 0 || fmap_cap < 1 || my_rank < 0 || owner_rank < 0 ||
        my_rank > 126 || owner_rank > 126 || !first_new_out || !n_new_out || !max_owner_id_out) { set_error("bad arguments"); return OBIA_E_INVALID; }
    obia_ctx *ctx = t->ctx;
    *first_new_out = t->S.next_id; *n_new_out = 0; *max_owner_id_out = 0;
    if (n == 0) return OBIA_OK;
    if (t->seam_cap < (size_t)n + 2) {
        if (t->seam_buf) (void)hipFree(t->seam_buf);
        t->seam_buf = nullptr; t->seam_cap = 0;
        if (hipMalloc(&t->seam_buf, sizeof(int) * ((size_t)n + 2)) != hipSuccess) { set_error("seam scratch allocation failed"); return OBIA_E_NOMEM; }
        t->seam_cap = (size_t)n + 2;
    }
    int *ctr = t->seam_buf, *new_list = t->seam_buf + 2;
    OBIA_TRY(fill_async(ctx, ctr, 0, sizeof(int) * 2));
    const int blocks = (int)grids::tiler_seam(n).x.n;
    hipLaunchKernelGGL(seam_mark_kernel, dim3(blocks), dim3(256), 0, ctx->stream, codes_dev, n, my_rank, owner_rank, fmap_dev, fmap_cap, new_list, ctr,
                       ids_out_dev);
    int h[2] = {0, 0};
    OBIA_TRY(read_back(ctx, h, ctr, sizeof(h)));
    *max_owner_id_out = h[1];
    const int n_new = h[0];
    if (t->S.next_id + n_new > t->S.id_cap) {
        hipLaunchKernelGGL(seam_unclaim_kernel, dim3((unsigned)grids::tiler_seam(n_new).x.n), dim3(256), 0, ctx->stream, new_list, n_new, fmap_dev);
        OBIA_HIP_TRY(hipStreamSynchronize(ctx->stream));
        set_error("segment id capacity exceeded (%d + %d > %d)", t->S.next_id, n_new, t->S.id_cap);
        return OBIA_E_NOMEM;
    }
    if (n_new > 0) {
        if (n_new <= SEAM_SORT)
            hipLaunchKernelGGL(seam_assign_sort_kernel, dim3(1), dim3(1024), 0, ctx->stream, new_list, n_new, t->S.next_id, owner_rank, fmap_dev, code_of_dev);
        else
            hipLaunchKernelGGL(seam_assign_count_kernel, dim3(256), dim3(256), 0, ctx->stream, new_list, n_new, t->S.next_id, owner_rank, fmap_dev, code_of_dev);
        hipLaunchKernelGGL(seam_translate_kernel, dim3(blocks), dim3(256), 0, ctx->stream, codes_dev, n, owner_rank, fmap_dev, fmap_cap, ids_out_dev);
        hipLaunchKernelGGL(seam_register_kernel, dim3(cdiv(n_new, 256)), dim3(256), 0, ctx->stream, t->S.seg_size, t->S.alive, t->S.next_id, n_new);
        t->S.next_id += n_new;
        OBIA_HIP_TRY(hipStreamSynchronize(ctx->stream));
    }
    *n_new_out = n_new;
    OBIA_HIP_TRY(hipGetLastError());
    return OBIA_OK;
}

int obia_test_seam_sort_limit(void) { return SEAM_SORT; }

int obia_tiler_finalize(obia_tiler *t, int64_t *n_segments_out) {
    OBIA_TRY(enter(t));
    const int rc = tiler_finalize(t->ctx, t->S, n_segments_out);
    return rc == OBIA_OK ? rc : quiesce(t->ctx, rc);
}

int obia_tiled_slic_seeded_f32_dev(obia_ctx *ctx, const float *img, const uint8_t *mask, int H, int W, int C,
                                   const obia_tiling_params *tiling, const obia_slic_params *params, int seeding,
                                   obia_pick_fn picks, void *picks_user, int32_t *labels_out, int64_t *n_segments_out) {
    OBIA_TRY(enter(ctx));
    return call_frame(ctx, FRAME_TOTAL, [&] {
        return tiled_slic_dev(ctx, img, mask, H, W, C, tiling, params, seeding, picks, picks_user, labels_out, n_segments_out);
    });
}

int obia_tiled_slic_f32_dev(obia_ctx *ctx, const float *img, const uint8_t *mask, int H, int W, int C,
                            const obia_tiling_params *tiling, const obia_slic_params *params, int32_t *labels_out,
                            int64_t *n_segments_out) {
    return obia_tiled_slic_seeded_f32_dev(ctx, img, mask, H, W, C, tiling, params, OBIA_SEEDING_GRID, nullptr, nullptr, labels_out, n_segments_out);
}

int obia_tiled_slic_seeded_f32(obia_ctx *ctx, const float *img, const uint8_t *mask, int H, int W, int C,
                               const obia_tiling_params *tiling, const obia_slic_params *params, int seeding,
                               obia_pick_fn picks, void *picks_user, int32_t *labels_out, int64_t *n_segments_out) {
    OBIA_TRY(enter(ctx));
    if (!img || !labels_out || H <= 0 || W <= 0 || C <= 0) { set_error("bad arguments"); return OBIA_E_INVALID; }
    OBIA_TRY(check_seeding(seeding, picks));
    const size_t npix = (size_t)H * W;
    Staging s(ctx);
    const float *d_img = s.in(img, npix * C);
    const uint8_t *d_mask = s.in(mask, npix);
    int32_t *d_lab = s.out<int32_t>(npix);
    s.run([&] {
        return obia_tiled_slic_seeded_f32_dev(ctx, d_img, d_mask, H, W, C, tiling, params, seeding, picks, picks_user, d_lab, n_segments_out);
    });
    s.fetch(labels_out, d_lab, npix);
    return s.finish();
}

int obia_tiled_slic_f32(obia_ctx *ctx, const float *img, const uint8_t *mask, int H, int W, int C,
                        const obia_tiling_params *tiling, const obia_slic_params *params, int32_t *labels_out,
                        int64_t *n_segments_out) {
    return obia_tiled_slic_seeded_f32(ctx, img, mask, H, W, C, tiling, params, OBIA_SEEDING_GRID, nullptr, nullptr, labels_out, n_segments_out);
}

}
```

Baseline: 7584.

## Slice white-tile min/max prefetch into readback-wait gaps and merge count readbacks

Adds an optional sliced prefetch in which the white-pass band min/max reduction is split into row slices. The slices are queued one at a time by a filler callback while the host waits on readback events, and the results come back through an async copy into a pinned landing buffer. The non-prefetch feature path also queues the features and count-valid kernels together and reads both back in a single transfer, saving one sync per batch. Slicing is off by default (env var OBIA_PREFETCH_SLICES, default 0), so the default gain comes from the merged readback; the slicing adds extra launches and bookkeeping complexity.

New measurement: 7516. About the same (-0.9%).

```diff
diff --git a/include/obia_testing.h b/include/obia_testing.h
--- a/include/obia_testing.h
+++ b/include/obia_testing.h
@@ -2,6 +2,7 @@
 #define OBIA_TESTING_H
 
 #include "obia_hip.h"
+#include "obia_testing_prefetch.h"
 
 #ifdef __cplusplus
 extern "C" {
diff --git a/include/obia_testing_prefetch.h b/include/obia_testing_prefetch.h
--- /dev/null
+++ b/include/obia_testing_prefetch.h
@@ -0,0 +1,19 @@
+#ifndef OBIA_TESTING_PREFETCH_H
+#define OBIA_TESTING_PREFETCH_H
+
+#include "obia_hip.h"
+
+#ifdef __cplusplus
+extern "C" {
+#endif
+
+int obia_test_prefetch_slices(const int32_t *heights, int n_windows, const int32_t *batch_windows, int n_batches, int rows,
+                              int32_t *slices_out, int cap, int32_t *n_slices_out, int32_t *last_out);
+
+int obia_test_minmax_slices_dev(obia_ctx *ctx, const float *raster_dev, int H, int W, int C, const int32_t *windows, int n, int rows,
+                                uint32_t *whole_out, uint32_t *sliced_out);
+
+#ifdef __cplusplus
+}
+#endif
+#endif
diff --git a/obia_amd/_lib.py b/obia_amd/_lib.py
--- a/obia_amd/_lib.py
+++ b/obia_amd/_lib.py
@@ -200,6 +200,10 @@
     "obia_test_launch_grid_names": (_I, [_P, ctypes.c_int64]),
     "obia_test_seam_sort_limit": (_I, []),
 }
+_PREFETCH_TEST_SIGNATURES = {
+    "obia_test_prefetch_slices": (_I, [_P, _I, _P, _I, _I, _P, _I, _P, _P]),
+    "obia_test_minmax_slices_dev": (_I, [_P, _P, _I, _I, _I, _P, _I, _I, _P, _P]),
+}
 
 _lib = None
 
@@ -221,7 +225,8 @@
         lib = ctypes.CDLL(LIB_PATH)
         for name, (res, args) in (list(_SIGNATURES.items()) + list(_IMAGE_SIGNATURES.items()) + list(_SHARPNESS_SIGNATURES.items())
                                    + list(_TRAINING_SIGNATURES.items()) + list(_CROWNS_SIGNATURES.items()) + list(_SEED_TABLE_SIGNATURES.items())
-                                   + list(_BOXES_SIGNATURES.items()) + list(_POINTS_SIGNATURES.items()) + list(_TEST_SIGNATURES.items())):
+                                   + list(_BOXES_SIGNATURES.items()) + list(_POINTS_SIGNATURES.items()) + list(_TEST_SIGNATURES.items())
+                                   + list(_PREFETCH_TEST_SIGNATURES.items())):
             try:
                 fn = getattr(lib, name)
             except AttributeError:
diff --git a/obia_amd/csrc/common.hpp b/obia_amd/csrc/common.hpp
--- a/obia_amd/csrc/common.hpp
+++ b/obia_amd/csrc/common.hpp
@@ -87,6 +87,12 @@
     obia::Arena arena;
     void *pinned = nullptr;
     size_t pinned_bytes = 0;
+    hipEvent_t rb_event = nullptr;
+    int (*filler)(obia_ctx *, void *) = nullptr;
+    void *filler_user = nullptr;
+    unsigned long long rb_serial = 0;
+    void *pf_landing = nullptr;
+    size_t pf_landing_bytes = 0;
     unsigned long long *defer_buf = nullptr;
     bool defer_pending = false;
     double defer_shared_px = 0;
diff --git a/obia_amd/csrc/context.cpp b/obia_amd/csrc/context.cpp
--- a/obia_amd/csrc/context.cpp
+++ b/obia_amd/csrc/context.cpp
@@ -200,7 +200,16 @@
     OBIA_TRY(ctx->plan.flush(ctx));
     OBIA_HIP_TRY(hipMemcpyAsync(ctx->pinned, dev_src, bytes, hipMemcpyDeviceToHost, ctx->stream));
     ctx->timing.readbacks += 1;
-    OBIA_HIP_TRY(hipStreamSynchronize(ctx->stream));
+    if (ctx->filler) {
+        if (!ctx->rb_event) OBIA_HIP_TRY(hipEventCreateWithFlags(&ctx->rb_event, hipEventDisableTiming));
+        OBIA_HIP_TRY(hipEventRecord(ctx->rb_event, ctx->stream));
+        const int filled = ctx->filler(ctx, ctx->filler_user);
+        OBIA_HIP_TRY(hipEventSynchronize(ctx->rb_event));
+        OBIA_TRY(filled);
+    } else {
+        OBIA_HIP_TRY(hipStreamSynchronize(ctx->stream));
+    }
+    ctx->rb_serial += 1;
     ctx->up_used = 0;
     memcpy(host_dst, ctx->pinned, bytes);
     return OBIA_OK;
@@ -460,6 +469,7 @@
     if (ctx->up_buf) (void)hipHostFree(ctx->up_buf);
     if (ctx->pinned) (void)hipHostFree(ctx->pinned);
     if (ctx->defer_buf) (void)hipHostFree(ctx->defer_buf);
+    if (ctx->pf_landing) (void)hipHostFree(ctx->pf_landing);
     if (ctx->cc_visited) (void)hipFree(ctx->cc_visited);
     for (auto e : ctx->event_pool) (void)hipEventDestroy(e);
     if (ctx->side) (void)hipStreamDestroy(ctx->side);
@@ -467,6 +477,7 @@
     if (ctx->aux_join) (void)hipEventDestroy(ctx->aux_join);
     if (ctx->grp_fork) (void)hipEventDestroy(ctx->grp_fork);
     if (ctx->grp_join) (void)hipEventDestroy(ctx->grp_join);
+    if (ctx->rb_event) (void)hipEventDestroy(ctx->rb_event);
     if (ctx->own_stream) (void)hipStreamDestroy(ctx->stream);
     delete ctx;
 }
diff --git a/obia_amd/csrc/launch_grids.hpp b/obia_amd/csrc/launch_grids.hpp
--- a/obia_amd/csrc/launch_grids.hpp
+++ b/obia_amd/csrc/launch_grids.hpp
@@ -80,6 +80,10 @@
 inline Grid rast_large(long long n_bands, long long max_w) { return Grid{whole(n_bands), strided(cdivl(max_w, RAST_LARGE_TILE_W), 1024)}; }
 
 inline Grid slic_band_minmax(long long maxh, long long np) { return Grid{strided(maxh, 2048), whole(np)}; }
+inline Grid slic_band_minmax_rows(long long rows) {
+    const long long trips = std::max(1LL, cdivl(rows, 2048));
+    return one_axis(strided(rows, cdivl(std::max(1LL, rows), trips)));
+}
 inline Grid slic_feature_rows(long long rows, long long np) { return Grid{strided(rows, 4096), whole(np)}; }
 inline Grid slic_gauss(long long n, long long np) { return Grid{strided(cdivl(n, 256), 65535), whole(np)}; }
 inline Grid slic_stage_features(long long n) { return one_axis(strided(cdivl(n, 256), 65535)); }
@@ -140,6 +144,7 @@
     OBIA_GRID2(rast_band_bin, "n_large max_nv"),
     OBIA_GRID2(rast_large, "n_bands max_w"),
     OBIA_GRID2(slic_band_minmax, "maxh np"),
+    OBIA_GRID1(slic_band_minmax_rows, "rows"),
     OBIA_GRID2(slic_feature_rows, "rows np"),
     OBIA_GRID2(slic_gauss, "n np"),
     OBIA_GRID1(slic_stage_features, "n"),
diff --git a/obia_amd/csrc/prefetch_slices.hpp b/obia_amd/csrc/prefetch_slices.hpp
--- /dev/null
+++ b/obia_amd/csrc/prefetch_slices.hpp
@@ -0,0 +1,47 @@
+#pragma once
+#include <cstddef>
+#include <vector>
+
+namespace obia {
+
+struct PrefetchSlice { int win, r0, r1; };
+
+struct PrefetchSchedule {
+    std::vector<PrefetchSlice> slices;
+    std::vector<int> last_of_win;
+    std::vector<int> first_win;
+    std::vector<int> count;
+    std::vector<int> last;
+};
+
+inline PrefetchSchedule plan_prefetch_slices(const std::vector<int> &heights, const std::vector<int> &batch_windows, int rows) {
+    PrefetchSchedule s;
+    if (rows < 1) rows = 1;
+    s.last_of_win.assign(heights.size(), -1);
+    for (size_t w = 0; w < heights.size(); ++w) {
+        for (int r = 0; r < heights[w];) {
+            const int n = rows < heights[w] - r ? rows : heights[w] - r;
+            s.slices.push_back(PrefetchSlice{(int)w, r, r + n});
+            r += n;
+        }
+        s.last_of_win[w] = (int)s.slices.size() - 1;
+    }
+    size_t w = 0;
+    for (int n : batch_windows) {
+        const size_t w0 = w;
+        s.first_win.push_back((int)w0);
+        if (n > 0) w += (size_t)n;
+        if (w > heights.size()) w = heights.size();
+        s.count.push_back((int)(w - w0));
+        s.last.push_back(w == 0 ? -1 : s.last_of_win[w - 1]);
+    }
+    return s;
+}
+
+inline int prefetch_batch_from(const PrefetchSchedule &s, size_t first) {
+    for (size_t k = 0; k < s.first_win.size(); ++k)
+        if ((size_t)s.first_win[k] == first && s.count[k] > 0) return (int)k;
+    return -1;
+}
+
+}
diff --git a/obia_amd/csrc/slic.hip b/obia_amd/csrc/slic.hip
--- a/obia_amd/csrc/slic.hip
+++ b/obia_amd/csrc/slic.hip
@@ -60,10 +60,11 @@
 __global__ __launch_bounds__(FP_NT) void band_minmax_kernel(const float *__restrict__ src, int Ws, int C,
                                                             const SrcWindow *__restrict__ wins,
                                                             unsigned *__restrict__ keys ,
-                                                            int *__restrict__ nonfinite) {
+                                                            int *__restrict__ nonfinite, int w0, int r0, int r1) {
     __shared__ unsigned s_mn[32], s_mx[32];
-    const int p = blockIdx.y;
+    const int p = w0 + blockIdx.y;
     const SrcWindow wdw = wins[p];
+    const int y_end = min(wdw.h, r1);
     const int period = C / VEC;
     const int active = (FP_NT / period) * period;
     const int tid = threadIdx.x;
@@ -75,7 +76,7 @@
     bool bad = false;
     if (tid < active) {
         const long long row_vecs = (long long)wdw.w * period;
-        for (int y = blockIdx.x; y < wdw.h; y += gridDim.x) {
+        for (int y = r0 + blockIdx.x; y < y_end; y += gridDim.x) {
             const float *row = src + ((long long)(wdw.y0 + y) * Ws + wdw.x0) * C;
             constexpr int MU = 4;
             for (long long e0 = tid; e0 < row_vecs; e0 += (long long)MU * active) {
@@ -394,10 +395,10 @@
         const int gx = (int)grids::slic_band_minmax(maxh, np).x.n;
         if (C % 4 == 0 && (reinterpret_cast<uintptr_t>(src) & 15) == 0)
             hipLaunchKernelGGL(HIP_KERNEL_NAME(band_minmax_kernel<4>), dim3(gx, np), dim3(FP_NT), 0, stream, src, Ws, C, d_windows,
-                               d_keys, (int *)d_nonfinite);
+                               d_keys, (int *)d_nonfinite, 0, 0, 0x7fffffff);
         else
             hipLaunchKernelGGL(HIP_KERNEL_NAME(band_minmax_kernel<1>), dim3(gx, np), dim3(FP_NT), 0, stream, src, Ws, C, d_windows,
-                               d_keys, (int *)d_nonfinite);
+                               d_keys, (int *)d_nonfinite, 0, 0, 0x7fffffff);
     }
     if (minmax_only) { OBIA_HIP_TRY(hipGetLastError()); return OBIA_OK; }
     const bool box = planes && d_fbox != nullptr;
@@ -447,6 +448,28 @@
         default: set_error("bad CP %d", CP); return OBIA_E_INVALID;
     }
 #undef LAUNCH_FEAT
+    OBIA_HIP_TRY(hipGetLastError());
+    return OBIA_OK;
+}
+
+int slic_minmax_init(hipStream_t stream, const SlicBatch &b, unsigned *d_keys) {
+    const size_t nkeys = (size_t)b.nprob * b.C * 2, ntot = nkeys + 2 * (size_t)b.nprob;
+    hipLaunchKernelGGL(keys_init_kernel, dim3(cdiv((long long)ntot, 256)), dim3(256), 0, stream, d_keys, (int)nkeys, (int)ntot);
+    OBIA_HIP_TRY(hipGetLastError());
+    return OBIA_OK;
+}
+int slic_minmax_slice_launch(hipStream_t stream, const SlicBatch &b, const float *src, int Ws, unsigned *d_keys, int w0, int w1, int r0, int r1) {
+    if (!b.normalize || w1 <= w0 || r1 <= r0) return OBIA_OK;
+    if (w0 < 0 || w1 > b.nprob || r0 < 0) { set_error("min / max slice outside the window set"); return OBIA_E_INVALID; }
+    const int C = b.C;
+    unsigned *d_nonfinite = d_keys + (size_t)b.nprob * C * 2;
+    const dim3 grid((unsigned)grids::slic_band_minmax_rows(r1 - r0).x.n, (unsigned)(w1 - w0));
+    if (C % 4 == 0 && (reinterpret_cast<uintptr_t>(src) & 15) == 0)
+        hipLaunchKernelGGL(HIP_KERNEL_NAME(band_minmax_kernel<4>), grid, dim3(FP_NT), 0, stream, src, Ws, C, b.d_windows, d_keys,
+                           (int *)d_nonfinite, w0, r0, r1);
+    else
+        hipLaunchKernelGGL(HIP_KERNEL_NAME(band_minmax_kernel<1>), grid, dim3(FP_NT), 0, stream, src, Ws, C, b.d_windows, d_keys,
+                           (int *)d_nonfinite, w0, r0, r1);
     OBIA_HIP_TRY(hipGetLastError());
     return OBIA_OK;
 }
@@ -572,18 +595,22 @@
     return OBIA_OK;
 }
 
+int slic_features_queue(obia_ctx *ctx, SlicBatch &b, const float *src, int Ws, unsigned *d_keys) {
+    ScopedSpan span(ctx, T_FEAT);
+    SmoothSpec sm;
+    for (int i = 0; i < 3; ++i) sm.sigma[i] = b.sigma[i];
+    OBIA_TRY(smooth_prepare(ctx, sm, b.total_pix, b.CP, b.nprob));
+    b.fuse_features = slic_fuse_features(b, src, Ws);
+    if (b.fuse_features) { b.raw_src = src; b.raw_ws = Ws; b.d_keys = d_keys; }
+    return slic_features_launch(ctx->stream, b, src, Ws, d_keys, &sm, b.fuse_features);
+}
+
 int slic_prepare_features(obia_ctx *ctx, SlicBatch &b, const float *src, int Ws, std::vector<int> *skip) {
-    ScopedSpan span(ctx, T_FEAT);
     const int np = b.nprob;
     const size_t nkeys = (size_t)np * b.C * 2, ntot = nkeys + 2 * (size_t)np;
     unsigned *d_keys = ctx->arena.get<unsigned>(ntot);
     if (!d_keys) return OBIA_E_NOMEM;
-    SmoothSpec sm;
-    for (int i = 0; i < 3; ++i) sm.sigma[i] = b.sigma[i];
-    OBIA_TRY(smooth_prepare(ctx, sm, b.total_pix, b.CP, np));
-    b.fuse_features = slic_fuse_features(b, src, Ws);
-    if (b.fuse_features) { b.raw_src = src; b.raw_ws = Ws; b.d_keys = d_keys; }
-    OBIA_TRY(slic_features_launch(ctx->stream, b, src, Ws, d_keys, &sm, b.fuse_features));
+    OBIA_TRY(slic_features_queue(ctx, b, src, Ws, d_keys));
     std::vector<unsigned> host(ntot);
     OBIA_TRY(read_back(ctx, host.data(), d_keys, ntot * sizeof(unsigned)));
     return slic_features_finish(b, host.data(), host.data() + nkeys, host.data() + nkeys + np, skip);
@@ -744,22 +771,30 @@
     return OBIA_OK;
 }
 
+int slic_count_valid_queue(obia_ctx *ctx, SlicBatch &b, int *d_cnt) {
+    OBIA_TRY(slic_plan_layout(ctx, b));
+    OBIA_TRY(ctx->plan.flush(ctx));
+    int blocks = cdiv(b.maxpix, 256 * 16 * 32);
+    if (blocks < 1) blocks = 1;
+    hipLaunchKernelGGL(count_valid_kernel, dim3(blocks, b.nprob), dim3(256), 0, ctx->stream, b.d_probs, b.d_mask, d_cnt);
+    OBIA_HIP_TRY(hipGetLastError());
+    return OBIA_OK;
+}
+
 int slic_count_valid(obia_ctx *ctx, SlicBatch &b, std::vector<int> &nvalid, int *d_cnt_cleared) {
     const int np = b.nprob;
     Arena &A = ctx->arena;
     nvalid.assign(np, 0);
     OBIA_TRY(slic_plan_layout(ctx, b));
     if (b.masked) {
-        OBIA_TRY(ctx->plan.flush(ctx));
         int *d_cnt = d_cnt_cleared;
         if (!d_cnt) {
+            OBIA_TRY(ctx->plan.flush(ctx));
             d_cnt = A.get<int>(np);
             if (!d_cnt) return OBIA_E_NOMEM;
             OBIA_TRY(fill_async(ctx, d_cnt, 0, sizeof(int) * np));
         }
-        int blocks = cdiv(b.maxpix, 256 * 16 * 32);
-        if (blocks < 1) blocks = 1;
-        hipLaunchKernelGGL(count_valid_kernel, dim3(blocks, np), dim3(256), 0, ctx->stream, b.d_probs, b.d_mask, d_cnt);
+        OBIA_TRY(slic_count_valid_queue(ctx, b, d_cnt));
         OBIA_TRY(read_back(ctx, nvalid.data(), d_cnt, sizeof(int) * np));
     } else {
         for (int p = 0; p < np; ++p) nvalid[p] = b.probs[p].H * b.probs[p].W;
diff --git a/obia_amd/csrc/slic.hpp b/obia_amd/csrc/slic.hpp
--- a/obia_amd/csrc/slic.hpp
+++ b/obia_amd/csrc/slic.hpp
@@ -144,6 +144,9 @@
 double slic_fscale(float maxabs);
 int slic_features_finish(SlicBatch &b, const unsigned *keys, const unsigned *nonfinite, const unsigned *maxabs_bits, std::vector<int> *skip);
 int slic_prepare_features(obia_ctx *ctx, SlicBatch &b, const float *src, int Ws, std::vector<int> *skip = nullptr);
+int slic_features_queue(obia_ctx *ctx, SlicBatch &b, const float *src, int Ws, unsigned *d_keys);
+int slic_minmax_init(hipStream_t stream, const SlicBatch &b, unsigned *d_keys);
+int slic_minmax_slice_launch(hipStream_t stream, const SlicBatch &b, const float *src, int Ws, unsigned *d_keys, int w0, int w1, int r0, int r1);
 float slic_prescale(float ratio, int normalize, int to_lab, bool slic_zero);
 bool slic_use_colour_bound(float ratio, bool to_lab = false);
 void slic_batch_settings(SlicBatch &b, const obia_slic_params &p, int C, int normalize_bands, bool masked);
@@ -158,6 +161,7 @@
 int slic_plan_and_seed(obia_ctx *ctx, SlicBatch &b, const std::vector<int> &n_segments,
                        const std::vector<int> *nvalid = nullptr, const ExternalSeeds *ext = nullptr);
 int slic_count_valid(obia_ctx *ctx, SlicBatch &b, std::vector<int> &nvalid, int *d_cnt_cleared = nullptr);
+int slic_count_valid_queue(obia_ctx *ctx, SlicBatch &b, int *d_cnt);
 int slic_plan_layout(obia_ctx *ctx, SlicBatch &b);
 
 int slic_run_sweeps(obia_ctx *ctx, SlicBatch &b);
diff --git a/obia_amd/csrc/tiling.hip b/obia_amd/csrc/tiling.hip
--- a/obia_amd/csrc/tiling.hip
+++ b/obia_amd/csrc/tiling.hip
@@ -1,3 +1,4 @@
+#include "prefetch_slices.hpp"
 #include "slic.hpp"
 #include "../../include/obia_testing.h"
 
@@ -291,6 +292,12 @@
         bool launched = false;
         bool on_side = false;
         size_t cursor = 0;
+        bool sliced = false;
+        PrefetchSchedule sched;
+        size_t next_slice = 0;
+        size_t host_slices = 0;
+        size_t copy_slices = 0;
+        unsigned long long copy_serial = 0;
     } pf;
 };
 
@@ -305,6 +312,8 @@
 #define OBIA_PREFETCH_BESIDE 0
 #endif
 static int prefetch_white_launch(obia_ctx *ctx, TileState &S, bool beside = false);
+static int prefetch_hand_over(obia_ctx *ctx, TileState &S, size_t first);
+static int prefetch_take(obia_ctx *ctx, TileState &S, size_t np);
 
 static int seed_tiles_skimage(obia_ctx *ctx, TileState &S, const SlicBatch &b, const std::vector<int> &nvalid, std::vector<int> &nseg,
                               std::vector<ExternalSeeds> &ext) {
@@ -367,6 +376,7 @@
     const int np = (int)wins.size();
     if (np == 0) return OBIA_OK;
     Arena &A = ctx->arena;
+    if (!white && S.pf.sliced && !S.pf.launched) OBIA_TRY(prefetch_white_launch(ctx, S));
     const Arena::Mark mk = A.mark();
     SlicBatch b = S.settings;
     for (auto &t : wins) b.windows.push_back(SrcWindow{t.y0, t.x0, t.h, t.w, 0, 0, 0});
@@ -405,8 +415,10 @@
     if (!d_wins || !b.d_windows) return OBIA_E_NOMEM;
     OBIA_TRY(slic_plan_layout(ctx, b));
     OBIA_TRY(ctx->plan.flush(ctx));
-    int *d_tile_any = A.get<int>(np), *d_cnt = A.get<int>(np);
-    if (!d_tile_any || !d_cnt) return OBIA_E_NOMEM;
+    const size_t nkeys = (size_t)np * (size_t)S.C * 2, ntot = nkeys + 2 * (size_t)np;
+    unsigned *d_own_keys = pre ? nullptr : A.get<unsigned>(ntot + (size_t)np);
+    int *d_tile_any = A.get<int>(np), *d_cnt = pre ? A.get<int>(np) : reinterpret_cast<int *>(d_own_keys + ntot);
+    if (!d_tile_any || !d_cnt || (!pre && !d_own_keys)) return OBIA_E_NOMEM;
     {
         ClearSet clr(ctx);
         if (white) {
@@ -433,17 +445,25 @@
         }
     }
     std::vector<int> skip;
+    std::vector<int> nvalid;
     if (pre) {
-        const size_t NP = S.pf.b.windows.size(), nkeys = NP * (size_t)S.C * 2;
+        if (S.pf.sliced) OBIA_TRY(prefetch_take(ctx, S, (size_t)np));
+        const size_t NP = S.pf.b.windows.size(), nk = NP * (size_t)S.C * 2;
         const unsigned *h = S.pf.host.data();
-        OBIA_TRY(slic_features_finish(b, h + S.pf.cursor * (size_t)S.C * 2, h + nkeys + S.pf.cursor, h + nkeys + NP + S.pf.cursor, &skip));
+        OBIA_TRY(slic_features_finish(b, h + S.pf.cursor * (size_t)S.C * 2, h + nk + S.pf.cursor, h + nk + NP + S.pf.cursor, &skip));
         S.pf.cursor += np;
+        debug_sync(ctx, "tiler: mask + features");
+        OBIA_TRY(slic_count_valid(ctx, b, nvalid, d_cnt));
     } else {
-        OBIA_TRY(slic_prepare_features(ctx, b, S.img, S.W, &skip));
-    }
-    std::vector<int> nvalid;
-    debug_sync(ctx, "tiler: mask + features");
-    OBIA_TRY(slic_count_valid(ctx, b, nvalid, d_cnt));
+        OBIA_TRY(slic_features_queue(ctx, b, S.img, S.W, d_own_keys));
+        debug_sync(ctx, "tiler: mask + features");
+        OBIA_TRY(slic_count_valid_queue(ctx, b, d_cnt));
+        std::vector<unsigned> host(ntot + (size_t)np);
+        OBIA_TRY(read_back(ctx, host.data(), d_own_keys, host.size() * sizeof(unsigned)));
+        OBIA_TRY(slic_features_finish(b, host.data(), host.data() + nkeys, host.data() + nkeys + np, &skip));
+        nvalid.resize(np);
+        memcpy(nvalid.data(), host.data() + ntot, sizeof(int) * (size_t)np);
+    }
     debug_sync(ctx, "tiler: count_valid");
     std::vector<int> nseg(np);
     const double pixel_area = S.tp.pixel_width * S.tp.pixel_height;
@@ -474,6 +494,7 @@
     unsigned *const mask4 = b.d_mask4;
     OBIA_TRY(slic_run_sweeps(ctx, b));
     debug_sync(ctx, "tiler: sweeps");
+    if (S.pf.sliced && S.pf.launched) OBIA_TRY(prefetch_hand_over(ctx, S, white ? S.pf.cursor : 0));
     int n_new = 0;
     CcResolve resolve{};
     if (S.sp.enforce_connectivity) {
@@ -655,6 +676,17 @@
                    std::min(S.cly_any, h), std::min(S.clx_any, w), 0};
 }
 
+#ifndef OBIA_PREFETCH_SLICES_DEFAULT
+#define OBIA_PREFETCH_SLICES_DEFAULT 0
+#endif
+constexpr size_t PREFETCH_KEYS_MAX = 64u << 10;
+static int prefetch_slice_rows() {
+    const char *e = std::getenv("OBIA_PREFETCH_SLICES");
+    if (!e || !*e) return OBIA_PREFETCH_SLICES_DEFAULT;
+    const long v = std::strtol(e, nullptr, 10);
+    return v < 0 ? 0 : (v > 0x7fffffffL ? 0x7fffffff : (int)v);
+}
+
 static int prefetch_white_plan(obia_ctx *ctx, TileState &S, int white_order) {
     const int T = S.tp.tile_size;
     const int ntx = cdiv(S.W, T), nty = cdiv(S.Hg, T);
@@ -662,17 +694,23 @@
     pf = TileState::PreFeat();
     if (S.sp.sigma_zyx[0] > 0.0 || S.sp.sigma_zyx[1] > 0.0 || S.sp.sigma_zyx[2] > 0.0) return OBIA_OK;
     SlicBatch b = S.settings;
-    for (int cls = 0; cls < (white_order == 1 ? 2 : 1); ++cls)
+    const bool per_class = white_order == 1 && T > 2 * S.tp.buffer;
+    std::vector<int> batch_windows;
+    for (int cls = 0; cls < (white_order == 1 ? 2 : 1); ++cls) {
+        if (per_class) batch_windows.push_back(0);
         for (int tj = 0; tj < nty; ++tj) {
             if (white_order == 1 && (tj & 1) != cls) continue;
+            if (!per_class) batch_windows.push_back(0);
             for (int ti = 0; ti < ntx; ++ti) {
                 if ((ti + tj) % 2 == 0) continue;
                 const TileWin t = white_window(S, tj, ti);
                 if (t.h <= 0 || t.w <= 0) continue;
                 if (t.y0 < 0 || t.y0 + t.h > S.H) return OBIA_OK;
                 b.windows.push_back(SrcWindow{t.y0, t.x0, t.h, t.w, 0, 0, 0});
+                batch_windows.back() += 1;
             }
         }
+    }
     const size_t NP = b.windows.size();
     if (NP == 0) return OBIA_OK;
     if (slic_batch_layout(b) != OBIA_OK) return OBIA_OK;
@@ -689,8 +727,62 @@
         if (!b.d_fbox) return OBIA_E_NOMEM;
     }
     pf.host.resize(ntot);
+    const int rows = prefetch_slice_rows();
+    if (pf.fused && rows > 0 && T > 2 * S.tp.buffer && ntot * sizeof(unsigned) <= PREFETCH_KEYS_MAX) {
+        std::vector<int> heights(NP);
+        for (size_t p = 0; p < NP; ++p) heights[p] = b.windows[p].h;
+        pf.sched = plan_prefetch_slices(heights, batch_windows, rows);
+        pf.sliced = true;
+    }
     pf.b = std::move(b);
     pf.planned = true;
+    return OBIA_OK;
+}
+
+static int prefetch_queue_slice(obia_ctx *ctx, TileState &S) {
+    TileState::PreFeat &pf = S.pf;
+    const PrefetchSlice &q = pf.sched.slices[pf.next_slice++];
+    ScopedSpan span(ctx, T_FEAT);
+    return slic_minmax_slice_launch(ctx->stream, pf.b, S.img, S.W, pf.d_keys, q.win, q.win + 1, q.r0, q.r1);
+}
+
+static int prefetch_filler(obia_ctx *ctx, void *user) {
+    TileState &S = *static_cast<TileState *>(user);
+    if (S.pf.next_slice >= S.pf.sched.slices.size()) { ctx->filler = nullptr; ctx->filler_user = nullptr; return OBIA_OK; }
+    return prefetch_queue_slice(ctx, S);
+}
+
+static int prefetch_drain(obia_ctx *ctx, TileState &S, int last) {
+    while ((long long)S.pf.next_slice <= (long long)last) OBIA_TRY(prefetch_queue_slice(ctx, S));
+    return OBIA_OK;
+}
+
+static int prefetch_hand_over(obia_ctx *ctx, TileState &S, size_t first) {
+    TileState::PreFeat &pf = S.pf;
+    const int k = prefetch_batch_from(pf.sched, first);
+    if (k < 0) return OBIA_OK;
+    const int last = pf.sched.last[k];
+    if ((long long)pf.host_slices > last || (long long)pf.copy_slices > last) return OBIA_OK;
+    OBIA_TRY(prefetch_drain(ctx, S, last));
+    OBIA_HIP_TRY(hipMemcpyAsync(ctx->pf_landing, pf.d_keys, pf.host.size() * sizeof(unsigned), hipMemcpyDeviceToHost, ctx->stream));
+    pf.copy_slices = pf.next_slice;
+    pf.copy_serial = ctx->rb_serial;
+    return OBIA_OK;
+}
+
+static int prefetch_take(obia_ctx *ctx, TileState &S, size_t np) {
+    TileState::PreFeat &pf = S.pf;
+    if (np == 0 || pf.cursor + np > pf.sched.last_of_win.size()) return OBIA_OK;
+    const int last = pf.sched.last_of_win[pf.cursor + np - 1];
+    if (pf.copy_slices > pf.host_slices && ctx->rb_serial > pf.copy_serial) {
+        memcpy(pf.host.data(), ctx->pf_landing, pf.host.size() * sizeof(unsigned));
+        pf.host_slices = pf.copy_slices;
+    }
+    if ((long long)pf.host_slices > last) return OBIA_OK;
+    OBIA_TRY(prefetch_drain(ctx, S, last));
+    const size_t queued = pf.next_slice;
+    OBIA_TRY(read_back(ctx, pf.host.data(), pf.d_keys, pf.host.size() * sizeof(unsigned)));
+    pf.host_slices = queued;
     return OBIA_OK;
 }
 
@@ -700,6 +792,19 @@
     pf.launched = true;
     if (pf.fused) beside = false;
     OBIA_TRY(upload_async(ctx, pf.b.d_windows, pf.b.windows.data(), sizeof(SrcWindow) * pf.b.windows.size()));
+    if (pf.sliced) {
+        const size_t bytes = pf.host.size() * sizeof(unsigned);
+        if (bytes > ctx->pf_landing_bytes) {
+            if (ctx->pf_landing) (void)hipHostFree(ctx->pf_landing);
+            ctx->pf_landing = nullptr; ctx->pf_landing_bytes = 0;
+            OBIA_HIP_TRY(hipHostMalloc(&ctx->pf_landing, PREFETCH_KEYS_MAX, hipHostMallocDefault));
+            ctx->pf_landing_bytes = PREFETCH_KEYS_MAX;
+        }
+        OBIA_TRY(slic_minmax_init(ctx->stream, pf.b, pf.d_keys));
+        ctx->filler = prefetch_filler;
+        ctx->filler_user = &S;
+        return OBIA_OK;
+    }
     if (beside) {
         OBIA_TRY(side_stream(ctx));
         hipStream_t side = ctx->side;
@@ -719,7 +824,7 @@
     if (!S.pf.planned) return OBIA_OK;
     OBIA_TRY(prefetch_white_launch(ctx, S));
     if (S.pf.on_side) { OBIA_HIP_TRY(hipStreamWaitEvent(ctx->stream, ctx->aux_join, 0)); S.pf.on_side = false; }
-    OBIA_TRY(read_back(ctx, S.pf.host.data(), S.pf.d_keys, S.pf.host.size() * sizeof(unsigned)));
+    if (!S.pf.sliced) OBIA_TRY(read_back(ctx, S.pf.host.data(), S.pf.d_keys, S.pf.host.size() * sizeof(unsigned)));
     S.pf.ready = true;
     S.pf.cursor = 0;
     return OBIA_OK;
@@ -785,6 +890,7 @@
                           const obia_tiling_params *tp, const obia_slic_params *sp, int seeding, obia_pick_fn picks, void *picks_user,
                           int32_t *labels_out, int64_t *n_segments_out) {
     TileState S;
+    struct FillerScope { obia_ctx *c; ~FillerScope() { c->filler = nullptr; c->filler_user = nullptr; } } filler_scope{ctx};
     OBIA_TRY(check_seeding(seeding, picks));
     OBIA_TRY(tiler_init(ctx, S, img, mask, H, W, C, H, 0, tp, sp, labels_out, 0));
     S.seeding = seeding; S.pick_fn = picks; S.pick_user = picks_user;
```
